# soham2560/MPCHoloNavigation

Hardware: AMD Instinct MI355X
Metric: rollouts/sec per computeVelocityCommands() tick (higher is better)
Workload: dtype f32

## Files before the change

mpcholonavigation_amd/csrc/smpc_api.cpp:

```cpp

#include "smpc_ctx.h"

#include <emmintrin.h>

namespace smpc_impl {

thread_local std::string g_create_error;

int fail(smpc_ctx* c, int code, const std::string& msg)
{
  if (c) c->err = msg; else g_create_error = msg;
  return code;
}

int wait_map_upload(smpc_ctx* c)
{
  if (!c->map_pending) return SMPC_OK;
  HIPCK(c, hipEventSynchronize(c->ev_map));
  c->map_pending = false;
  return SMPC_OK;
}

void bar_copy(void* dev_dst, const void* host_src, size_t n)
{
  const __m128i* src = static_cast<const __m128i*>(host_src);
  __m128i* dst = static_cast<__m128i*>(dev_dst);
  for (size_t i = 0; i < n / 16; ++i) _mm_stream_si128(dst + i, _mm_load_si128(src + i));
  _mm_sfence();
}

void bar_flush(const smpc_ctx* c)
{
  if (c->hdp_flush) *c->hdp_flush = 1u;
}

static volatile uint32_t* find_hdp_flush(int dev)
{
  hipDeviceProp_t prop;
  if (hipGetDeviceProperties(&prop, dev) != hipSuccess) return nullptr;
  void* h = dlopen("libhsa-runtime64.so.1", RTLD_NOW | RTLD_NOLOAD);
  if (!h) h = dlopen("libhsa-runtime64.so.1", RTLD_NOW | RTLD_LOCAL);
  if (!h) return nullptr;
  using agent_t = struct {uint64_t handle;};
  using iterate_fn = int (*)(int (*)(agent_t, void*), void*);
  using info_fn = int (*)(agent_t, int, void*);
  using init_fn = int (*)();
  static init_fn p_init = reinterpret_cast<init_fn>(dlsym(h, "hsa_init"));
  static iterate_fn p_iter = reinterpret_cast<iterate_fn>(dlsym(h, "hsa_iterate_agents"));
  static info_fn p_info = reinterpret_cast<info_fn>(dlsym(h, "hsa_agent_get_info"));
  if (!p_init || !p_iter || !p_info || p_init() != 0) return nullptr;
  struct Want {
    uint32_t domain, bdf;
    volatile uint32_t* reg;
  } want{static_cast<uint32_t>(prop.pciDomainID),
         (static_cast<uint32_t>(prop.pciBusID) << 8) | (static_cast<uint32_t>(prop.pciDeviceID) << 3), nullptr};
  auto cb = [](agent_t a, void* data) -> int {
    Want* w = static_cast<Want*>(data);
    int type = 0;
    if (p_info(a, 17, &type) != 0 || type != 1) return 0;
    uint32_t bdf = 0, domain = 0;
    if (p_info(a, 0xA006, &bdf) != 0) return 0;
    if (p_info(a, 0xA00F, &domain) != 0) domain = w->domain;
    if ((bdf & ~7u) != w->bdf || domain != w->domain) return 0;
    struct {uint32_t* mem; uint32_t* reg;} f{nullptr, nullptr};
    if (p_info(a, 0xA00E, &f) == 0) w->reg = f.mem;
    return 1;
  };
  (void)p_iter(cb, &want);
  return want.reg;
}

void free_ctx(smpc_ctx* c)
{
  if (!c) return;
  (void)hipSetDevice(c->device);
  for (float* p : {c->d_tvx, c->d_nvx, c->d_nvy, c->d_nwz, c->d_costs[0], c->d_costs[1], c->d_traj[0],
         c->d_traj[1], c->d_traj[2], c->d_partials, c->d_tuple, c->d_out, c->d_u_iter, c->d_furthest})
    if (p) (void)hipFree(p);
  if (c->d_stats || c->d_stats_part) {
    (void)hipStreamSynchronize(c->stream);
    if (c->d_stats) (void)hipFree(c->d_stats);
    if (c->d_stats_part) (void)hipFree(c->d_stats_part);
  }
  for (hipEvent_t e : c->ev_stats) if (e) (void)hipEventDestroy(e);
  if (c->l_gm || c->l_rm[0] || c->l_rm[1] || c->l_rm[2]) {
    (void)hipStreamSynchronize(c->stream);
    for (float* p : {c->l_gm, c->l_rm[0], c->l_rm[1], c->l_rm[2]})
      if (p) (void)hipFree(p);
  }
  for (hipEvent_t e : c->ev_lim) if (e) (void)hipEventDestroy(e);
  if (c->fill_stream) {
    (void)hipStreamSynchronize(c->fill_stream);
    (void)hipStreamDestroy(c->fill_stream);
  }
  if (c->ev_fill) (void)hipEventDestroy(c->ev_fill);
  for (float* p : {c->b_tvx, c->b_nvx, c->b_nvy, c->b_nwz})
    if (p) (void)hipFree(p);
  if (c->d_map) (void)hipFree(c->d_map);
  if (c->d_timeline) (void)hipFree(c->d_timeline);
  if (c->map.cells) (void)hipHostFree(c->map.cells);
  if (c->ev_map) (void)hipEventDestroy(c->ev_map);
  if (c->d_tick && !c->defer_upload) (void)hipFree(c->d_tick);
  if (c->d_lut) (void)hipFree(c->d_lut);
  if (c->d_lut_fp) (void)hipFree(c->d_lut_fp);
  if (c->h_lut_fp) (void)hipHostFree(c->h_lut_fp);
  if (c->h_lut) (void)hipHostFree(c->h_lut);
  if (c->h_tick && !c->defer_upload) (void)hipHostFree(c->h_tick);
  if (c->h_out) (void)hipHostFree(c->h_out);
  if (c->comm && rccl()) (void)rccl()->CommDestroy(c->comm);
  if (c->d_all) (void)hipFree(c->d_all);
  for (uint32_t r = 0; r < c->p2p.world; ++r)
    if (r != c->p2p.rank && c->p2p.peer[r]) (void)hipIpcCloseMemHandle(c->p2p.peer[r]);
  if (c->p2p_mailbox) (void)hipFree(c->p2p_mailbox);
  if (c->ev0) (void)hipEventDestroy(c->ev0);
  if (c->ev1) (void)hipEventDestroy(c->ev1);
  for (hipEvent_t e : c->evp) if (e) (void)hipEventDestroy(e);
  if (c->own_stream) (void)hipStreamDestroy(c->own_stream);
  delete c;
}

void begin_limit_iteration(smpc_ctx* c, const float* u_dev)
{
  c->lim_u_dev = u_dev;
  if (++c->lim_iter == 0) ++c->lim_iter;
}

static int limit_noise(smpc_ctx* c, bool group_major)
{
  const uint32_t B = c->cfg.batch_size, T = c->cfg.time_steps;
  SmpcLimitArgs a{};
  if (group_major) {
    const size_t ngm = SMPC_GM_ELEMS(B, T);
    if (!c->l_gm) {
      HIPCK(c, hipMalloc(&c->l_gm, 3 * ngm * sizeof(float)));
      HIPCK(c, hipMemsetAsync(c->l_gm, 0, 3 * ngm * sizeof(float), c->stream));
    }
    a.src[0] = c->d_tvx; a.src[1] = c->holonomic ? c->d_tvy : nullptr; a.src[2] = c->d_twz;
    a.dst[0] = c->l_gm; a.dst[1] = c->holonomic ? c->l_gm + ngm : nullptr; a.dst[2] = c->l_gm + 2 * ngm;
  } else {
    const int rc = ensure_row_major(c);
    if (rc != SMPC_OK) return rc;
    for (int k = 0; k < 3; ++k)
      if (!c->l_rm[k] && (k != 1 || c->holonomic)) HIPCK(c, hipMalloc(&c->l_rm[k], static_cast<size_t>(B) * T * sizeof(float)));
    a.src[0] = c->d_nvx; a.src[1] = c->holonomic ? c->d_nvy : nullptr; a.src[2] = c->d_nwz;
    for (int k = 0; k < 3; ++k) a.dst[k] = c->l_rm[k];
  }
  a.B = B; a.T = T;
  a.u_dev = c->lim_u_dev;
  if (!a.u_dev) {
    const TickLayout tl = tick_layout(T, std::max(c->P, 1u));
    memcpy(a.u_arg, c->h_tick + tl.u, 3 * T * sizeof(float));
  }
  a.v0[0] = c->dev.svx; a.v0[1] = c->dev.svy; a.v0[2] = c->dev.swz;
  const float dt = c->cfg.model_dt;
  a.dhi[0] = dt * c->lim[0]; a.dhi[1] = dt * c->lim[2]; a.dhi[2] = dt * c->lim[3];
  a.dlo[0] = dt * c->lim[1]; a.dlo[1] = -a.dhi[1]; a.dlo[2] = -a.dhi[2];
  const bool prof = (c->cfg.flags & SMPC_FLAG_PROFILE) != 0;
  if (prof) {
    for (hipEvent_t& e : c->ev_lim)
      if (!e) HIPCK(c, hipEventCreate(&e));
    HIPCK(c, hipEventRecord(c->ev_lim[0], c->stream));
  }
  c->launched = true;
  HIPCK(c, smpc_launch_limit_noise(a, group_major, c->stream));
  if (prof) HIPCK(c, hipEventRecord(c->ev_lim[1], c->stream));
  return SMPC_OK;
}

int use_limited_noise(smpc_ctx* c, SmpcDev& d, bool group_major)
{
  if (!c->lim_on) return SMPC_OK;
  uint32_t& have = group_major ? c->lim_gm_iter : c->lim_rm_iter;
  if (have != c->lim_iter || c->lim_iter == 0) {
    if (c->lim_iter == 0) begin_limit_iteration(c, nullptr);
    const int rc = limit_noise(c, group_major);
    if (rc != SMPC_OK) return rc;
    have = c->lim_iter;
  }
  if (group_major) {
    const size_t ngm = SMPC_GM_ELEMS(c->cfg.batch_size, c->cfg.time_steps);
    d.tvx = c->l_gm; d.tvy = c->l_gm + ngm; d.twz = c->l_gm + 2 * ngm;
  } else {
    d.nvx = c->l_rm[0]; d.nwz = c->l_rm[2];
    if (c->holonomic) d.nvy = c->l_rm[1];
  }
  return SMPC_OK;
}

int launch_furthest(smpc_ctx* c, float* d_furthest)
{
  {
    const int rc = ensure_row_major(c);
    if (rc != SMPC_OK) return rc;
  }
  HIPCK(c, hipMemsetAsync(d_furthest, 0, sizeof(float), c->stream));
  SmpcDev d = c->dev;
  {
    const int rc = use_limited_noise(c, d, false);
    if (rc != SMPC_OK) return rc;
  }
  d.flags = c->gate_flags & SD_NEED_FURTHEST;
  d.furthest_out = reinterpret_cast<uint32_t*>(d_furthest);
  SmpcLds L = make_lds(0, c->P, d.T, (pass_block(c->R) / 64), false);
  c->launched = true;
  HIPCK(c, wave_launch(wave_select(c->R, 1, d.T), d, L, c->plan.wave.grid, c->plan.wave.block, c->stream));
  return SMPC_OK;
}

int begin_tick(smpc_ctx* c, const smpc_tick_in* in, const float* u_in)
{
  const int rc = prepare_tick(c, in, u_in);
  if (rc != SMPC_OK) return rc;
  c->passes = 0;
  c->evp_used = 0;
  c->costs_cur = 0;
  return SMPC_OK;
}

int refuse_sharded(smpc_ctx* c)
{
  if (c->two_coll_fp)
    return fail(c, SMPC_ERR_UNSUPPORTED,
                "sharded tick: consider_footprint=true with both ObstaclesCritic and CostCritic in the list");
  if (c->cfg.iteration_count != 1)
    return fail(c, SMPC_ERR_UNSUPPORTED, "sharded tick: iteration_count must be 1");
  return SMPC_OK;
}

uint32_t next_seq(smpc_ctx* c)
{
  if (++c->seq == 0) ++c->seq;
  c->poll_seq = c->seq;
  return c->seq;
}

void fill_score_args(smpc_ctx* c, uint32_t flags, const float* u_dev, const float* d_furthest,
                     uint32_t furthest_hint, bool finish, const float* finish_furthest, SmpcDev& d,
                     SmpcFinal& fin)
{
  d = c->dev;
  d.flags = flags;
  if (u_dev) {
    d.u = u_dev;
    d.u_inline = 0;
  }
  d.d_furthest = d_furthest;
  d.furthest_hint = furthest_hint;
  d.costs = c->d_costs[c->costs_cur];
  d.costs_prev = c->d_costs[c->costs_cur ^ 1];
  fin = SmpcFinal{};
  fin.enabled = finish ? 1 : 0;
  fin.vx_max = c->c_vx_max; fin.vx_min = c->c_vx_min; fin.vy_max = c->c_vy; fin.wz_max = c->c_wz;
  fin.u_dev = c->d_out; fin.u_host = c->h_out_dev; fin.furthest_used = finish_furthest;
  if (finish && c->knobs.poll) {
    fin.done_counter = scratch_word(c, SMPC_SCRATCH_REDUCE_COUNTER);
    fin.seq = next_seq(c);
  }
  if (finish && c->acker_r >= 0.f) {
    c->acker_seq = fin.seq;
    fin.done_counter = nullptr;
    fin.seq = 0;
  }
}

struct PassChoice {
  PassPlan::Kind kind;
  const void* inst;
  const PassGeom* geom;
};
static PassChoice pass_for(const smpc_ctx* c, uint32_t flags)
{
  const PassPlan& pl = c->plan;
  const uint32_t T = c->dev.T;
  if (pl.kind == PassPlan::kSplit)
    if (const SplitInst* k = split_select(flags, T, c->dev.step, pl.split_nseg)) return {PassPlan::kSplit, k, &pl.split};
  if (pl.kind != PassPlan::kWave) {
    const LaneInst* k = lane_select(flags, T, pl.rr, false, c->acker_r, pl.pow, pl.nh);
    if (k || !(pl.rr || (flags & SD_STORE_TRAJ))) return {PassPlan::kLane, k, &pl.lane};
  }
  return {PassPlan::kWave, wave_select(c->R, c->score_mode, T), &pl.wave};
}

int launch_score(smpc_ctx* c, uint32_t flags, const float* u_dev, const float* d_furthest,
                 uint32_t furthest_hint, float* d_tuple, bool finish, const float* finish_furthest)
{
  SmpcDev d;
  SmpcFinal fin;
  fill_score_args(c, flags, u_dev, d_furthest, furthest_hint, finish, finish_furthest, d, fin);
  const PassChoice pass = pass_for(c, flags);
  {
    const int rc = use_limited_noise(c, d, pass.kind != PassPlan::kWave);
    if (rc != SMPC_OK) return rc;
  }
  const bool prof = (c->cfg.flags & SMPC_FLAG_PROFILE) && c->evp_used + 2 <= 8;
  if (prof) HIPCK(c, hipEventRecord(c->evp[c->evp_used], c->stream));
  const uint32_t nblk = pass.geom->grid;
  const bool tail = pass.kind != PassPlan::kSplit && c->knobs.fused_reduce && nblk <= SMPC_TAIL_MAX_GRID &&
    (pass.kind != PassPlan::kLane || pass.geom->block == smpc_lane_block()) && pass.geom->lds.total >= smpc_tail_lds_bytes(d.T);
  const bool polled = fin.enabled && fin.done_counter;
  c->poll_words = !polled ? 0u : tail ? smpc_tail_reduce_blocks(d.T, nblk) : smpc_reduce_blocks(d.T);
  static_assert(smpc_reduce_blocks(64u * SMPC_MAX_R) <= kPollWords, "one completion word per reducing block");
  if (tail) {
    float& mark = c->h_out[SMPC_RESULT_AT(d.T) + SMPC_R_MARK];
    if (mark == SMPC_MARK_TAIL_LATE) mark = SMPC_MARK_NONE;
    d.tail = 1;
    d.tail_counter = scratch_word(c, SMPC_SCRATCH_TAIL_COUNTER);
    d.tuple = d_tuple;
    d.fin = fin;
  }
  c->launched = true;
  c->last_pass_kind = pass.kind;
  if (pass.kind == PassPlan::kSplit) {
    HIPCK(c, split_launch(static_cast<const SplitInst*>(pass.inst), d, pass.geom->lds, nblk, c->stream));
  } else if (pass.kind == PassPlan::kLane) {
    HIPCK(c, lane_launch(static_cast<const LaneInst*>(pass.inst), d, nullptr, 1, pass.geom->lds, nblk, pass.geom->block, c->stream));
  } else {
    const int rc_rm = ensure_row_major(c);
    if (rc_rm != SMPC_OK) return rc_rm;
    HIPCK(c, wave_launch(static_cast<const WaveInst*>(pass.inst), d, pass.geom->lds, nblk, pass.geom->block, c->stream));
  }
  if (prof) {
    HIPCK(c, hipEventRecord(c->evp[c->evp_used + 1], c->stream));
    c->evp_used += 2;
  }
  if (!tail) HIPCK(c, smpc_launch_reduce(c->d_partials, nblk, d.T, d.neg_inv_temp, d_tuple, fin, c->stream));
  if (finish && c->acker_r >= 0.f)
    HIPCK(c, smpc_launch_ackermann(c->d_out, c->h_out_dev, d.T, c->acker_r, c->acker_seq, c->stream));
  c->passes++;
  return SMPC_OK;
}

int launch_combine(smpc_ctx* c, const float* d_tuples, uint32_t n, const float* d_furthest_used)
{
  const uint32_t T = c->cfg.time_steps;
  uint32_t seq = 0;
  if (c->knobs.poll) {
    seq = next_seq(c);
    c->poll_words = 0;
  }
  const bool acker = c->acker_r >= 0.f;
  HIPCK(c, smpc_launch_combine(d_tuples, n, T, c->dev.neg_inv_temp, c->c_vx_max, c->c_vx_min,
                               c->c_vy, c->c_wz, c->d_out, c->d_out + SMPC_RESULT_AT(T), d_furthest_used,
                               c->h_out_dev, acker ? 0u : seq, c->stream));
  if (acker) HIPCK(c, smpc_launch_ackermann(c->d_out, c->h_out_dev, T, c->acker_r, seq, c->stream));
  return SMPC_OK;
}

void store_control_sequence(const smpc_ctx* c, float* u_inout)
{
  const uint32_t T = c->cfg.time_steps;
  if (c->holonomic) {
    memcpy(u_inout, c->h_out, 3 * T * sizeof(float));
    return;
  }
  memcpy(u_inout, c->h_out, T * sizeof(float));
  memcpy(u_inout + 2 * T, c->h_out + 2 * T, T * sizeof(float));
}

static int check_canary(smpc_ctx* c)
{
  c->launched = false;
  if (!c->canary_expect) return SMPC_OK;
  const uint32_t got = reinterpret_cast<const volatile uint32_t*>(c->h_out)[SMPC_RESULT_AT(c->cfg.time_steps) + SMPC_R_CANARY];
  if (got == c->canary_expect) return SMPC_OK;
  char msg[200];
  snprintf(msg, sizeof(msg), "the scoring pass read tick block %u, not %u: the per-tick upload did not reach the "
           "device in time (CPU stores through the BAR: %s); SMPC_NO_BAR_TICK=1 selects the copy", got, c->canary_expect,
           c->bar_tick ? "on" : "off");
  c->bar_tick = false;
  return fail(c, SMPC_ERR_DEVICE, msg);
}

int fetch_out(smpc_ctx* c)
{
  if (c->poll_seq) {
    const volatile uint32_t* flag =
      reinterpret_cast<const volatile uint32_t*>(c->h_out + SMPC_RESULT_AT(c->cfg.time_steps) + SMPC_R_DONE);
    const uint32_t want = c->poll_seq;
    c->poll_seq = 0;
    const uint32_t nwords = c->poll_words;
    static_assert(SMPC_R_BLOCK_DONE == SMPC_R_DONE + 1u, "the per-block words follow the completion word");
    c->poll_words = 0;
    auto arrived = [&]() {
      if (nwords == 0) return *flag == want;
      for (uint32_t r = 0; r < nwords; ++r)
        if (flag[1 + r] != want) return false;
      return true;
    };
    for (uint32_t spin = 0; spin < 4000000u; ++spin) {
      if (arrived()) {
        __atomic_thread_fence(__ATOMIC_ACQUIRE);
        if (tick_result(c).mark() == SMPC_MARK_TAIL_LATE)
          return fail(c, SMPC_ERR_DEVICE, "the scoring launch's reduction did not see every block's partial");
        return check_canary(c);
      }
      __builtin_ia32_pause();
    }
  }
  HIPCK(c, hipStreamSynchronize(c->stream));
  return check_canary(c);
}

float profile_pass_ms(smpc_ctx* c)
{
  float sum = 0.f;
  uint32_t n = 0;
  for (uint32_t i = 0; i + 1 < c->evp_used; i += 2) {
    float ms = 0.f;
    if (hipEventElapsedTime(&ms, c->evp[i], c->evp[i + 1]) == hipSuccess) {
      sum += ms;
      n++;
    }
  }
  return n ? sum / n : 0.f;
}

int fill_tick_out(smpc_ctx* c, smpc_tick_out* out, bool fail_flag, bool furthest_valid, uint32_t furthest,
                  const float* non_colliding, bool device_ms)
{
  if (!out) return SMPC_OK;
  const TickResult r = tick_result(c);
  memset(out, 0, sizeof(*out));
  out->fail_flag = fail_flag ? 1 : 0;
  out->furthest_valid = furthest_valid ? 1 : 0;
  out->furthest_reached_path_point = furthest;
  out->non_colliding = static_cast<uint32_t>(non_colliding ? *non_colliding : r.non_colliding());
  out->min_cost = r.min_cost();
  out->sum_w = r.sum_w();
  out->passes = c->passes;
  if (device_ms && (c->cfg.flags & SMPC_FLAG_PROFILE)) {
    HIPCK(c, hipEventSynchronize(c->ev1));
    float ms = 0.f;
    if (hipEventElapsedTime(&ms, c->ev0, c->ev1) == hipSuccess) out->device_ms = ms;
  }
  out->score_pass_ms = profile_pass_ms(c);
  out->pass_kind = c->last_pass_kind;
  return SMPC_OK;
}

uint32_t fail_only_flags(const smpc_ctx* c)
{
  const uint32_t coll = (c->gate_flags & SD_COST) ? (SD_COST | SD_FP_COST) : (SD_OBSTACLES | SD_FP_OBSTACLES);
  return c->gate_flags & (SD_CONSTRAINT | coll | SD_STORE_TRAJ | SD_TRACK_UNKNOWN);
}

uint32_t scoring_flags(const smpc_ctx* c, bool fail_sticky)
{
  const uint32_t keep = SD_STORE_TRAJ | SD_TRACK_UNKNOWN;
  return fail_sticky ? (c->gate_flags & keep) : c->gate_flags;
}

int update_time_major(smpc_ctx* c)
{
  if (!c->use_tpr) return SMPC_OK;
  const uint32_t B = c->cfg.batch_size, T = c->cfg.time_steps;
  HIPCK(c, smpc_launch_relayout(c->d_nvx, c->d_tvx, B, T, true, c->stream));
  HIPCK(c, smpc_launch_relayout(c->d_nvy, c->d_tvy, B, T, true, c->stream));
  HIPCK(c, smpc_launch_relayout(c->d_nwz, c->d_twz, B, T, true, c->stream));
  return SMPC_OK;
}

int ensure_row_major(smpc_ctx* c)
{
  if (c->rm_valid) return SMPC_OK;
  const uint32_t B = c->cfg.batch_size, T = c->cfg.time_steps;
  HIPCK(c, smpc_launch_relayout(c->d_tvx, c->d_nvx, B, T, false, c->stream));
  if (c->holonomic) HIPCK(c, smpc_launch_relayout(c->d_tvy, c->d_nvy, B, T, false, c->stream));
  HIPCK(c, smpc_launch_relayout(c->d_twz, c->d_nwz, B, T, false, c->stream));
  c->rm_valid = true;
  return SMPC_OK;
}

static int launch_draw(smpc_ctx* c, float* nvx, float* nvy, float* nwz, float* tvx, float* tvy, float* twz,
                       hipStream_t st, bool* rm_valid_out)
{
  const uint64_t n = static_cast<uint64_t>(c->cfg.batch_size) * c->cfg.time_steps;
  const uint64_t base = c->cfg.shard_offset * c->cfg.time_steps;
  const uint32_t B = c->cfg.batch_size, T = c->cfg.time_steps;
  if (c->use_tpr && (T & 3u) == 0 && !getenv("SMPC_NO_FUSED_FILL")) {
    HIPCK(c, smpc_launch_fill_noise_tm(tvx, B, T, base, c->seed, 0, c->epoch, c->cfg.vx_std, st));
    HIPCK(c, smpc_launch_fill_noise_tm(twz, B, T, base, c->seed, 1, c->epoch, c->cfg.wz_std, st));
    if (c->holonomic)
      HIPCK(c, smpc_launch_fill_noise_tm(tvy, B, T, base, c->seed, 2, c->epoch, c->cfg.vy_std, st));
    else
      HIPCK(c, hipMemsetAsync(tvy, 0, SMPC_GM_ELEMS(B, T) * sizeof(float), st));
    *rm_valid_out = false;
    return SMPC_OK;
  }
  HIPCK(c, smpc_launch_fill_noise(nvx, n, base, c->seed, 0, c->epoch, c->cfg.vx_std, st));
  HIPCK(c, smpc_launch_fill_noise(nwz, n, base, c->seed, 1, c->epoch, c->cfg.wz_std, st));
  if (c->holonomic) HIPCK(c, smpc_launch_fill_noise(nvy, n, base, c->seed, 2, c->epoch, c->cfg.vy_std, st));
  if (c->use_tpr) {
    HIPCK(c, smpc_launch_relayout(nvx, tvx, B, T, true, st));
    HIPCK(c, smpc_launch_relayout(nvy, tvy, B, T, true, st));
    HIPCK(c, smpc_launch_relayout(nwz, twz, B, T, true, st));
  }
  *rm_valid_out = true;
  return SMPC_OK;
}

int cancel_redraw(smpc_ctx* c)
{
  if (!c->redraw_pending) return SMPC_OK;
  HIPCK(c, hipEventSynchronize(c->ev_fill));
  c->redraw_pending = false;
  return SMPC_OK;
}

int absorb_redraw(smpc_ctx* c)
{
  if (!c->redraw_pending) return SMPC_OK;
  HIPCK(c, hipStreamWaitEvent(c->stream, c->ev_fill, 0));
  std::swap(c->d_nvx, c->b_nvx);
  std::swap(c->d_nvy, c->b_nvy);
  std::swap(c->d_nwz, c->b_nwz);
  std::swap(c->d_tvx, c->b_tvx);
  std::swap(c->d_tvy, c->b_tvy);
  std::swap(c->d_twz, c->b_twz);
  c->rm_valid = c->redraw_rm_valid;
  c->redraw_pending = false;
  c->noise_gen++;
  return SMPC_OK;
}

int draw_noise(smpc_ctx* c)
{
  int rc = cancel_redraw(c);
  if (rc != SMPC_OK) return rc;
  bool rm = true;
  rc = launch_draw(c, c->d_nvx, c->d_nvy, c->d_nwz, c->d_tvx, c->d_tvy, c->d_twz, c->stream, &rm);
  if (rc != SMPC_OK) return rc;
  HIPCK(c, hipStreamSynchronize(c->stream));
  c->have_noise = true;
  c->rm_valid = rm;
  c->noise_gen++;
  return SMPC_OK;
}

int redraw_async(smpc_ctx* c)
{
  if (c->redraw_pending) return SMPC_OK;
  const size_t n = static_cast<size_t>(c->cfg.batch_size) * c->cfg.time_steps * sizeof(float);
  if (!c->fill_stream) {
    HIPCK(c, hipStreamCreateWithFlags(&c->fill_stream, hipStreamNonBlocking));
    HIPCK(c, hipEventCreateWithFlags(&c->ev_fill, hipEventDisableTiming));
  }
  if (c->use_tpr && !c->b_tvx) {
    const size_t ngm = SMPC_GM_ELEMS(c->cfg.batch_size, c->cfg.time_steps) * sizeof(float);
    HIPCK(c, hipMalloc(&c->b_tvx, 3 * ngm));
    HIPCK(c, hipMemset(c->b_tvx, 0, 3 * ngm));
    c->b_tvy = c->b_tvx + ngm / sizeof(float);
    c->b_twz = c->b_tvy + ngm / sizeof(float);
  }
  if (!c->b_nvx) {
    HIPCK(c, hipMalloc(&c->b_nvx, n));
    HIPCK(c, hipMalloc(&c->b_nvy, n));
    HIPCK(c, hipMalloc(&c->b_nwz, n));
    if (!c->holonomic) HIPCK(c, hipMemset(c->b_nvy, 0, n));
  }
  c->epoch++;
  bool rm = true;
  const int rc = launch_draw(c, c->b_nvx, c->b_nvy, c->b_nwz, c->b_tvx, c->b_tvy, c->b_twz, c->fill_stream, &rm);
  if (rc != SMPC_OK) return rc;
  HIPCK(c, hipEventRecord(c->ev_fill, c->fill_stream));
  c->redraw_rm_valid = rm;
  c->redraw_pending = true;
  return SMPC_OK;
}

static Knobs read_knobs()
{
  Knobs k;
  auto set = [](const char* name) {return getenv(name) != nullptr;};
  auto number = [](const char* name, int unset) {const char* e = getenv(name); return e ? atoi(e) : unset;};
  if (const char* e = getenv("SMPC_PASS"))
    k.pass = !strcmp(e, "wave") ? Knobs::kWave : !strcmp(e, "lane") ? Knobs::kLane : !strcmp(e, "split") ? Knobs::kSplit : Knobs::kAuto;
  k.no_split = set("SMPC_NO_SPLIT");
  k.split_nseg = static_cast<uint32_t>(std::max(0, number("SMPC_SPLIT_NSEG", 0)));
  k.lane_reread = number("SMPC_LANE_REREAD", 0) != 0;
  k.half_blocks = !set("SMPC_NO_HALF_BLOCKS");
  k.max_blocks_per_cu = static_cast<uint32_t>(std::max(0, number("SMPC_MAX_BLOCKS_PER_CU", 0)));
  k.balanced_grid = !set("SMPC_NO_BALANCED_GRID");
  k.fused_reduce = set("SMPC_FUSED_REDUCE");
  k.no_inline_tick = set("SMPC_NO_INLINE_TICK");
  k.pinned_tick = set("SMPC_PINNED_TICK");
  k.poll = !set("SMPC_NO_POLL");
  k.bar_tick = !set("SMPC_NO_BAR_TICK");
  k.hdp_flush = !set("SMPC_NO_HDP_FLUSH");
  k.repeat_pass = set("SMPC_DEBUG_REPEAT_PASS");
  k.stale_tick = static_cast<uint32_t>(number("SMPC_DEBUG_STALE_TICK", 0));
  k.small_window = set("SMPC_SMALL_WINDOW");
  k.window_side_max = number("SMPC_WINDOW_SIDE_MAX", -1);
  k.furthest_prune = number("SMPC_FURTHEST_PRUNE", 1) != 0;
  if (const char* e = getenv("SMPC_FOOTPRINT_PASS")) k.footprint_general = !strcmp(e, "general");
  if (const char* e = getenv("SMPC_NONHOLO_PASS")) k.nonholo_omni = !strcmp(e, "omni");
  return k;
}

using clk = std::chrono::steady_clock;
static void report_tick_timing(clk::time_point t_in, clk::time_point t_prep, clk::time_point t_launch, clk::time_point t_fetch)
{
  static thread_local double acc[5] = {0, 0, 0, 0, 0};
  static thread_local unsigned n = 0;
  static thread_local clk::time_point t_prev_out;
  const auto t_out = clk::now();
  auto us = [](clk::time_point a, clk::time_point b) {return std::chrono::duration<double, std::micro>(b - a).count();};
  if (n > 0) acc[0] += us(t_prev_out, t_in);
  acc[1] += us(t_in, t_prep);
  acc[2] += us(t_prep, t_launch);
  acc[3] += us(t_launch, t_fetch);
  acc[4] += us(t_fetch, t_out);
  t_prev_out = t_out;
  if (++n == 1024) {
    fprintf(stderr, "[smpc tick timing] caller %.2f us, prepare + upload %.2f, launches %.2f, wait %.2f, collect %.2f (per tick, %u ticks)\n",
            acc[0] / (n - 1), acc[1] / n, acc[2] / n, acc[3] / n, acc[4] / n, n);
    n = 0;
    for (double& a : acc) a = 0;
  }
// ... 817 lines not shown
```

mpcholonavigation_amd/csrc/smpc_ctx.h:

```cpp
#ifndef SMPC_CTX_H_
#define SMPC_CTX_H_

#include <hip/hip_runtime.h>
#include <rccl/rccl.h>
#include <dlfcn.h>

#include <algorithm>
#include <chrono>
#include <cmath>
#include <cstdio>
#include <cstdlib>
#include <cstring>
#include <limits>
#include <new>
#include <string>
#include <vector>

#include "../../include/smpc.h"
#include "smpc_dev.h"
#include "smpc_inst.h"
#include "smpc_limit.h"

#pragma GCC visibility push(hidden)

hipError_t smpc_launch_reduce(const float* partials, uint32_t nblk, uint32_t T,
                              float neg_inv_temp, float* tuple, const SmpcFinal& fin,
                              hipStream_t st);
hipError_t smpc_launch_combine(const float* tuples, uint32_t G, uint32_t T, float neg_inv_temp,
                               float vx_max, float vx_min, float vy_max, float wz_max,
                               float* u_out, float* result, const float* furthest_used,
                               float* host_out, uint32_t seq, hipStream_t st);
hipError_t smpc_launch_fill_noise(float* out, uint64_t n, uint64_t base, uint64_t seed,
                                  uint32_t stream, uint32_t epoch, float sigma, hipStream_t st);
hipError_t smpc_launch_fill_noise_tm(float* dst, uint32_t B, uint32_t T, uint64_t base, uint64_t seed,
                                     uint32_t stream, uint32_t epoch, float sigma, hipStream_t st);
hipError_t smpc_launch_ackermann(float* u_dev, float* u_host, uint32_t T, float min_r, uint32_t seq,
                                 hipStream_t st);
hipError_t smpc_launch_p2p_exchange(const float* my_tuple, const SmpcP2P& x, uint32_t T, int mode,
                                    float* d_furthest, float neg_inv_temp, float vx_max, float vx_min,
                                    float vy_max, float wz_max, float* u_out, float* result,
                                    const float* furthest_used, float* host_out, uint32_t seq,
                                    hipStream_t st);

hipError_t smpc_launch_relayout(const float* src, float* dst, uint32_t B, uint32_t T, bool to_gm, hipStream_t st);
uint32_t smpc_lane_block();
uint32_t smpc_lane_block_rr();
hipError_t smpc_launch_lane_reduce(const float* v, const float* w, float* out, hipStream_t st);
hipError_t smpc_launch_row_reduce(const float* v, float* out, uint32_t n, hipStream_t st);
uint32_t smpc_split_block();
uint32_t smpc_split_rollouts_per_block(uint32_t nseg);
hipError_t smpc_launch_reduce_many(const SmpcReduceArgs* d_many, uint32_t n, uint32_t T, hipStream_t st);
hipError_t smpc_launch_sincos(const float* x, uint32_t n, float* sn, float* cs, hipStream_t st);
hipError_t smpc_launch_philox(const uint32_t* ctr, uint32_t k0, uint32_t k1, uint32_t n, uint32_t* out,
                              hipStream_t st);
hipError_t smpc_launch_box_muller(const uint32_t* r0, const uint32_t* r1, uint32_t n, float* z0, float* z1,
                                  hipStream_t st);

hipError_t smpc_launch_limit_noise(const SmpcLimitArgs& a, bool group_major, hipStream_t st);

namespace smpc_impl {

extern thread_local std::string g_create_error;


struct RcclApi {
  ncclResult_t (*GetUniqueId)(ncclUniqueId*) = nullptr;
  ncclResult_t (*CommInitRank)(ncclComm_t*, int, ncclUniqueId, int) = nullptr;
  ncclResult_t (*CommDestroy)(ncclComm_t) = nullptr;
  ncclResult_t (*AllGather)(const void*, void*, size_t, ncclDataType_t, ncclComm_t, hipStream_t) = nullptr;
  ncclResult_t (*AllReduce)(const void*, void*, size_t, ncclDataType_t, ncclRedOp_t, ncclComm_t,
                            hipStream_t) = nullptr;
  const char* (*GetErrorString)(ncclResult_t) = nullptr;
};
const RcclApi* rccl();

inline uint32_t pass_block(int R) {return R == 4 ? 512u : 1024u;}
constexpr uint32_t kLaneMinBatch = 60u * 1024u;
constexpr uint32_t kSplitMinBatch = 12u * 1024u;
constexpr uint32_t kSplitMinBatchShort = 20000u;
constexpr uint32_t kLaneMaxT = 128;
constexpr uint32_t kPollWords = SMPC_BLOCK_DONE_WORDS;
static_assert(SMPC_TUPLE_HEADER == SMPC_R_F_USED, "the shard tuple's header is the first four result slots, in their order");
constexpr uint32_t kMaxGrid = SMPC_MAX_GRID;
constexpr uint32_t kWindowBytes = 96 * 96;
constexpr uint32_t kWindowSideMax = 144;
constexpr uint32_t kLdsPerCu = 160 * 1024;

inline uint32_t align_up(uint32_t v, uint32_t a) {return (v + a - 1) / a * a;}

struct HostCostmap {
  uint8_t* cells = nullptr;
  size_t cap = 0;
  uint32_t W = 0, H = 0;
  double ox = 0, oy = 0, res = 1;
  bool track_unknown = false;
  float inscribed_radius = 0, cost_scaling_factor = 0, inflation_radius = 0;
  bool set = false;
};

inline bool world_to_map(const HostCostmap& c, double wx, double wy, unsigned& mx, unsigned& my)
{
  if (wx < c.ox || wy < c.oy) return false;
  const double qx = (wx - c.ox) / c.res, qy = (wy - c.oy) / c.res;
  if (!(qx < 4294967296.0) || !(qy < 4294967296.0)) return false;
  mx = static_cast<unsigned>(qx);
  my = static_cast<unsigned>(qy);
  return mx < c.W && my < c.H;
}

inline bool within_tol(float tol, double rx, double ry, double gx, double gy)
{
  const double dist_sq = std::pow(gx - rx, 2) + std::pow(gy - ry, 2);
  const float tol_sq = tol * tol;
  return dist_sq < tol_sq;
}

struct Knobs {
  enum Pass {kAuto, kWave, kLane, kSplit} pass = kAuto;
  bool no_split = false;
  uint32_t split_nseg = 0;
  bool lane_reread = false;
  bool half_blocks = true;
  uint32_t max_blocks_per_cu = 0;
  bool balanced_grid = true;
  bool fused_reduce = false;
  bool no_inline_tick = false;
  bool pinned_tick = false;
  bool poll = true;
  bool bar_tick = true;
  bool hdp_flush = true;
  bool repeat_pass = false;
  uint32_t stale_tick = 0;
  bool small_window = false;
  int window_side_max = -1;
  bool furthest_prune = true;
  bool footprint_general = false;
  bool nonholo_omni = false;
};

struct OccCache {
  const void* fn = nullptr;
  uint32_t block = 0, lds = 0;
  uint32_t blocks = 1;
  uint32_t get(const void* f, uint32_t blk, uint32_t lds_bytes)
  {
    if (f != fn || blk != block || lds_bytes != lds) {
      int nb = 0;
      if (inst_occupancy(f, blk, lds_bytes, &nb) != hipSuccess || nb < 1) nb = 1;
      fn = f; block = blk; lds = lds_bytes;
      blocks = static_cast<uint32_t>(nb);
    }
    return blocks;
  }
};

struct PassGeom {
  uint32_t grid = 0, block = 0;
  SmpcLds lds{};
};
struct PassPlan {
  enum Kind : uint32_t {kWave = 0, kLane = 1, kSplit = 2};
  Kind kind = kWave;
  PassGeom wave;
  PassGeom lane;
  PassGeom split;
  bool rr = false;
  bool pow = false;
  bool nh = false;
  uint32_t split_nseg = 4;
  uint32_t window_bytes = 0;
};

struct FurthestPredictor {
  bool hint_valid = false;
  uint32_t hint = 0;
  float hint_F = 0.f;
  float hint_Fp = 0.f;
  bool hint_Fp_valid = false;
  bool hint_is_this_ticks = false;
  float hint_drift = 0.f;
  bool anchor_valid = false;
  double anchor_x = 0, anchor_y = 0;
  double anchor_ex = 0, anchor_ey = 0, cur_ex = 0, cur_ey = 0;
  bool anchor_e_valid = false, cur_e_valid = false;
  std::vector<float> anchor_px, anchor_py;
  uint32_t noise_gen_remembered = 0;
  void forget()
  {
    hint_valid = false;
    hint_Fp_valid = false;
    hint_is_this_ticks = false;
    hint_drift = 0.f;
  }
  void drop_hint() {hint_valid = false;}
};

}

struct smpc_ctx {
  smpc_config cfg{};
  smpc_critic_params critics{};
  float c_vx_max = 0, c_vx_min = 0, c_vy = 0, c_wz = 0;
  int device = 0;
  int num_cu = 256;
  hipStream_t own_stream = nullptr, stream = nullptr;
  hipEvent_t ev0 = nullptr, ev1 = nullptr;
  hipEvent_t evp[8] = {};
  uint32_t evp_used = 0;
  float* d_nvx = nullptr;
  float* d_nvy = nullptr;
  float* d_nwz = nullptr;
  float* d_tvx = nullptr;
  float* d_tvy = nullptr;
  float* d_twz = nullptr;
  float* b_nvx = nullptr;
  float* b_nvy = nullptr;
  float* b_nwz = nullptr;
  float* b_tvx = nullptr;
  float* b_tvy = nullptr;
  float* b_twz = nullptr;
  hipStream_t fill_stream = nullptr;
  hipEvent_t ev_fill = nullptr;
  bool redraw_pending = false, redraw_rm_valid = true;
  uint32_t noise_gen = 0;
  bool use_tpr = false;
  bool rm_valid = true;
  smpc_impl::Knobs knobs;
  smpc_impl::PassPlan plan;
  smpc_impl::OccCache occ_wave, occ_lane, occ_split;
  bool lane_forced = false;
  bool two_coll_fp = false;
  uint32_t last_pass_kind = 0;
  bool defer_upload = false;
  std::vector<double> fp_x, fp_y;
  double fp_circumscribed_radius = 0.0, fp_layer_scale = -1.0;
  SmpcLut* d_lut_fp = nullptr;
  SmpcLut* h_lut_fp = nullptr;
  ncclComm_t comm = nullptr;
  int comm_rank = 0, comm_world = 0;
  float* d_all = nullptr;
  float* p2p_mailbox = nullptr;
  SmpcP2P p2p{};
  uint32_t p2p_xseq = 0;
  uint32_t p2p_timeout_ms = 10000;
  bool p2p_failed = false;
  bool pang_any = false;
  float prune_table[SMPC_PRUNE_FLOATS] = {};
  std::vector<float> prune_px, prune_py;
  uint32_t prune_k0 = 0;
  bool in_group = false;
  float* d_costs[2] = {nullptr, nullptr};
  float* d_traj[3] = {nullptr, nullptr, nullptr};
  int costs_cur = 0;
  bool have_noise = false, rng_mode = false;
  uint64_t seed = 0;
  uint32_t epoch = 0;
  smpc_impl::HostCostmap map;
  uint8_t* d_map = nullptr;
  size_t d_map_bytes = 0;
  hipEvent_t ev_map = nullptr;
  bool map_pending = false;
  uint64_t map_bytes_last = 0, map_bytes_total = 0;
  unsigned long long* d_timeline = nullptr;
  SmpcLut* d_lut = nullptr;
  SmpcLut* h_lut = nullptr;
  uint64_t lut_key = 0, map_version = 1, critics_version = 1;
  bool lut_valid = false;
  uint8_t* d_tick = nullptr;
  uint8_t* h_tick = nullptr;
  size_t tick_cap = 0;
  bool bar_tick = false;
  volatile uint32_t* hdp_flush = nullptr;
  size_t tick_used = 0;
  uint32_t tick_no = 0;
  uint32_t canary_expect = 0;
  bool launched = false;
  float* d_partials = nullptr;
  float* d_tuple = nullptr;
  float* d_out = nullptr;
  float* d_u_iter = nullptr;
  float* h_out = nullptr;
  float* h_out_dev = nullptr;
  float* d_furthest = nullptr;
  int R = 1;
  SmpcDev dev{};
  uint32_t gate_flags = 0;
  int score_mode = 0;
  static int score_mode_for(const smpc_critic_params& cr)
  {
    return (cr.obstacles.cost_power == 1 && cr.path_align.cost_power == 1 &&
           cr.path_follow.cost_power == 1 && cr.goal_angle.cost_power == 1 &&
           cr.prefer_forward.cost_power == 1) ? 0 : 2;
  }
  bool tick_ready = false;
  bool fail_in = false;
  uint32_t P = 0;
  uint32_t passes = 0;
  smpc_impl::FurthestPredictor pred;
  uint64_t spec_misses = 0;
  smpc_tick_in step_in{};
  std::vector<float> step_px, step_py;
  bool step_remembered = false;
  bool holonomic = true;
  float acker_r = -1.f;
  uint32_t acker_seq = 0;
  uint32_t seq = 0, poll_seq = 0;
  uint32_t poll_words = 0;
  float* d_stats = nullptr;
  double* d_stats_part = nullptr;
  uint32_t stats_ld = 0;
  bool lim_on = false;
  float lim[4] = {0.f, 0.f, 0.f, 0.f};
  float* l_rm[3] = {nullptr, nullptr, nullptr};
  float* l_gm = nullptr;
  const float* lim_u_dev = nullptr;
  uint32_t lim_iter = 0;
  uint32_t lim_rm_iter = 0, lim_gm_iter = 0;
  hipEvent_t ev_lim[2] = {};
  hipEvent_t ev_stats[4] = {};
  float stats_pass_ms = 0.f, stats_reduce_ms = 0.f;
  std::string err;
};

namespace smpc_impl {

int fail(smpc_ctx* c, int code, const std::string& msg);

#define HIPCK(ctx, call)                                                               \
  do {                                                                                 \
    hipError_t e__ = (call);                                                           \
    if (e__ != hipSuccess)                                                             \
      return fail(ctx, SMPC_ERR_DEVICE,                                                \
                  std::string(#call) + ": " + hipGetErrorString(e__));                \
  } while (0)

int wait_map_upload(smpc_ctx* c);
void bar_copy(void* dev_dst, const void* host_src, size_t n);
void bar_flush(const smpc_ctx* c);
void free_ctx(smpc_ctx* c);

struct TickLayout {
  size_t u, px, py, pyaw, D, pf_idx, pvalid, pa_active, pang_active, pal_active, lut_cost, canary, prune, total;
};
TickLayout tick_layout(uint32_t T, uint32_t P);
void build_prune_table(const float* px, const float* py, uint32_t P, uint32_t k0, bool on, float* out);

SmpcLds make_lds(uint32_t window_bytes, uint32_t P, uint32_t T, uint32_t nwave, bool with_map,
                 uint32_t nsamp = 0);
SmpcLds lane_lds(uint32_t window_bytes, uint32_t P, uint32_t T, bool rr = false);
SmpcLds split_lds(uint32_t window_bytes, uint32_t P, uint32_t T, uint32_t nseg);

int check_tick(smpc_ctx* c, const smpc_tick_in* in);
void remember_furthest(smpc_ctx* c, const smpc_tick_in* in, float F);
void predict_hint(smpc_ctx* c, const smpc_tick_in* in, const float* u_in);
int prepare_tick(smpc_ctx* c, const smpc_tick_in* in, const float* u_in);

int launch_furthest(smpc_ctx* c, float* d_furthest);
void fill_score_args(smpc_ctx* c, uint32_t flags, const float* u_dev, const float* d_furthest,
                     uint32_t furthest_hint, bool finish, const float* finish_furthest, SmpcDev& d,
                     SmpcFinal& fin);
int launch_score(smpc_ctx* c, uint32_t flags, const float* u_dev, const float* d_furthest,
                 uint32_t furthest_hint, float* d_tuple, bool finish = false,
                 const float* finish_furthest = nullptr);
int launch_combine(smpc_ctx* c, const float* d_tuples, uint32_t n, const float* d_furthest_used);
void store_control_sequence(const smpc_ctx* c, float* u_inout);
int fetch_out(smpc_ctx* c);

int begin_tick(smpc_ctx* c, const smpc_tick_in* in, const float* u_in);
int refuse_sharded(smpc_ctx* c);
uint32_t next_seq(smpc_ctx* c);
inline uint32_t* scratch_word(const smpc_ctx* c, uint32_t k) {return reinterpret_cast<uint32_t*>(c->d_furthest) + k;}
struct TickResult {
  const float* slot;
  float min_cost() const {return slot[SMPC_R_MIN_COST];}
  float sum_w() const {return slot[SMPC_R_SUM_W];}
  float F_local() const {return slot[SMPC_R_F_LOCAL];}
  float non_colliding() const {return slot[SMPC_R_NON_COLLIDING];}
  float F_used() const {return slot[SMPC_R_F_USED];}
  float mark() const {return slot[SMPC_R_MARK];}
};
inline TickResult tick_result(const smpc_ctx* c) {return TickResult{c->h_out + SMPC_RESULT_AT(c->cfg.time_steps)};}
int fill_tick_out(smpc_ctx* c, smpc_tick_out* out, bool fail_flag, bool furthest_valid, uint32_t furthest,
                  const float* non_colliding = nullptr, bool device_ms = false);
float profile_pass_ms(smpc_ctx* c);
uint32_t fail_only_flags(const smpc_ctx* c);
uint32_t scoring_flags(const smpc_ctx* c, bool fail_sticky);
void begin_limit_iteration(smpc_ctx* c, const float* u_dev);
int use_limited_noise(smpc_ctx* c, SmpcDev& d, bool group_major);
int update_time_major(smpc_ctx* c);
int ensure_row_major(smpc_ctx* c);
int draw_noise(smpc_ctx* c);
int redraw_async(smpc_ctx* c);
int cancel_redraw(smpc_ctx* c);
int absorb_redraw(smpc_ctx* c);

}

#pragma GCC visibility pop

#endif
```

mpcholonavigation_amd/csrc/smpc_dev.h:

```cpp
#ifndef SMPC_DEV_H_
#define SMPC_DEV_H_

#include <stdint.h>

#define SD_OBSTACLES 0x001u
#define SD_PATH_ALIGN 0x002u
#define SD_PATH_FOLLOW 0x004u
#define SD_GOAL_ANGLE 0x008u
#define SD_PREFER_FORWARD 0x010u
#define SD_USE_PATH_YAW 0x020u
#define SD_ACCUMULATE 0x040u
#define SD_STORE_TRAJ 0x080u
#define SD_TRACK_UNKNOWN 0x100u
#define SD_NEED_FURTHEST 0x200u
#define SD_LOCAL_FURTHEST 0x400u
#define SD_CONSTRAINT 0x800u
#define SD_COST 0x1000u
#define SD_GOAL 0x2000u
#define SD_TWIRLING 0x4000u
#define SD_PATH_ANGLE 0x8000u
#define SD_DEADBAND 0x10000u
#define SD_FP_OBSTACLES 0x20000u
#define SD_FP_COST 0x40000u
#define SD_PATH_ALIGN_LEGACY 0x80000u
#define SD_PAL_USE_PATH_YAW 0x100000u
#define SD_EXTRA_CRITICS (SD_CONSTRAINT | SD_COST | SD_GOAL | SD_TWIRLING | SD_PATH_ANGLE | SD_DEADBAND | \
                          SD_FP_OBSTACLES | SD_FP_COST | SD_PATH_ALIGN_LEGACY)

#define SMPC_GM_ROLLOUTS(B) ((((B) + 63u) / 64u) * 64u)
#define SMPC_GM_STEPS(T) (((T) + 3u) & ~3u)
#define SMPC_GM_ELEMS(B, T) ((size_t)SMPC_GM_ROLLOUTS(B) * SMPC_GM_STEPS(T))
#define SMPC_GM_INDEX(b, t, T) \
  (((((size_t)(b) >> 6) * (SMPC_GM_STEPS(T) >> 2) + ((t) >> 2)) * 64u + ((b) & 63u)) * 4u + ((t) & 3u))

#define SMPC_MAX_PATH 1024
#define SMPC_MAX_R 4

struct SmpcLut {
  float crit;
  float rep;
};

struct SmpcFinal {
  int enabled;
  float vx_max, vx_min, vy_max, wz_max;
  float* u_dev;
  float* u_host;
  const float* furthest_used;
  uint32_t* done_counter;
  uint32_t seq;
};

struct SmpcDev {
  uint32_t B, T, P;
  uint32_t nsamp;
  uint32_t step;
  uint32_t flags;
  double x0, y0;
  float yaw0, cos0, sin0;
  float svx, svy, swz;
  float dt;
  const float* nvx;
  const float* nvy;
  const float* nwz;
  const float* tvx;
  const float* tvy;
  const float* twz;
  const float* u;
  const float* costs_prev;
  float* costs;
  float* traj_x;
  float* traj_y;
  float* traj_yaw;
  const uint8_t* map;
  uint32_t W, H;
  double ox, oy, res;
  float oxf, oyf, rinvf;
  float cell_eps;
  uint32_t cost_t0;
  int32_t win_x0, win_y0, win_w, win_h;
  float wxf, wyf;
  float cxf, cyf;
  float cell_eps_w;
  float x00f, y00f;
  const SmpcLut* lut;
  const float* px;
  const float* py;
  const float* pyaw;
  const float* D;
  const uint8_t* pvalid;
  const uint8_t* pa_active;
  const uint32_t* pf_idx;
  const float* prune;
  const float* d_furthest;
  uint32_t furthest_hint;
  float obs_critical_w, obs_repulsion_w, obs_collision_cost;
  float obs_rep_over_T;
  uint32_t obs_power;
  float pa_weight;
  uint32_t pa_power;
  float pf_weight;
  uint32_t pf_power;
  float ga_weight, ga_goal_yaw;
  uint32_t ga_power;
  float pfw_weight;
  uint32_t pfw_power;
  float con_weight, con_max_vel, con_min_vel;
  uint32_t con_power;
  float con_acker_r;
  const float* lut_cost;
  float cost_w254, cost_collision_cost;
  float cost_critical;
  uint32_t cost_near_goal;
  uint32_t cost_power;
  double goal_x, goal_y;
  float goal_weight;
  uint32_t goal_power;
  float tw_weight;
  uint32_t tw_power;
  const uint8_t* pang_active;
  float pang_weight;
  uint32_t pang_power, pang_offset;
  int32_t pang_correct;
  const uint8_t* pal_active;
  float pal_weight, pal_eval;
  uint32_t pal_power;
  double db_vx, db_vy, db_wz;
  float db_weight;
  uint32_t db_power;
  uint32_t fp_n;
  float fp_pic;
  const SmpcLut* lut_fp;
  double fp_x[16], fp_y[16];
  float g_vx, g_vy, g_wz;
  float neg_inv_temp;
  float k2;
  float* partials;
  uint32_t* furthest_out;
  uint32_t tail;
  uint32_t* tail_counter;
  float* tuple;
  SmpcFinal fin;
  unsigned long long* timeline;
  uint32_t canary_echo;
  uint32_t tick_inline;
  uint32_t u_inline;
  uint16_t io_px, io_py, io_pyaw, io_D, io_pf_idx, io_pvalid, io_pa_active, io_pang_active, io_pal_active, io_pad;
  uint8_t tick_bytes[1536] __attribute__((aligned(16)));
  float u_arg[3 * 64] __attribute__((aligned(16)));
};
#define SMPC_INLINE_TICK_CAP 1536u
#define SMPC_MAX_GRID 2048u
#define SMPC_CANARY_SLOT(T) (SMPC_MAX_GRID * (4u + 3u * (T)))
#define SMPC_TAIL_MAX_GRID 512u
#define SMPC_TAIL_STAMPS_AT (8192u + 2048u * 8u)
#define SMPC_SCAN_COUNT_AT (SMPC_TAIL_STAMPS_AT + 8u * 16u)
#define SMPC_PRUNE_ENTRIES 16u
#define SMPC_PRUNE_FLOATS (4u + 8u * SMPC_PRUNE_ENTRIES)
static inline uint32_t smpc_tail_lds_bytes(uint32_t T) {return (512u + 64u + ((4u + 3u * T + 63u) / 64u) * 2048u + 4u) * 4u;}

#define SMPC_R_MIN_COST 0u
#define SMPC_R_SUM_W 1u
#define SMPC_R_F_LOCAL 2u
#define SMPC_R_NON_COLLIDING 3u
#define SMPC_R_F_USED 4u
#define SMPC_R_CANARY 5u
#define SMPC_R_MARK 6u
#define SMPC_R_DONE 7u
#define SMPC_R_BLOCK_DONE 8u
#define SMPC_BLOCK_DONE_WORDS 32u
#define SMPC_RESULT_AT(T) (3u * (T))
#define SMPC_RESULT_FLOATS(T) (SMPC_RESULT_AT(T) + SMPC_R_BLOCK_DONE)
#define SMPC_RESULT_HOST_FLOATS(T) (SMPC_RESULT_FLOATS(T) + SMPC_BLOCK_DONE_WORDS)
static_assert(SMPC_R_MIN_COST == 0u && SMPC_R_SUM_W == 1u && SMPC_R_F_LOCAL == 2u && SMPC_R_NON_COLLIDING == 3u &&
              SMPC_R_F_USED == 4u, "result slots 0-4: the tuple header, then the furthest point used");
static_assert(SMPC_R_CANARY == 5u && SMPC_R_MARK == 6u && SMPC_R_DONE == 7u && SMPC_R_BLOCK_DONE == 8u,
              "result slots 5-8: canary echo, mark, completion word, per-block completion words");
static inline constexpr uint32_t smpc_tuple_floats(uint32_t T) {return SMPC_R_F_USED + 3u * T;}
#define SMPC_MARK_NONE 0.0f
#define SMPC_MARK_PEER_LATE 1.0f
#define SMPC_MARK_TAIL_LATE 2.0f
static inline constexpr uint32_t smpc_reduce_blocks(uint32_t T) {return (smpc_tuple_floats(T) + 31u) / 32u;}
static inline constexpr uint32_t smpc_tail_reduce_blocks(uint32_t T, uint32_t grid)
{
  const uint32_t groups = (smpc_tuple_floats(T) + 63u) / 64u;
  return groups < grid ? groups : grid;
}

#define SMPC_SCRATCH_FURTHEST 0u
#define SMPC_SCRATCH_REDUCE_COUNTER 2u
#define SMPC_SCRATCH_P2P_STATE 3u
#define SMPC_SCRATCH_TAIL_COUNTER 4u
#define SMPC_SCRATCH_WORDS 8u
static_assert(SMPC_SCRATCH_TAIL_COUNTER + 2u <= SMPC_SCRATCH_WORDS, "the scratch allocation holds every word");

#if defined(__HIPCC__)
struct SmpcTickPtrs {
  const float* u;
  const float* px;
  const float* py;
  const float* pyaw;
  const float* D;
  const uint32_t* pf_idx;
  const uint8_t* pvalid;
  const uint8_t* pa_active;
  const uint8_t* pang_active;
  const uint8_t* pal_active;
};
__device__ __forceinline__ SmpcTickPtrs smpc_tick_ptrs(const SmpcDev& p, bool kernarg_is_dev)
{
  SmpcTickPtrs t{p.u, p.px, p.py, p.pyaw, p.D, p.pf_idx, p.pvalid, p.pa_active, p.pang_active, p.pal_active};
#if defined(__HIP_DEVICE_COMPILE__)
  if (kernarg_is_dev && p.tick_inline) {
    const uint8_t* k = reinterpret_cast<const uint8_t*>(__builtin_amdgcn_kernarg_segment_ptr()) +
                       __builtin_offsetof(SmpcDev, tick_bytes);
    if (p.u_inline) t.u = reinterpret_cast<const float*>(reinterpret_cast<const uint8_t*>(__builtin_amdgcn_kernarg_segment_ptr()) +
                                                         __builtin_offsetof(SmpcDev, u_arg));
    t.px = reinterpret_cast<const float*>(k + p.io_px);
    t.py = reinterpret_cast<const float*>(k + p.io_py);
    t.pyaw = reinterpret_cast<const float*>(k + p.io_pyaw);
    t.D = reinterpret_cast<const float*>(k + p.io_D);
    t.pf_idx = reinterpret_cast<const uint32_t*>(k + p.io_pf_idx);
    t.pvalid = k + p.io_pvalid;
    t.pa_active = k + p.io_pa_active;
    t.pang_active = k + p.io_pang_active;
    t.pal_active = k + p.io_pal_active;
  }
#else
  (void)kernarg_is_dev;
#endif
  return t;
}
#endif

#if defined(__HIPCC__)
__host__ __device__
#endif
static inline uint32_t smpc_furthest_index(float F) {return (uint32_t)(F + 0.5f);}


#define SMPC_P2P_MAX_RANKS 16
struct SmpcP2P {
  float* peer[SMPC_P2P_MAX_RANKS];
  uint32_t world, rank;
  uint32_t slot_floats;
  uint32_t xseq;
  uint32_t* state;
  unsigned long long timeout_ticks;
};

struct SmpcReduceArgs {
  const float* partials;
  float* tuple;
  uint32_t nblk;
  SmpcFinal fin;
  float* host_out;
  uint32_t seq;
  float neg_inv_temp;
};

struct SmpcLds {
  uint32_t off_lut, off_px, off_py, off_pyaw, off_D, off_valid, off_scr;
  uint32_t off_pts4;
  uint32_t off_prune;
  uint32_t scr_stride;
  uint32_t scr_pts;
  uint32_t scr_ring;
  uint32_t scr_c;
  uint32_t seg_shift;
  uint32_t group;
  uint32_t total;
};

struct SmpcWaveGeom {
  SmpcLds lds;
  uint32_t grid;
};

struct SmpcStatsDst {
  float* stats;
  uint32_t ld;
};

#endif
```

mpcholonavigation_amd/csrc/smpc_group.cpp:

```cpp
#include "smpc_ctx.h"
#include "smpc_group.h"

using namespace smpc_impl;

extern "C" {

int smpc_group_create(smpc_ctx* const* ctxs, uint32_t n, smpc_group** out)
{
  if (!ctxs || !n || !out) return fail(nullptr, SMPC_ERR_INVALID, "null argument");
  *out = nullptr;
  for (uint32_t i = 0; i < n; ++i) {
    if (!ctxs[i]) return fail(nullptr, SMPC_ERR_INVALID, "null ctx");
    if (ctxs[i]->device != ctxs[0]->device || ctxs[i]->cfg.time_steps != ctxs[0]->cfg.time_steps)
      return fail(nullptr, SMPC_ERR_INVALID, "a group's contexts share the device and time_steps");
    if (ctxs[i]->defer_upload) return fail(nullptr, SMPC_ERR_STATE, "ctx already in a group");
  }
  smpc_group* g = new (std::nothrow) smpc_group();
  if (!g) return fail(nullptr, SMPC_ERR_NOMEM, "out of memory");
  smpc_ctx* c0 = ctxs[0];
  if (hipSetDevice(c0->device) != hipSuccess) {
    delete g;
    return fail(nullptr, SMPC_ERR_DEVICE, "hipSetDevice");
  }
  g->slot = align_up(static_cast<uint32_t>(c0->tick_cap), 256);
  g->off_dev = g->slot * n;
  g->off_red = g->off_dev + align_up(static_cast<uint32_t>(sizeof(SmpcDev)) * n, 256);
  g->off_geo = g->off_red + align_up(static_cast<uint32_t>(sizeof(SmpcReduceArgs)) * n, 256);
  g->total = g->off_geo + align_up(static_cast<uint32_t>(sizeof(SmpcWaveGeom)) * n, 256);
  g->off_fdev = g->total;
  g->off_fgeo = g->off_fdev + align_up(static_cast<uint32_t>(sizeof(SmpcDev)) * n, 256);
  g->off_sdst = g->off_fgeo + align_up(static_cast<uint32_t>(sizeof(SmpcWaveGeom)) * n, 256);
  g->off_sred = g->off_sdst + align_up(static_cast<uint32_t>(sizeof(SmpcStatsDst)) * n, 256);
  g->total_stats = g->off_sred + align_up(static_cast<uint32_t>(sizeof(SmpcStatsReduceArgs)) * n, 256);
  if (hipHostMalloc(&g->h_all, g->total_stats, hipHostMallocDefault) != hipSuccess ||
    hipMalloc(&g->d_all, g->total_stats) != hipSuccess)
  {
    if (g->h_all) (void)hipHostFree(g->h_all);
    delete g;
    return fail(nullptr, SMPC_ERR_NOMEM, "group buffers");
  }
  g->stream = c0->own_stream;
  for (uint32_t i = 0; i < n; ++i) {
    smpc_ctx* c = ctxs[i];
    (void)hipStreamSynchronize(c->stream);
    g->ctxs.push_back(c);
    g->saved_stream.push_back(c->stream);
    g->saved_h_tick.push_back(c->h_tick);
    g->saved_d_tick.push_back(c->d_tick);
    c->stream = g->stream;
    c->h_tick = g->h_all + g->slot * i;
    c->d_tick = g->d_all + g->slot * i;
    c->defer_upload = true;
    c->in_group = true;
    c->lut_valid = false;
  }
  *out = g;
  return SMPC_OK;
}

void smpc_group_destroy(smpc_group* g)
{
  if (!g) return;
  (void)hipStreamSynchronize(g->stream);
  for (size_t i = 0; i < g->ctxs.size(); ++i) {
    smpc_ctx* c = g->ctxs[i];
    c->stream = g->saved_stream[i];
    c->h_tick = g->saved_h_tick[i];
    c->d_tick = g->saved_d_tick[i];
    c->defer_upload = false;
    c->in_group = false;
  }
  if (g->h_all) (void)hipHostFree(g->h_all);
  if (g->d_all) (void)hipFree(g->d_all);
  if (g->d_stats) (void)hipFree(g->d_stats);
  if (g->d_stats_part) (void)hipFree(g->d_stats_part);
  if (g->h_stats_out) (void)hipHostFree(g->h_stats_out);
  delete g;
}

int smpc_group_stats(const smpc_group* g, uint64_t* batched_launches, uint64_t* single_ticks)
{
  if (!g) return SMPC_ERR_INVALID;
  if (batched_launches) *batched_launches = g->batched_launches;
  if (single_ticks) *single_ticks = g->single_ticks;
  return SMPC_OK;
}

int smpc_group_optimize_some(smpc_group* g, const smpc_tick_in* ins, float* const* u_inout,
                             smpc_tick_out* outs, const uint8_t* take)
{
  if (!g || !ins || !u_inout) return fail(nullptr, SMPC_ERR_INVALID, "null argument");
  const uint32_t n = static_cast<uint32_t>(g->ctxs.size());
  auto taken = [&](uint32_t i) {return !take || take[i] != 0;};
  uint32_t first = 0;
  while (first < n && !taken(first)) ++first;
  if (first == n) return SMPC_OK;
  smpc_ctx* c0 = g->ctxs[first];
  HIPCK(c0, hipSetDevice(c0->device));
  if (g->launched) {
    HIPCK(c0, hipStreamSynchronize(g->stream));
    g->launched = false;
  }
  auto single = [&](uint32_t i) -> int {
    smpc_ctx* c = g->ctxs[i];
    c->defer_upload = false;
    const int rc = smpc_optimize(c, &ins[i], u_inout[i], outs ? &outs[i] : nullptr);
    c->defer_upload = true;
    g->single_ticks++;
    return rc;
  };
  static const bool timing = getenv("SMPC_GROUP_TIMING") != nullptr;
  auto now = [] {return std::chrono::steady_clock::now();};
  auto us_between = [](auto a, auto b) {return std::chrono::duration<double, std::micro>(b - a).count();};
  const auto t_start = now();
  const uint32_t T = c0->cfg.time_steps;
  std::vector<const void*> part(n, nullptr);
  std::vector<uint32_t> flags(n);
  bool lane_ok = true;
  uint32_t lane_first = n, Pmax = 0, window_bytes = 0, gridx = 0;
  const LaneInst* inst = nullptr;
  static const char kLaneTag = 0;
  for (uint32_t i = 0; i < n; ++i) {
    if (!taken(i)) continue;
    smpc_ctx* c = g->ctxs[i];
    if (!u_inout[i]) return fail(c, SMPC_ERR_INVALID, "null control sequence");
    int rc = begin_tick(c, &ins[i], u_inout[i]);
    if (rc != SMPC_OK) return rc;
    flags[i] = scoring_flags(c, c->fail_in);
    const bool need_f = (flags[i] & SD_NEED_FURTHEST) != 0;
    if (need_f) flags[i] |= SD_LOCAL_FURTHEST;
    const bool ok = c->cfg.iteration_count == 1 && !c->fail_in &&
      !(c->cfg.flags & (SMPC_FLAG_NO_SPECULATION | SMPC_FLAG_PROFILE)) && (!need_f || c->pred.hint_valid) &&
      c->knobs.poll && c->acker_r < 0.f && !c->two_coll_fp;
    if (!ok) continue;
    const LaneInst* k = c->plan.kind == PassPlan::kLane && !c->plan.rr && !c->plan.pow
      ? lane_select(flags[i], T, false, true, c->acker_r, false) : nullptr;
    if (k) {
      part[i] = &kLaneTag;
      if (lane_first == n) {
        lane_first = i;
        window_bytes = c->plan.window_bytes;
      }
      else if (c->plan.window_bytes != window_bytes || (inst && k->obst != inst->obst) ||
               c->plan.lane.block != g->ctxs[lane_first]->plan.lane.block)
        lane_ok = false;
      if (!inst || k->dep) inst = k;
      Pmax = std::max(Pmax, c->P);
      gridx = std::max(gridx, c->plan.lane.grid);
      continue;
    }
    if (c->plan.kind == PassPlan::kWave && c->R == 1 && !c->knobs.fused_reduce)
      part[i] = wave_select(c->R, c->score_mode, T, true);
  }
  SmpcLds L{};
  if (lane_first != n) {
    L = lane_lds(window_bytes, Pmax, T);
    if (L.total > kLdsPerCu) lane_ok = false;
  }
  struct Launch { const WaveInst* wave; uint32_t first, count, grid, lds; };
  std::vector<uint32_t> order;
  std::vector<Launch> launches;
  if (lane_first != n && lane_ok) {
    launches.push_back({nullptr, 0, 0, gridx, L.total});
    for (uint32_t i = 0; i < n; ++i)
      if (part[i] == &kLaneTag) order.push_back(i);
    launches.back().count = static_cast<uint32_t>(order.size());
  }
  for (uint32_t i = 0; i < n; ++i) {
    if (!part[i] || part[i] == &kLaneTag) continue;
    bool seen = false;
    for (const Launch& l : launches) seen = seen || l.wave == part[i];
    if (seen) continue;
    Launch l{static_cast<const WaveInst*>(part[i]), static_cast<uint32_t>(order.size()), 0, 0, 0};
    for (uint32_t j = i; j < n; ++j) {
      if (part[j] != part[i]) continue;
      order.push_back(j);
      l.count++;
      l.grid = std::max(l.grid, g->ctxs[j]->plan.wave.grid);
      l.lds = std::max(l.lds, g->ctxs[j]->plan.wave.lds.total);
    }
    if (l.count >= 2) launches.push_back(l);
    else order.pop_back();
  }
  {
    std::vector<bool> rides(n, false);
    for (uint32_t i : order) rides[i] = true;
    for (uint32_t i = 0; i < n; ++i) {
      if (rides[i] || !taken(i)) continue;
      const int rc = single(i);
      if (rc != SMPC_OK) return rc;
    }
  }
  if (order.empty()) return SMPC_OK;
  const uint32_t m = static_cast<uint32_t>(order.size());
  const auto t_prep = now();
  SmpcDev* hd = reinterpret_cast<SmpcDev*>(g->h_all + g->off_dev);
  SmpcReduceArgs* hr = reinterpret_cast<SmpcReduceArgs*>(g->h_all + g->off_red);
  SmpcWaveGeom* hg = reinterpret_cast<SmpcWaveGeom*>(g->h_all + g->off_geo);
  for (const Launch& l : launches) {
    for (uint32_t j = l.first; j < l.first + l.count; ++j) {
      const uint32_t i = order[j];
      smpc_ctx* c = g->ctxs[i];
      if (l.wave) {
        const int rc = ensure_row_major(c);
        if (rc != SMPC_OK) return rc;
      }
      SmpcFinal fin;
      fill_score_args(c, flags[i], nullptr, nullptr, c->pred.hint, true, nullptr, hd[j], fin);
      {
        const int rc = use_limited_noise(c, hd[j], !l.wave);
        if (rc != SMPC_OK) return rc;
      }
      hr[j].partials = c->d_partials;
      hr[j].tuple = c->d_tuple;
      hr[j].nblk = l.wave ? c->plan.wave.grid : gridx;
      hr[j].host_out = fin.u_host;
      hr[j].seq = fin.seq;
      hr[j].neg_inv_temp = c->dev.neg_inv_temp;
      fin.u_host = nullptr;
      fin.done_counter = nullptr;
      hr[j].fin = fin;
      hg[j].lds = c->plan.wave.lds;
      hg[j].grid = c->plan.wave.grid;
      c->passes++;
      c->last_pass_kind = l.wave ? PassPlan::kWave : PassPlan::kLane;
    }
  }
  if (c0->bar_tick) {
    for (uint32_t i : order) bar_copy(g->d_all + g->slot * i, g->h_all + g->slot * i, g->ctxs[i]->tick_used);
    bar_copy(g->d_all + g->off_dev, g->h_all + g->off_dev, g->total - g->off_dev);
    bar_flush(c0);
  }
  else HIPCK(c0, hipMemcpyAsync(g->d_all, g->h_all, g->total, hipMemcpyHostToDevice, g->stream));
  for (const Launch& l : launches) {
    const SmpcDev* d_dev = reinterpret_cast<const SmpcDev*>(g->d_all + g->off_dev) + l.first;
    if (l.wave) {
      HIPCK(c0, wave_launch_many(l.wave, d_dev, reinterpret_cast<const SmpcWaveGeom*>(g->d_all + g->off_geo) + l.first,
                                 l.count, l.grid, l.lds, pass_block(1), g->stream));
    } else {
      HIPCK(c0, lane_launch(inst, c0->dev, d_dev, l.count, L, l.grid, g->ctxs[lane_first]->plan.lane.block, g->stream));
    }
    g->launched = true;
    if (l.count >= 2) g->batched_launches++;
  }
  HIPCK(c0, smpc_launch_reduce_many(reinterpret_cast<const SmpcReduceArgs*>(g->d_all + g->off_red), m,
                                    T, g->stream));
  g->batched_ticks++;
  const auto t_launch = now();
  for (uint32_t i : order) {
    smpc_ctx* c = g->ctxs[i];
    int rc = fetch_out(c);
    if (rc != SMPC_OK) return rc;
    const bool need_f = (flags[i] & SD_NEED_FURTHEST) != 0;
    const TickResult res = tick_result(c);
    const float F_true = res.F_local();
    const uint32_t S_true = smpc_furthest_index(F_true);
    const bool miss = need_f && S_true != c->pred.hint;
    const bool all_collide = (flags[i] & (SD_OBSTACLES | SD_COST)) && res.non_colliding() == 0.0f;
    if (miss || all_collide) {
      if (miss) {
        c->spec_misses++;
        remember_furthest(c, &ins[i], F_true);
        c->pred.hint_F = F_true;
        c->pred.hint_is_this_ticks = true;
      }
      rc = single(i);
      if (rc != SMPC_OK) return rc;
      if (outs) outs[i].passes++;
      continue;
    }
    if (need_f) remember_furthest(c, &ins[i], F_true);
    store_control_sequence(c, u_inout[i]);
    rc = fill_tick_out(c, outs ? &outs[i] : nullptr, false, need_f, need_f ? S_true : 0u);
    if (rc != SMPC_OK) return rc;
  }
  g->launched = false;
  if (timing && (g->batched_ticks % 64) == 0)
    fprintf(stderr, "[smpc_group] prepare %.1f us, fill+launch %.1f us, wait+collect %.1f us; batched %llu single %llu\n",
            us_between(t_start, t_prep), us_between(t_prep, t_launch), us_between(t_launch, now()),
            (unsigned long long)g->batched_ticks, (unsigned long long)g->single_ticks);
  return SMPC_OK;
}

int smpc_group_optimize(smpc_group* g, const smpc_tick_in* ins, float* const* u_inout,
                        smpc_tick_out* outs)
{
  return smpc_group_optimize_some(g, ins, u_inout, outs, nullptr);
}

}
```

mpcholonavigation_amd/csrc/smpc_inst.h:

```cpp
#ifndef SMPC_INST_H_
#define SMPC_INST_H_

#include <hip/hip_runtime.h>
#include <stdint.h>

#include "smpc_dev.h"

#pragma GCC visibility push(hidden)

struct WaveInst { int r, mode; bool full, many; const void* fn; };
struct LaneInst { bool full, obst, many; int nch; bool rr, ga, quads; int tc; bool dep; const void* fn; bool pow, nh; };
struct SplitInst { int nseg; bool full; const void* fn; };

const WaveInst* wave_select(int R, int mode, uint32_t T, bool many = false);
const LaneInst* lane_select(uint32_t flags, uint32_t T, bool rr, bool many, float acker_r, bool pow, bool nh = false);
const SplitInst* split_select(uint32_t flags, uint32_t T, uint32_t step, uint32_t nseg);

const LaneInst* lane_occupancy_row(uint32_t T, bool rr);
const SplitInst* split_occupancy_row(uint32_t nseg);

hipError_t wave_launch(const WaveInst* k, const SmpcDev& p, const SmpcLds& L, uint32_t grid, uint32_t block, hipStream_t st);
hipError_t wave_launch_many(const WaveInst* k, const SmpcDev* d_many, const SmpcWaveGeom* d_geom, uint32_t n, uint32_t grid_max,
                            uint32_t lds_max, uint32_t block, hipStream_t st);
hipError_t lane_launch(const LaneInst* k, const SmpcDev& p, const SmpcDev* d_many, uint32_t n, const SmpcLds& L,
                       uint32_t grid, uint32_t block, hipStream_t st);
hipError_t split_launch(const SplitInst* k, const SmpcDev& p, const SmpcLds& L, uint32_t grid, hipStream_t st);

struct StatsInst { int r; bool full; const void* fn; };
const StatsInst* stats_select(int R, uint32_t T);
hipError_t stats_launch(const StatsInst* k, const SmpcDev& p, const SmpcLds& L, float* stats, uint32_t ld, uint32_t grid,
                        uint32_t block, hipStream_t st);
hipError_t stats_set_lds_limit(int bytes);
struct SmpcStatsOut {
  uint32_t best_rollout;
  float best_cost, effective_samples;
  float non_colliding;
  float sum[13], min[13], max[13], weighted[13], at_best[13];
};
uint32_t stats_reduce_slices(uint32_t B, uint32_t* slice_out);
hipError_t stats_launch_reduce(const float* stats, uint32_t ld, const float* costs, uint32_t B, float k2, double* part,
                               const float* pass_partials, uint32_t nblk, uint32_t T, SmpcStatsOut* out, hipStream_t st);

struct StatsManyInst { int r; bool full; const void* fn; const void* fn_furthest; };
const StatsManyInst* stats_many_select(int R, uint32_t T);
hipError_t stats_many_set_lds_limit(int bytes);
struct SmpcStatsReduceArgs {
  const float* stats;
  const float* costs;
  double* part;
  const float* pass_partials;
  SmpcStatsOut* out;
  uint32_t ld, B, slice, S;
  uint32_t nblk, TL;
  float k2;
};
hipError_t stats_launch_furthest_many(const StatsManyInst* k, const SmpcDev* d_many, const SmpcWaveGeom* d_geom, uint32_t n,
                                      uint32_t grid_max, uint32_t lds_max, uint32_t block, hipStream_t st);
hipError_t stats_launch_many(const StatsManyInst* k, const SmpcDev* d_many, const SmpcWaveGeom* d_geom, const SmpcStatsDst* d_dst,
                             uint32_t n, uint32_t grid_max, uint32_t lds_max, uint32_t block, hipStream_t st);
hipError_t stats_launch_reduce_many(const SmpcStatsReduceArgs* d_many, uint32_t n, uint32_t slices_max, hipStream_t st);

hipError_t wave_set_lds_limit(int bytes);
hipError_t lane_set_lds_limit(int bytes);
hipError_t split_set_lds_limit(int bytes);

extern char smpc_last_pass_kernel[96];

template <typename Inst, size_t N>
inline hipError_t inst_set_lds_limit(const Inst (&table)[N], int bytes)
{
  hipError_t e = hipSuccess;
  for (size_t k = 0; k < N && e == hipSuccess; ++k)
    e = hipFuncSetAttribute(table[k].fn, hipFuncAttributeMaxDynamicSharedMemorySize, bytes);
  return e;
}

inline hipError_t inst_occupancy(const void* fn, uint32_t block, uint32_t lds_bytes, int* blocks_per_cu)
{
  if (!fn) return hipErrorInvalidValue;
  return hipOccupancyMaxActiveBlocksPerMultiprocessor(blocks_per_cu, fn, static_cast<int>(block), lds_bytes);
}

inline hipError_t inst_launch(const void* fn, dim3 grid, uint32_t block, void** args, uint32_t lds_bytes, hipStream_t st)
{
  (void)hipLaunchKernel(fn, grid, dim3(block), args, lds_bytes, st);
  return hipGetLastError();
}

#pragma GCC visibility pop

#endif
```

mpcholonavigation_amd/csrc/smpc_lane.hip:

```cpp

#include <hip/hip_runtime.h>
#include <stdint.h>
#include <stdio.h>

#include <type_traits>

#include "smpc_dev.h"
#include "smpc_device_math.h"
#include "smpc_tail.h"
#include "smpc_lane_common.h"
#include "smpc_inst.h"

#ifndef WAVE
#define WAVE 64
#endif
#define LANE_BLOCK 512
#define LANE_BLOCK_RR 512

template <bool TO_GM>
__global__ void __launch_bounds__(256) smpc_relayout(const float* __restrict__ src, float* __restrict__ dst,
                                                    uint32_t B, uint32_t T)
{
  __shared__ float tile[32][33];
  const uint32_t b0 = blockIdx.x * 32, t0 = blockIdx.y * 32;
  const uint32_t lx = threadIdx.x & 31, ly = threadIdx.x >> 5;
  if (TO_GM) {
    for (uint32_t k = ly; k < 32; k += 8) {
      const uint32_t b = b0 + k, t = t0 + lx;
      tile[k][lx] = (b < B && t < T) ? src[(size_t)b * T + t] : 0.f;
    }
    __syncthreads();
    for (uint32_t k = ly; k < 32; k += 8) {
      const uint32_t e = k * 32 + lx, tl = 4 * (e >> 7) + (e & 3), bb = (e >> 2) & 31;
      const uint32_t t = t0 + tl, b = b0 + bb;
      if (b < B && t < T) dst[SMPC_GM_INDEX(b, t, T)] = tile[bb][tl];
    }
  } else {
    for (uint32_t k = ly; k < 32; k += 8) {
      const uint32_t e = k * 32 + lx, tl = 4 * (e >> 7) + (e & 3), bb = (e >> 2) & 31;
      const uint32_t t = t0 + tl, b = b0 + bb;
      tile[bb][tl] = (b < B && t < T) ? src[SMPC_GM_INDEX(b, t, T)] : 0.f;
    }
    __syncthreads();
    for (uint32_t k = ly; k < 32; k += 8) {
      const uint32_t b = b0 + k, t = t0 + lx;
      if (b < B && t < T) dst[(size_t)b * T + t] = tile[k][lx];
    }
  }
}

hipError_t smpc_launch_relayout(const float* src, float* dst, uint32_t B, uint32_t T, bool to_gm, hipStream_t st)
{
  const dim3 grid((B + 31) / 32, (T + 31) / 32);
  if (to_gm) hipLaunchKernelGGL(smpc_relayout<true>, grid, dim3(256), 0, st, src, dst, B, T);
  else hipLaunchKernelGGL(smpc_relayout<false>, grid, dim3(256), 0, st, src, dst, B, T);
  return hipGetLastError();
}

__global__ void __launch_bounds__(64) smpc_lane_reduce_kernel(const float* __restrict__ v,
                                                              const float* __restrict__ w,
                                                              float* __restrict__ out)
{
  const int lane = threadIdx.x;
  float V[64];
#pragma unroll
  for (int t = 0; t < 64; ++t) V[t] = v[lane * 64 + t];
  const LaneW lw = lane_weights(w[lane], lane);
  out[lane] = lane_reduce64(V, lw, lane);
}

hipError_t smpc_launch_lane_reduce(const float* v, const float* w, float* out, hipStream_t st)
{
  hipLaunchKernelGGL(smpc_lane_reduce_kernel, dim3(1), dim3(64), 0, st, v, w, out);
  return hipGetLastError();
}

#define LANE_PASS_KERNEL smpc_pass_lane
#define LANE_PASS_POW false
#define LANE_PASS_NH false
#include "smpc_lane_pass.inc"
#undef LANE_PASS_KERNEL
#undef LANE_PASS_POW
#undef LANE_PASS_NH
#define LANE_PASS_KERNEL smpc_pass_lane_pow
#define LANE_PASS_POW true
#define LANE_PASS_NH false
#include "smpc_lane_pass.inc"
#undef LANE_PASS_KERNEL
#undef LANE_PASS_POW
#undef LANE_PASS_NH
#define LANE_PASS_KERNEL smpc_pass_lane_nh
#define LANE_PASS_POW false
#define LANE_PASS_NH true
#include "smpc_lane_pass.inc"
#undef LANE_PASS_KERNEL
#undef LANE_PASS_POW
#undef LANE_PASS_NH

#define LANE_INST(...) {__VA_ARGS__, reinterpret_cast<const void*>(&smpc_pass_lane<__VA_ARGS__>), false, false}
#define LANE_INST_POW(...) {__VA_ARGS__, reinterpret_cast<const void*>(&smpc_pass_lane_pow<__VA_ARGS__>), true, false}
#define LANE_INST_NH(...) {__VA_ARGS__, reinterpret_cast<const void*>(&smpc_pass_lane_nh<__VA_ARGS__>), false, true}
static const LaneInst kLaneInst[] = {
  LANE_INST(false, false, false, 1, false, false, false, 0, false),
  LANE_INST(true, false, false, 1, false, false, true, 0, false),
  LANE_INST(false, true, false, 1, false, false, false, 0, false),
  LANE_INST(true, true, false, 1, false, false, true, 0, false),
  LANE_INST(false, true, false, 1, false, false, true, 0, false),
  LANE_INST(false, true, false, 1, false, false, true, 56, false),
  LANE_INST(false, false, true, 1, false, false, false, 0, false),
  LANE_INST(true, false, true, 1, false, false, true, 0, false),
  LANE_INST(false, true, true, 1, false, false, false, 0, false),
  LANE_INST(true, true, true, 1, false, false, true, 0, false),
  LANE_INST(true, true, false, 1, true, false, true, 0, false),
  LANE_INST(true, true, false, 2, true, false, true, 0, false),
  LANE_INST(false, true, false, 1, false, true, false, 0, false),
  LANE_INST(true, true, false, 1, false, true, true, 0, false),
  LANE_INST(true, true, false, 1, false, false, true, 0, true),
  LANE_INST(false, true, false, 1, false, false, true, 56, true),
  LANE_INST(true, true, true, 1, false, false, true, 0, true),
  LANE_INST(false, true, true, 1, false, false, true, 56, true),
  LANE_INST_POW(true, true, false, 1, false, false, true, 0, false),
  LANE_INST_POW(false, true, false, 1, false, false, true, 0, false),
  LANE_INST_POW(false, true, false, 1, false, false, true, 56, false),
  LANE_INST_POW(false, true, false, 1, false, false, false, 0, false),
  LANE_INST_POW(true, true, false, 1, false, true, true, 0, false),
  LANE_INST_POW(false, true, false, 1, false, true, false, 0, false),
  LANE_INST_POW(true, false, false, 1, false, false, true, 0, false),
  LANE_INST_POW(false, false, false, 1, false, false, false, 0, false),
  LANE_INST_NH(true, true, false, 1, false, false, true, 0, false),
  LANE_INST_NH(false, true, false, 1, false, false, true, 56, false),
  LANE_INST_NH(false, true, false, 1, false, false, true, 0, false),
};
#undef LANE_INST
#undef LANE_INST_POW
#undef LANE_INST_NH

static const LaneInst* lane_find(bool full, bool obst, bool many, int nch, bool rr, bool ga, bool quads, int tc, bool dep,
                                 bool pow = false, bool nh = false)
{
  for (const LaneInst& k : kLaneInst)
    if (k.full == full && k.obst == obst && k.many == many && k.nch == nch && k.rr == rr && k.ga == ga &&
        k.quads == quads && k.tc == tc && k.dep == dep && k.pow == pow && k.nh == nh)
      return &k;
  return nullptr;
}

const LaneInst* lane_select(uint32_t flags, uint32_t T, bool rr, bool many, float acker_r, bool pow, bool nh)
{
  if (nh) {
    const LaneInst* k = lane_select(flags, T, rr, many, acker_r, pow, false);
    if (!k || !k->obst || k->many || k->rr || k->ga || k->dep || k->pow || !k->quads) return k;
    return lane_find(k->full, true, false, 1, false, false, true, k->tc, false, false, true);
  }
  const uint32_t dep_set = SD_CONSTRAINT | SD_COST | SD_TWIRLING, lean_extra = dep_set | SD_GOAL | SD_PATH_ANGLE;
  if (flags & (SD_STORE_TRAJ | SD_USE_PATH_YAW | (SD_EXTRA_CRITICS & ~lean_extra))) return nullptr;
  const bool obst = (flags & (SD_OBSTACLES | SD_COST)) != 0;
  const bool full = T == 64u;
  if (pow) {
    if (rr || many || T > 64u || (flags & lean_extra)) return nullptr;
    if (flags & SD_GOAL_ANGLE) return obst ? lane_find(full, true, false, 1, false, true, full, 0, false, true) : nullptr;
    if (obst && T == 56u) return lane_find(false, true, false, 1, false, false, true, 56, false, true);
    return lane_find(full, obst, false, 1, false, false, full || (obst && (T & 3u) == 0u), 0, false, true);
  }
  if (rr) {
    if (!(flags & SD_OBSTACLES) || (flags & (lean_extra | SD_GOAL_ANGLE)) || (T != 64u && T != 128u)) return nullptr;
    return lane_find(true, true, many, T > 64u ? 2 : 1, true, false, true, 0, false);
  }
  if (T > 64u) return nullptr;
  if (flags & dep_set) {
    if (!obst || (flags & (SD_GOAL_ANGLE | SD_GOAL)) || ((flags & SD_COST) && (flags & SD_OBSTACLES)) ||
        acker_r >= 0.f || (!full && T != 56u))
      return nullptr;
    return lane_find(full, true, many, 1, false, false, true, full ? 0 : 56, true);
  }
  if (flags & (SD_GOAL | SD_PATH_ANGLE)) return nullptr;
  if (flags & SD_GOAL_ANGLE)
    return obst ? lane_find(full, true, many, 1, false, true, full, 0, false) : nullptr;
  if (many) return lane_find(full, obst, true, 1, false, false, full, 0, false);
  if (obst && T == 56u) return lane_find(false, true, false, 1, false, false, true, 56, false);
  return lane_find(full, obst, false, 1, false, false, full || (obst && (T & 3u) == 0u), 0, false);
}

const LaneInst* lane_occupancy_row(uint32_t T, bool rr)
{
  if (rr) return lane_find(true, true, false, T > 64u ? 2 : 1, true, false, true, 0, false);
  return lane_find(T == 64u, true, false, 1, false, false, T == 64u, 0, false);
}

hipError_t lane_launch(const LaneInst* k, const SmpcDev& p, const SmpcDev* d_many, uint32_t n, const SmpcLds& L,
                       uint32_t grid, uint32_t block, hipStream_t st)
{
  if (!k || k->many != (d_many != nullptr)) return hipErrorInvalidValue;
  if (k->rr ? block != LANE_BLOCK_RR : (block != LANE_BLOCK && block != LANE_BLOCK / 2)) return hipErrorInvalidValue;
  auto b = [](bool v) {return v ? "true" : "false";};
  snprintf(smpc_last_pass_kernel, sizeof(smpc_last_pass_kernel), "smpc_pass_lane%s<%s, %s, %s, %d, %s, %s, %s, %d, %s>",
           k->pow ? "_pow" : (k->nh ? "_nh" : ""), b(k->full), b(k->obst), b(k->many), k->nch, b(k->rr), b(k->ga), b(k->quads), k->tc, b(k->dep));
  static const SmpcDev none{};
  void* args[] = {const_cast<SmpcDev*>(d_many ? &none : &p), const_cast<SmpcLds*>(&L), &d_many};
  return inst_launch(k->fn, d_many ? dim3(grid, n) : dim3(grid), block, args, L.total, st);
}

uint32_t smpc_lane_block() {return LANE_BLOCK;}
uint32_t smpc_lane_block_rr() {return LANE_BLOCK_RR;}

hipError_t lane_set_lds_limit(int bytes) {return inst_set_lds_limit(kLaneInst, bytes);}
```

mpcholonavigation_amd/csrc/smpc_lane_common.h:

```cpp
#ifndef SMPC_LANE_COMMON_H_
#define SMPC_LANE_COMMON_H_

#include <hip/hip_runtime.h>
#include <stdint.h>

#include "smpc_dev.h"
#include "smpc_device_math.h"

#ifndef WAVE
#define WAVE 64
#endif

typedef unsigned u32x2 __attribute__((ext_vector_type(2)));
typedef const float __attribute__((address_space(4))) * cfloat_p;
typedef float f32x32 __attribute__((ext_vector_type(32)));
typedef float f32x4 __attribute__((ext_vector_type(4)));
typedef float f32x2 __attribute__((ext_vector_type(2)));
#define LANE_PARK_STRIDE 68

struct LaneW {
  float wa, wb;
};

#define SMPC_DPP_NODE(NAME, CTRL, BANKS)                                                    \
  __device__ __forceinline__ float NAME(float a, float b)                                   \
  {                                                                                         \
    float t;                                                                                \
    asm("s_nop 1\n\t"                                                              \
                 "v_add_f32_dpp %0, %1, %1 " CTRL " row_mask:0xf bank_mask:0xf\n\t"         \
                 "v_add_f32_dpp %0, %2, %2 " CTRL " row_mask:0xf bank_mask:" BANKS          \
                 : "=&v"(t)                                                                 \
                 : "v"(a), "v"(b));                                                         \
    return t;                                                                               \
  }
SMPC_DPP_NODE(node_bit3, "row_ror:8", "0xc")
SMPC_DPP_NODE(node_bit2, "row_half_mirror", "0xa")

template <int CTRL>
__device__ __forceinline__ float dpp_mov(float v)
{
  return __uint_as_float(
    (uint32_t)__builtin_amdgcn_update_dpp(0, (int)__float_as_uint(v), CTRL, 0xF, 0xF, false));
}

template <int K, int Rr>
__device__ __forceinline__ float lane_reduce_node(const float (&V)[64], const LaneW& w, int lane)
{
  if constexpr (K == 0) {
    return V[Rr];
  } else {
    const float a = lane_reduce_node<K - 1, Rr>(V, w, lane);
    const float b = lane_reduce_node<K - 1, Rr + (64 >> K)>(V, w, lane);
    if constexpr (K == 1) {
      const u32x2 s = __builtin_amdgcn_permlane32_swap(__float_as_uint(a), __float_as_uint(b),
                                                       false, false);
      return fmaf(w.wa, __uint_as_float(s.x), w.wb * __uint_as_float(s.y));
    } else if constexpr (K == 2) {
      const u32x2 s = __builtin_amdgcn_permlane16_swap(__float_as_uint(a), __float_as_uint(b),
                                                       false, false);
      return __uint_as_float(s.x) + __uint_as_float(s.y);
    } else if constexpr (K == 3) {
      return node_bit3(a, b);
    } else if constexpr (K == 4) {
      return node_bit2(a, b);
    } else if constexpr (K == 5) {
      const float ta = a + dpp_mov<0x4E>(a);
      const float tb = b + dpp_mov<0x4E>(b);
      return (lane & 2) ? tb : ta;
    } else {
      const float ta = a + dpp_mov<0xB1>(a);
      const float tb = b + dpp_mov<0xB1>(b);
      return (lane & 1) ? tb : ta;
    }
  }
}

__device__ __forceinline__ LaneW lane_weights(float w, int lane)
{
  const float wo = __shfl_xor(w, 32, WAVE);
  LaneW r;
  r.wa = lane < 32 ? w : wo;
  r.wb = lane < 32 ? wo : w;
  return r;
}

__device__ __forceinline__ float lane_reduce64(const float (&V)[64], const LaneW& w, int lane)
{
  return lane_reduce_node<6, 0>(V, w, lane);
}

__device__ __forceinline__ int cvt_floor_i32(float q)
{
  int r;
  asm("v_cvt_flr_i32_f32 %0, %1" : "=v"(r) : "v"(q));
  return r;
}

__device__ __forceinline__ float add_min_zero(float acc, float x)
{
  float m;
  asm("v_min_f32 %1, 0, %2\n\tv_add_f32 %0, %0, %1" : "+v"(acc), "=&v"(m) : "v"(x));
  return acc;
}

__device__ __forceinline__ uint32_t cell_byte_exact(const SmpcDev& p, uint8_t* s_map, float x,
                                                    float y, uint32_t slot)
{
  const uint32_t nwin = (uint32_t)(p.win_w * p.win_h);
  uint32_t mx = 0, my = 0;
  bool on = cell_index_exact((double)x, p.ox, p.res, p.W, mx);
  on = cell_index_exact((double)y, p.oy, p.res, p.H, my) && on;
  if (!on) return nwin;
  const uint32_t wx = mx - (uint32_t)p.win_x0, wy = my - (uint32_t)p.win_y0;
  if (wx < (uint32_t)p.win_w && wy < (uint32_t)p.win_h) return wy * p.win_w + wx;
  s_map[nwin + 1 + slot] = p.map[(size_t)my * p.W + mx];
  return nwin + 1 + slot;
}

#endif
```

mpcholonavigation_amd/csrc/smpc_lane_furthest.inc:

```
    if (want_local_furthest) {
      int reps = 1;
      if constexpr (LANE_FURTHEST_PRUNE) {
        if (furthest_pending) {
          reps = 2;
        } else if (wave != 0 && grp == gw && grp + nW < ngroups &&
                   __builtin_amdgcn_readfirstlane((int)__float_as_uint(fmaxf(F_local, s_prune[2]))) == 0) {
          park[lane * LANE_PARK_STRIDE + 64] = x;
          park[lane * LANE_PARK_STRIDE + 65] = y;
          furthest_pending = true;
          reps = 0;
        }
      }
      for (int rep = 0; rep < reps; ++rep) {
      bool flive = live;
      if constexpr (LANE_FURTHEST_PRUNE) {
        if (rep == 1) {
          x = park[lane * LANE_PARK_STRIDE + 64];
          y = park[lane * LANE_PARK_STRIDE + 65];
          flive = true;
          furthest_pending = false;
        }
      }
      bool scan = true;
      if constexpr (LANE_FURTHEST_PRUNE) {
        const uint32_t* s_prune_u = reinterpret_cast<const uint32_t*>(s_prune);
        const float theta = __uint_as_float((uint32_t)__builtin_amdgcn_readfirstlane(
            (int)__float_as_uint(fmaxf(F_local, s_prune[2]))));
        const float Kf = rintf(theta);
        const uint32_t ent = (uint32_t)(int)Kf - s_prune_u[0];
        bool may_raise = flive;
        if (ent < s_prune_u[1]) {
          const f32x4 ea = reinterpret_cast<const f32x4*>(s_prune + 4)[2 * ent];
          const f32x4 eb = reinterpret_cast<const f32x4*>(s_prune + 4)[2 * ent + 1];
          const float ex = x - ea[0], ey = y - ea[1];
          const float ps = ea[2] * ex + ea[3] * ey, pt = ea[2] * ey - ea[3] * ex;
          const bool prunable = (fmaxf(fabsf(ps), fabsf(pt)) <= 1.0f) && (ps + eb[0] * fabsf(pt) <= eb[1]) &&
                                (Kf + fmaxf(ps * eb[2] + eb[3], -0.45f) <= theta);
          may_raise = flive && !prunable;
        }
        scan = __any(may_raise);
      }
      if (scan) {
      auto block_d2 = [&](const float* bx, const float* by, float (&dd)[4]) {
        const f32x4 qx = *reinterpret_cast<const f32x4*>(bx);
        const f32x4 qy = *reinterpret_cast<const f32x4*>(by);
#pragma unroll
        for (int e = 0; e < 4; ++e) {
          const float ex = qx[e] - x, ey = qy[e] - y;
          dd[e] = ex * ex + ey * ey;
        }
      };
      float best = 3.4028234663852886e38f;
      uint32_t bj = 0;
      const uint32_t P4 = (p.P + 3u) & ~3u;
      constexpr bool kWindow = !GA && !DEP && !MANY;
      const uint32_t j_lo = (kWindow && (S >> 2) > 3u) ? ((S >> 2) - 3u) << 2 : 0u;
      for (uint32_t j = j_lo; j < P4; j += 4) {
        float dd[4];
        block_d2(s_px + j, s_py + j, dd);
        const float mn = fminf(fminf(dd[0], dd[1]), fminf(dd[2], dd[3]));
        if (mn < best) {
          best = mn;
          bj = j;
        }
      }
      auto point_F = [&]() -> float {
        float dd[4];
        block_d2(s_px + bj, s_py + bj, dd);
        const uint32_t bi = bj + (dd[0] == best ? 0u : dd[1] == best ? 1u : dd[2] == best ? 2u : dd[3] == best ? 3u : 0u);
        float F = (float)bi;
        if (bi + 1 < p.P) {
          const float nx = s_px[bi + 1], ny = s_py[bi + 1];
          const float sgx = nx - s_px[bi], sgy = ny - s_py[bi];
          const float d_next = (nx - x) * (nx - x) + (ny - y) * (ny - y);
          const float seg2 = sgx * sgx + sgy * sgy;
          const float tt = seg2 > 0.f ? 0.5f + 0.5f * (best - d_next) * fast_rcp(seg2) : 0.f;
          F = fmaxf(F + fminf(fmaxf(tt, -0.45f), 0.45f), 0.f);
        }
        return F;
      };
      float F = point_F();
      float m = flive ? F : 0.f;
      for (int o = 32; o > 0; o >>= 1) m = fmaxf(m, __shfl_xor(m, o, WAVE));
      if (kWindow && j_lo) {
        const unsigned long long holders = __ballot(flive && F == m);
        bool below = false;
        if (holders) {
          const int wl = __builtin_ctzll(holders);
          const float wx = __shfl(x, wl, WAVE), wy = __shfl(y, wl, WAVE), wbest = __shfl(best, wl, WAVE);
          for (uint32_t k = (uint32_t)lane; k < j_lo; k += WAVE) {
            const float ex = s_px[k] - wx, ey = s_py[k] - wy;
            below = below || (ex * ex + ey * ey <= wbest);
          }
        }
        if (__builtin_expect(__any(below), 0)) {
          for (uint32_t jj = j_lo; jj > 0; jj -= 4) {
            const uint32_t j = jj - 4;
            float dd[4];
            block_d2(s_px + j, s_py + j, dd);
            const float mn = fminf(fminf(dd[0], dd[1]), fminf(dd[2], dd[3]));
            if (mn <= best) {
              best = mn;
              bj = j;
            }
          }
          F = point_F();
          m = flive ? F : 0.f;
          for (int o = 32; o > 0; o >>= 1) m = fmaxf(m, __shfl_xor(m, o, WAVE));
        }
      }
      F_local = fmaxf(F_local, m);
      if constexpr (LANE_FURTHEST_PRUNE) {
        if (lane == 0)
          (void)__hip_atomic_fetch_max(reinterpret_cast<uint32_t*>(s_prune) + 2, __float_as_uint(m), __ATOMIC_RELAXED,
                                       __HIP_MEMORY_SCOPE_WORKGROUP);
        if (__builtin_expect(p.timeline != nullptr, 0) && lane == 0)
          p.timeline[SMPC_SCAN_COUNT_AT + blockIdx.x * 8 + wave] += 1ull;
      }
      }
      }
    }
```

mpcholonavigation_amd/csrc/smpc_lane_pass.inc:

```
template <bool FULL, bool OBST, bool MANY, int NCH, bool RR, bool GA = false, bool QUADS = FULL, int TC = 0, bool DEP = false>
__global__ void __launch_bounds__(RR ? LANE_BLOCK_RR : LANE_BLOCK, 1)
LANE_PASS_KERNEL(const SmpcDev p0, const SmpcLds L, const SmpcDev* __restrict__ many)
{
  constexpr bool POW = LANE_PASS_POW;
  constexpr bool NH = LANE_PASS_NH;
  static_assert(!NH || (OBST && !MANY && !RR && !GA && !DEP && !POW && NCH == 1 && QUADS),
                "no vy stream: the plain ObstaclesCritic rows of whole quads only");
  static_assert(RR || NCH == 1, "parked controls: one chunk of 64 steps");
  static_assert(!POW || (!MANY && !RR && !DEP), "cost powers: the single-context parking form of the five critics");
  static_assert(!FULL || QUADS, "T == 64 is a multiple of four");
  static_assert(TC == 0 || (!FULL && QUADS && !RR && TC < 64 && (TC & 3) == 0), "compile-time horizon: whole quads below 64");
  static_assert(!DEP || (OBST && !RR && !GA), "deployed-list instances: parking form");
  const SmpcDev& p = MANY ? many[blockIdx.y] : p0;
  const SmpcTickPtrs tk{p.u, p.px, p.py, p.pyaw, p.D, p.pf_idx, p.pvalid, p.pa_active, p.pang_active, p.pal_active};
  extern __shared__ __attribute__((aligned(16))) unsigned char smem[];
  uint8_t* s_map = smem;
  const SmpcLut* s_lut = reinterpret_cast<const SmpcLut*>(smem + L.off_lut);
  float* s_px = reinterpret_cast<float*>(smem + L.off_px);
  float* s_py = reinterpret_cast<float*>(smem + L.off_py);
  float* s_D = reinterpret_cast<float*>(smem + L.off_D) + 1;
  f32x4* s_pts4 = reinterpret_cast<f32x4*>(smem + L.off_pts4);
  float* s_su2 = reinterpret_cast<float*>(smem + L.off_scr) - 4;
  constexpr bool kPrune = !GA && !DEP && !MANY && !RR && !POW;
  float* s_prune = reinterpret_cast<float*>(smem + L.off_prune);

  constexpr int BLK = RR ? LANE_BLOCK_RR : LANE_BLOCK;
  const int blk = blockDim.x;
  const int tid = threadIdx.x;
  const int lane = tid & (WAVE - 1);
  const int wave = __builtin_amdgcn_readfirstlane(tid >> 6);
  const int nwave = blockDim.x >> 6;
  auto stamp = [&](int k) {
    if (__builtin_expect(p.timeline != nullptr, 0) && tid == 0)
      p.timeline[blockIdx.x * 8 + k] = __builtin_amdgcn_s_memtime();
  };
  stamp(0);
  float* park = reinterpret_cast<float*>(smem + L.off_scr) + (size_t)wave * L.scr_stride;
  float* s_w = park + 64 * LANE_PARK_STRIDE;

  {
    const int ww = OBST ? p.win_w : 0, wh = OBST ? p.win_h : 0;
    const bool vec = OBST && ((ww & 3) == 0) && ((p.W & 3u) == 0) && ((p.win_x0 & 3) == 0);
    const int w4 = OBST ? (ww >> 2) : 1, n4 = vec ? w4 * wh : 0;
    auto word = [&](int i) -> uint32_t {
      const int ry = i / w4, rx = i - ry * w4;
      return reinterpret_cast<const uint32_t*>(p.map + (size_t)(p.win_y0 + ry) * p.W + p.win_x0)[rx];
    };
    constexpr int kAhead = 96 * 96 / 4 / BLK + 1;
    uint32_t tmp[kAhead];
#pragma unroll
    for (int k = 0; k < kAhead; ++k) {
      const int i = tid + k * blk;
      tmp[k] = i < n4 ? word(i) : 0u;
    }
    const SmpcLut lut_e = (OBST && tid < 256) ? p.lut[tid] : SmpcLut{0.f, 0.f};
    const bool pt_on = (uint32_t)tid < p.P, seg_on = (uint32_t)tid + 1 < p.P;
    const float g_px = pt_on ? tk.px[tid] : 0.f, g_py = pt_on ? tk.py[tid] : 0.f;
    const float g_D = seg_on ? tk.D[tid] : 0.f;
    const bool g_valid = seg_on && tk.pvalid[tid] != 0;
    const float g_prune = (kPrune && tid < (int)SMPC_PRUNE_FLOATS) ? p.prune[tid] : 0.f;

    if (OBST) {
#pragma unroll
      for (int k = 0; k < kAhead; ++k) {
        const int i = tid + k * blk;
        if (i < n4) reinterpret_cast<uint32_t*>(s_map)[i] = tmp[k];
      }
      for (int i = tid + kAhead * blk; i < n4; i += blk)
        reinterpret_cast<uint32_t*>(s_map)[i] = word(i);
      if (!vec) {
        for (int i = tid; i < ww * wh; i += blockDim.x) {
          const int ry = i / ww, rx = i - ry * ww;
          s_map[i] = p.map[(size_t)(p.win_y0 + ry) * p.W + p.win_x0 + rx];
        }
      }
      if (tid < 256) const_cast<SmpcLut*>(s_lut)[tid] = lut_e;
      if (tid == 0) const_cast<SmpcLut*>(s_lut)[256] = SmpcLut{0.f, 0.f};
      if (tid == 0) s_map[ww * wh] = 255;
    }
    for (uint32_t i = p.P + tid; i < ((p.P + 3u) & ~3u); i += blockDim.x) s_px[i] = s_py[i] = 1.0e18f;
    if (kPrune && tid < (int)SMPC_PRUNE_FLOATS) s_prune[tid] = g_prune;
    if (pt_on) {
      s_px[tid] = g_px;
      s_py[tid] = g_py;
      if (seg_on) s_D[tid] = g_D;
      s_pts4[tid] = f32x4{g_px, g_py, g_valid ? 1.0f : 0.f, 0.f};
    }
    if (tid < WAVE) {
      float a = 0.f, b = 0.f, c = 0.f;
      const uint32_t Tn = FULL ? 64u * NCH : (TC ? (uint32_t)TC : p.T);
      for (uint32_t t = (uint32_t)tid; t < Tn; t += WAVE) {
        const float ux = tk.u[t], uy = NH ? 0.f : tk.u[Tn + t], uz = tk.u[2 * Tn + t];
        a = fmaf(ux, ux, a);
        b = fmaf(uy, uy, b);
        c = fmaf(uz, uz, c);
      }
      for (int o = 32; o > 0; o >>= 1) {
        a += __shfl_xor(a, o, WAVE);
        b += __shfl_xor(b, o, WAVE);
        c += __shfl_xor(c, o, WAVE);
      }
      if (tid == 0) {
        s_su2[0] = a;
        s_su2[1] = b;
        s_su2[2] = c;
      }
    }
    for (uint32_t i = tid + blk; i < p.P; i += blk) {
      const float qx = tk.px[i], qy = tk.py[i];
      const bool seg = i + 1 < p.P;
      s_px[i] = qx;
      s_py[i] = qy;
      if (seg) s_D[i] = tk.D[i];
      s_pts4[i] = f32x4{qx, qy, (seg && tk.pvalid[i]) ? 1.0f : 0.f, 0.f};
    }
  }
  __syncthreads();
  stamp(1);

  const cfloat_p cu = (cfloat_p)(uintptr_t)p.u;
  const uint32_t T = FULL ? 64u * NCH : (TC ? (uint32_t)TC : p.T), B = p.B;
  const uint32_t T4 = SMPC_GM_STEPS(T);
  const uint32_t noise_bytes = (uint32_t)SMPC_GM_ELEMS(B, T) * 4u;
  const __amdgpu_buffer_rsrc_t rn = __builtin_amdgcn_make_buffer_rsrc(const_cast<float*>(p.tvx), 0, 3u * noise_bytes, 0x00020000);
  const float dt = p.dt, yaw0 = p.yaw0;
  const double x0 = p.x0, y0 = p.y0;
  uint32_t S = 0;
  if (p.flags & SD_NEED_FURTHEST) {
    S = p.d_furthest ? smpc_furthest_index(*p.d_furthest) : p.furthest_hint;
    if (S >= p.P) S = p.P ? p.P - 1 : 0;
  }
  if (lane == 0) {
    s_D[-1] = -3.0e38f;
    s_D[S] = 3.0e38f;
  }
  const bool pa_on = (p.flags & SD_PATH_ALIGN) && p.P > 0 && tk.pa_active[S] && S > 0;
  float pf_x = 0.f, pf_y = 0.f;
  if ((p.flags & SD_PATH_FOLLOW) && p.P > 0) {
    const uint32_t idx = tk.pf_idx[S];
    pf_x = tk.px[idx];
    pf_y = tk.py[idx];
  }
  const uint32_t bs_iters = S > 1 ? 32u - (uint32_t)__builtin_clz(S - 1) : 0u;
  float pa_inv_spacing = 0.f;
  if (pa_on && S > 1 && tk.D[S - 1] > 0.f) pa_inv_spacing = (float)(S - 1) / tk.D[S - 1];
  const bool want_local_furthest = (p.flags & SD_NEED_FURTHEST) && (p.flags & SD_LOCAL_FURTHEST);
  const bool con_on = DEP && (p.flags & SD_CONSTRAINT) != 0, tw_on = DEP && (p.flags & SD_TWIRLING) != 0;
  const float k_con = p.dt * p.con_weight, k_tw = p.tw_weight / (float)(FULL ? 64 * NCH : (TC ? TC : (int)p.T));
  const bool cost_mode = DEP && (p.flags & SD_COST) != 0;
  constexpr bool ga_on = GA;
  const uint32_t nquad = (T + 3u) >> 2;

  float m_run = 3.0e38f, s_run = 0.f;
  float Ux[NCH], Uy[NCH], Uz[NCH];
#pragma unroll
  for (int h = 0; h < NCH; ++h) Ux[h] = Uy[h] = Uz[h] = 0.f;
  float F_local = 0.f;
  bool furthest_pending = false;
  uint32_t n_noncoll = 0;

  const uint32_t ngroups = (B + WAVE - 1) / WAVE;
  const uint32_t gw = blockIdx.x * nwave + wave;
  const uint32_t nW = gridDim.x * nwave;

  using T_ = std::true_type;
  using F_ = std::false_type;
  auto group_body = [&](auto safe_c, const uint32_t grp) -> bool {
    constexpr bool SAFE = decltype(safe_c)::value;
    const uint32_t b = grp * WAVE + lane;
    const bool live = b < B;
    const uint32_t bl = live ? b : B - 1;
    f32x32 PX0, PX1, PY0, PY1;
    if constexpr (NH) {
      if (!FULL) PX0 = PX1 = (f32x32)(0.f);
    } else if (!FULL && !RR) PX0 = PX1 = PY0 = PY1 = (f32x32)(0.f);

    float cpx = p.svx, cpy = NH ? 0.f : p.svy, cpz = p.swz;
    float acc_yaw = 0.f, ax = 0.f, ay = 0.f;
    float cs_prev = p.cos0, sn_prev = p.sin0;
    float x = 0.f, y = 0.f;
    float crit = 0.f, rep = 0.f;
    float yaw_max = 0.f;
    float alive = 1.0f;
    uint32_t cell_q = 256u;
    f32x2 e_q = {0.f, 0.f};
    auto lookup_wait = [&]() {};
    auto lookup_accumulate = [&]() {
      alive = e_q.x < 0.f ? 0.f : alive;
      crit = fmaf(alive, e_q.x, crit);
      rep = fmaf(alive, e_q.y, rep);
    };
    auto lookup_issue_entry = [&]() {
      const SmpcLut e = s_lut[cell_q];
      e_q = f32x2{e.crit, e.rep};
    };
    auto lookup_issue_byte = [&](uint32_t idx) {cell_q = s_map[idx];};
    float pfw = 0.f, gx = 0.f, gy = 0.f, gz = 0.f;
    float ga_sum = 0.f;
    float ext = 0.f;
    float traj_dist = 0.f, pa_sum = 0.f, pa_num = 0.f, sx_prev = p.x00f, sy_prev = p.y00f;
    uint32_t path_pt = 0;

    constexpr bool kCellVgpr = OBST && QUADS && (FULL || TC != 0) && !GA && !DEP && !MANY && !RR && !POW;
    const float k_rinv = p.rinvf, k_cx = kCellVgpr ? in_vgpr(p.cxf) : p.cxf, k_cy = kCellVgpr ? in_vgpr(p.cyf) : p.cyf;
    const float k_edge = 0.5f - p.cell_eps_w;
    constexpr bool kAddAtTop = FULL && !RR && (GA || (MANY && DEP));
    constexpr int kFetchAt = GA ? 3 : 1;
    auto do_step = [&](const uint32_t t, const bool sample_slot, const float ux, const float uy, const float uz,
                       const float n0, const float n1, const float n2, float& cvx, float& cvy,
                       float& cwz) __attribute__((always_inline)) {
      if constexpr (!kAddAtTop) {
        cvx = ux + n0;
        if constexpr (!NH) cvy = uy + n1;
        cwz = uz + n2;
      }
      const float vx = cpx, vy = cpy, wz = cpz;
      cpx = cvx;
      if constexpr (!NH) cpy = cvy;
      cpz = cwz;
      acc_yaw = acc_yaw + wz * dt;
      const float yaw = acc_yaw + yaw0;
      const float dxr = NH ? vx * cs_prev : vx * cs_prev - vy * sn_prev;
      const float dyr = NH ? vx * sn_prev : vx * sn_prev + vy * cs_prev;
      ax = ax + dxr * dt;
      ay = ay + dyr * dt;
      if constexpr (DEP) {
        if (con_on) {
          const float sp = fast_sqrt(vx * vx + vy * vy);
          const float vt = vx > 0.f ? sp : -sp;
          const float e = fmaxf(vt - p.con_max_vel, 0.f) + fmaxf(p.con_min_vel - vt, 0.f);
          ext = fmaf(e, k_con, ext);
        }
        if (tw_on) ext = fmaf(fabsf(wz), k_tw, ext);
      }
      if (ga_on) {
        const float a = p.ga_goal_yaw - yaw;
        const float kf = fmaf(a, 0.15915494309189535f, 12582912.0f);
        const float k = kf - 12582912.0f;
        float r = fmaf(-k, 6.2831854820251465f, a);
        r = fmaf(-k, -1.7484555e-07f, r);
        ga_sum += fabsf(r);
      }

      uint32_t idx = 0;
      if (OBST) {
        const float qx = fmaf(ax, k_rinv, k_cx), qy = fmaf(ay, k_rinv, k_cy);
        const float rx = __builtin_amdgcn_fractf(qx), ry = __builtin_amdgcn_fractf(qy);
        const int lx = cvt_floor_i32(qx), ly = cvt_floor_i32(qy);
        const float edge = fmaxf(fabsf(rx - 0.5f), fabsf(ry - 0.5f));
        const bool fast = (edge <= k_edge) &
                          ((uint32_t)lx < (uint32_t)p.win_w) & ((uint32_t)ly < (uint32_t)p.win_h);
        idx = __umul24((uint32_t)ly, (uint32_t)p.win_w) + (uint32_t)lx;
        if (__builtin_expect(__builtin_amdgcn_ballot_w64(!fast) != 0, 0)) {
          if (!fast)
            idx = cell_byte_exact(p, s_map, (float)(x0 + (double)ax), (float)(y0 + (double)ay),
                                  (uint32_t)(wave * WAVE + lane));
        }
      }

      if (SAFE) {
        smpc_sincos(yaw, sn_prev, cs_prev);
      } else {
        yaw_max = fmaxf(yaw_max, fabsf(yaw));
        smpc_sincos_fast(yaw, sn_prev, cs_prev);
      }
      pfw = add_min_zero(pfw, vx);
      gx = fmaf(ux, cvx, gx);
      gz = fmaf(uz, cwz, gz);
      if constexpr (!NH) gy = fmaf(uy, cvy, gy);

      if (sample_slot && pa_on && t != 0) {
        x = (float)(x0 + (double)ax);
        y = (float)(y0 + (double)ay);
        const float ddx = x - sx_prev, ddy = y - sy_prev;
        traj_dist += fast_sqrt(ddx * ddx + ddy * ddy);
        sx_prev = x;
        sy_prev = y;
        const float dist = traj_dist;
        uint32_t gi = (uint32_t)(dist * pa_inv_spacing);
        gi = gi < S ? gi : S - 1;
        const float da = s_D[(int)gi - 1];
        const float db = s_D[gi];
        const float dc = s_D[gi + 1];
        const bool c0 = da < dist, c1 = db < dist, c2 = dc < dist;
        uint32_t lo = gi + (c1 ? 1u : 0u);
        float dl = c1 ? db : da, dh = c1 ? dc : db;
        if (__builtin_expect(__builtin_amdgcn_ballot_w64(!c0 || c2) != 0, 0)) {
          uint32_t base = 0, nn = S;
          for (uint32_t it = 0; it < bs_iters; ++it) {
            const uint32_t half = nn >> 1;
            base = (s_D[base + half - 1 + (half == 0)] < dist && half) ? base + half : base;
            nn -= half;
          }
          const float d_base = s_D[base];
          lo = base + (d_base < dist ? 1u : 0u);
          dl = lo > 0 ? s_D[lo - 1] : 0.f;
          dh = lo < S ? s_D[lo] : 0.f;
        }
        uint32_t pt;
        if (lo == path_pt) pt = 0;
        else if (lo >= S) pt = S - 1;
        else pt = (dist - dl < dh - dist) ? lo - 1 : lo;
        path_pt = pt;
        const f32x4 q = s_pts4[pt];
        const float ex = q[0] - x, ey = q[1] - y;
        const float d = fast_sqrt(ex * ex + ey * ey);
        pa_num += q[2];
        pa_sum = fmaf(q[2], d, pa_sum);
      }
      if (OBST) {
        lookup_wait();
        lookup_accumulate();
        lookup_issue_entry();
        lookup_issue_byte(idx);
      }
    };

    const uint32_t loff = (bl >> 6) * (T4 * 256u) + (bl & 63u) * 16u;
    constexpr uint32_t quad_bytes = 1024u;
    auto ldq = [&](uint32_t tensor, uint32_t q) -> f32x4 {
      const uint32_t qc = (FULL || TC || q < nquad) ? q : nquad - 1;
      return __builtin_bit_cast(f32x4, __builtin_amdgcn_raw_buffer_load_b128(rn, loff, tensor * noise_bytes + qc * quad_bytes, 0));
    };
    auto ldu = [&](uint32_t ctrl, uint32_t t) -> float {return cu[ctrl * T + ((FULL || t < T) ? t : T - 1)];};
    f32x4 nq0, nq1, nq2;
    float uq[12];
    nq0 = ldq(0, 0);
    if constexpr (!NH) nq1 = ldq(1, 0);
    nq2 = ldq(2, 0);
#pragma unroll
    for (int i = 0; i < 4; ++i) {
#pragma unroll
      for (int k = 0; k < 3; ++k) {
        if constexpr (NH) {
          if (k == 1) continue;
        }
        uq[3 * i + k] = ldu(k, i);
      }
    }
    uint64_t clk = __builtin_amdgcn_s_memtime();
    auto run_quad = [&](auto hi_c, auto swap_c, const uint32_t q, float (&cq)[12]) __attribute__((always_inline)) {
      constexpr bool SWAP = decltype(swap_c)::value;
      if constexpr (SWAP) {
        __builtin_amdgcn_s_setprio(0);
        if (((uint32_t)(clk >> 15) + (uint32_t)(wave >> 2)) & 1u) __builtin_amdgcn_s_setprio(1);
        clk = __builtin_amdgcn_s_memtime();
      }
      float uc[12];
#pragma unroll
      for (int j = 0; j < 12; ++j) {
        if constexpr (NH) {
          if (j % 3 == 1) continue;
        }
        uc[j] = uq[j];
      }
      constexpr bool kAlwaysAhead = !FULL && TC == 0;
      if (kAlwaysAhead || q + 1 < nquad) {
#pragma unroll
        for (int i = 0; i < 4; ++i)
#pragma unroll
          for (int k = 0; k < 3; ++k) {
            if constexpr (NH) {
              if (k == 1) continue;
            }
            uq[3 * i + k] = ldu(k, 4 * (q + 1) + i);
          }
      }
      const f32x4 nc0 = nq0, nc1 = NH ? (f32x4)(0.f) : nq1, nc2 = nq2;
      if constexpr (kAddAtTop) {
#pragma unroll
        for (int i = 0; i < 4; ++i) {
          cq[3 * i] = uc[3 * i] + nc0[i];
          cq[3 * i + 1] = uc[3 * i + 1] + nc1[i];
          cq[3 * i + 2] = uc[3 * i + 2] + nc2[i];
        }
      }
      auto fetch = [&]() __attribute__((always_inline)) {
        if (kAlwaysAhead || q + 1 < nquad) {
          nq0 = ldq(0, q + 1);
          if constexpr (!NH) nq1 = ldq(1, q + 1);
          nq2 = ldq(2, q + 1);
        }
      };
      if constexpr (!kAddAtTop) fetch();
#pragma unroll
      for (int i = 0; i < 4; ++i) {
        const uint32_t t = 4 * q + i;
        if constexpr (kAddAtTop) {
          if (i == kFetchAt) {
            __builtin_amdgcn_sched_barrier(0);
            fetch();
            __builtin_amdgcn_sched_barrier(0);
          }
        }
        const float n0 = nc0[i], n1 = nc1[i], n2 = nc2[i];
        if constexpr (!kAddAtTop) cq[3 * i] = cq[3 * i + 1] = cq[3 * i + 2] = 0.f;
        if (QUADS || t < T)
          do_step(t, i == 0, uc[3 * i], NH ? 0.f : uc[3 * i + 1], uc[3 * i + 2], n0, n1, n2, cq[3 * i], cq[3 * i + 1],
                  cq[3 * i + 2]);
      }
    };
    constexpr bool kPairLoops = FULL || TC != 0;
#define LANE_PARK_QUAD(HI, Q) \
      if constexpr (!RR) { \
        _Pragma("unroll") for (int i = 0; i < 4; ++i) { \
          if constexpr (HI) { \
            PX1[8 * i + ((Q) - 8)] = cq[3 * i]; \
            if constexpr (!NH) PY1[8 * i + ((Q) - 8)] = cq[3 * i + 1]; \
          } else { \
            PX0[8 * i + (Q)] = cq[3 * i]; \
            if constexpr (!NH) PY0[8 * i + (Q)] = cq[3 * i + 1]; \
          } \
          park[(4 * (Q) + i) * LANE_PARK_STRIDE + lane] = cq[3 * i + 2]; \
        } \
      }
    if constexpr (kPairLoops) {
#define LANE_QUAD(HI, SWAP, Q) \
    { \
      float cq[12]; \
      run_quad(std::bool_constant<HI>{}, std::bool_constant<SWAP>{}, (Q), cq); \
      LANE_PARK_QUAD(HI, Q) \
    }
#define LANE_QUADS(HI, Q0, QE)    \
    { \
      uint32_t q = (Q0); \
      const uint32_t qe = (QE); \
      for (; q + 1 < qe; q += 2) { \
        LANE_QUAD(HI, true, q) \
        LANE_QUAD(HI, false, q + 1) \
      } \
      if (q < qe) LANE_QUAD(HI, true, q) \
    }
    if constexpr (RR) {
      LANE_QUADS(false, 0u, nquad)
    } else {
      LANE_QUADS(false, 0u, nquad < 8u ? nquad : 8u)
      LANE_QUADS(true, 8u, nquad)
    }
#undef LANE_QUADS
#undef LANE_QUAD
    } else if constexpr (RR) {
#pragma unroll 2
      for (uint32_t q = 0; q < nquad; ++q) {
        float cq[12];
        run_quad(F_{}, T_{}, q, cq);
      }
    } else {
      const uint32_t qh = nquad < 8u ? nquad : 8u;
      if constexpr (QUADS && !FULL && TC == 0) {
        auto quad_lo = [&](const uint32_t q) {
          float cq[12];
          run_quad(F_{}, T_{}, q, cq);
          LANE_PARK_QUAD(false, q)
        };
        auto quad_hi = [&](const uint32_t q) {
          float cq[12];
          run_quad(T_{}, T_{}, q, cq);
          LANE_PARK_QUAD(true, q)
        };
        uint32_t q = 0;
        for (; q + 1 < qh; q += 2) {
          quad_lo(q);
          quad_lo(q + 1);
        }
        if (q < qh) quad_lo(q);
        q = 8;
        for (; q + 1 < nquad; q += 2) {
          quad_hi(q);
          quad_hi(q + 1);
        }
        if (q < nquad) quad_hi(q);
      } else {
#pragma unroll 2
        for (uint32_t q = 0; q < qh; ++q) {
          float cq[12];
          run_quad(F_{}, T_{}, q, cq);
          LANE_PARK_QUAD(false, q)
        }
#pragma unroll 2
        for (uint32_t q = 8; q < nquad; ++q) {
          float cq[12];
          run_quad(T_{}, T_{}, q, cq);
          LANE_PARK_QUAD(true, q)
        }
      }
    }
#undef LANE_PARK_QUAD
    if (OBST) {
      lookup_wait();
      lookup_accumulate();
      lookup_issue_entry();
      lookup_wait();
      lookup_accumulate();
    }
    if (!SAFE && __builtin_expect(__any(!(yaw_max < 65536.0f) || !(fabsf(acc_yaw) < 65536.0f)), 0)) return true;

    x = (float)(x0 + (double)ax);
    y = (float)(y0 + (double)ay);

    if constexpr (!kPrune) {
#define LANE_FURTHEST_PRUNE false
#include "smpc_lane_furthest.inc"
#undef LANE_FURTHEST_PRUNE
    }
    float cost = (p.flags & SD_ACCUMULATE) ? p.costs_prev[bl] : 0.f;
    if constexpr (POW) {
      if (OBST) {
        const bool collided = alive == 0.f;
        const float raw = collided ? p.obs_collision_cost : crit;
        const float v = (p.obs_critical_w * raw) + (p.obs_repulsion_w * rep / (float)T);
        cost = add_cost_pow(cost, (double)v, p.obs_power);
        n_noncoll += (uint32_t)__popcll(__ballot(live && !collided));
      }
      if (pa_on) {
        const float c_pa = pa_num > 0.f ? pa_sum / pa_num : 0.f;
        cost = add_cost_pow(cost, (double)(c_pa * p.pa_weight), p.pa_power);
      }
      if (p.flags & SD_PATH_FOLLOW) {
        const double ddx = (double)(x - pf_x), ddy = (double)(y - pf_y);
        cost = add_cost_pow(cost, (double)in_vgpr(p.pf_weight) * sqrt_unscaled(ddx * ddx + ddy * ddy), p.pf_power);
      }
      if (ga_on) {
        const double Td = (FULL || TC) ? (double)T : (double)in_vgpr((float)T);
        cost = add_cost_pow(cost, (double)ga_sum / Td * (double)in_vgpr(p.ga_weight), p.ga_power);
      }
      if (p.flags & SD_PREFER_FORWARD) cost = add_cost_pow(cost, (double)((pfw * -dt) * p.pfw_weight), p.pfw_power);
      cost += p.g_vx * (gx - s_su2[0]);
      cost += p.g_wz * (gz - s_su2[2]);
      cost += p.g_vy * (gy - s_su2[1]);
    } else {
      float lin = 0.f, uni = 0.f;
      if (OBST) {
        const bool collided = alive == 0.f;
        if (cost_mode) {
          const float k = p.cost_w254 / (float)T;
          lin = collided ? 0.f : k * rep;
          uni = collided ? k * p.cost_collision_cost : 0.f;
        } else {
          lin = (collided ? 0.f : p.obs_critical_w * crit) + p.obs_rep_over_T * rep;
          uni = collided ? p.obs_critical_w * p.obs_collision_cost : 0.f;
        }
        n_noncoll += (uint32_t)__popcll(__ballot(live && !collided));
      }
      if constexpr (DEP) lin += ext;
      if (p.flags & SD_PATH_FOLLOW) {
        const float fdx = x - pf_x, fdy = y - pf_y;
        uni += p.pf_weight * fast_sqrt(fdx * fdx + fdy * fdy);
      }
      if (p.flags & SD_PREFER_FORWARD) lin += (pfw * -dt) * p.pfw_weight;
      if (ga_on) uni += (ga_sum / (float)T) * p.ga_weight;
      lin += p.g_vx * (gx - s_su2[0]);
      lin += p.g_wz * (gz - s_su2[2]);
      if constexpr (!NH) lin += p.g_vy * (gy - s_su2[1]);
      cost += uni + lin;
      if (pa_on) {
        const float c_pa = pa_num > 0.f ? pa_sum * fast_rcp(pa_num) : 0.f;
        cost += c_pa * p.pa_weight;
      }
    }
    if (live) p.costs[b] = cost;

    float cmin = live ? cost : 3.0e38f;
    for (int o = 32; o > 0; o >>= 1) cmin = fminf(cmin, __shfl_xor(cmin, o, WAVE));
    const float m_new = fminf(m_run, cmin);
    const float f = __builtin_amdgcn_exp2f(p.k2 * (m_run - m_new));
    const float w = live ? __builtin_amdgcn_exp2f(p.k2 * (cost - m_new)) : 0.f;
    float wsum = w;
    for (int o = 32; o > 0; o >>= 1) wsum += __shfl_xor(wsum, o, WAVE);
    s_run = fmaf(s_run, f, wsum);
    m_run = m_new;

    const LaneW lw = lane_weights(w, lane);
    if constexpr (RR) {
#pragma unroll
      for (int h = 0; h < NCH; ++h) {
#pragma unroll
        for (int ctrl = 0; ctrl < 3; ++ctrl) {
          float V[64];
#pragma unroll
          for (int j = 0; j < 16; ++j) {
            const f32x4 v = ldq(ctrl, 16u * h + j);
#pragma unroll
            for (int e = 0; e < 4; ++e) V[4 * j + e] = v[e];
          }
          __builtin_amdgcn_sched_barrier(0);
#pragma unroll
          for (int t = 0; t < 64; ++t) {
            const uint32_t tt = 64u * h + t;
            const float c = ldu(ctrl, tt) + V[t];
            V[t] = (FULL || tt < T) ? c : 0.f;
          }
          const float r = lane_reduce64(V, lw, lane);
          if (ctrl == 0) Ux[h] = fmaf(Ux[h], f, r);
          else if (ctrl == 1) Uy[h] = fmaf(Uy[h], f, r);
          else Uz[h] = fmaf(Uz[h], f, r);
        }
      }
    } else {
      {
        float V[64];
#pragma unroll
        for (int t = 0; t < 32; ++t) {
          V[t] = PX0[8 * (t & 3) + (t >> 2)];
          V[32 + t] = PX1[8 * (t & 3) + (t >> 2)];
        }
        Ux[0] = fmaf(Ux[0], f, lane_reduce64(V, lw, lane));
        if constexpr (!NH) {
#pragma unroll
          for (int t = 0; t < 32; ++t) {
            V[t] = PY0[8 * (t & 3) + (t >> 2)];
            V[32 + t] = PY1[8 * (t & 3) + (t >> 2)];
          }
          Uy[0] = fmaf(Uy[0], f, lane_reduce64(V, lw, lane));
        }
      }
      {
        s_w[lane] = w;
        __builtin_amdgcn_fence(__ATOMIC_RELEASE, "wavefront");
        __builtin_amdgcn_wave_barrier();
        __builtin_amdgcn_fence(__ATOMIC_ACQUIRE, "wavefront");
        const f32x4* row = reinterpret_cast<const f32x4*>(park + lane * LANE_PARK_STRIDE);
        float acc0 = 0.f, acc1 = 0.f;
#pragma unroll
        for (int bq = 0; bq < 16; bq += 2) {
          const f32x4 w0 = reinterpret_cast<const f32x4*>(s_w)[bq], c0 = row[bq];
          const f32x4 w1 = reinterpret_cast<const f32x4*>(s_w)[bq + 1], c1 = row[bq + 1];
#pragma unroll
          for (int e = 0; e < 4; ++e) {
            acc0 = fmaf(w0[e], c0[e], acc0);
            acc1 = fmaf(w1[e], c1[e], acc1);
          }
        }
        Uz[0] = fmaf(Uz[0], f, acc0 + acc1);
        __builtin_amdgcn_wave_barrier();
      }
    }
    if constexpr (kPrune) {
#define LANE_FURTHEST_PRUNE true
#include "smpc_lane_furthest.inc"
#undef LANE_FURTHEST_PRUNE
    }
    return false;
  };

  stamp(2);
  int stamp_k = 3;
  for (uint32_t grp = gw; grp < ngroups; grp += nW) {
    if (__builtin_expect(group_body(F_{}, grp), 0)) group_body(T_{}, grp);
    if (stamp_k < 5) stamp(stamp_k++);
  }

  if (__builtin_expect(p.timeline != nullptr, 0) && lane == 0)
    p.timeline[8192 + blockIdx.x * 8 + wave] = __builtin_amdgcn_s_memtime();
  __syncthreads();
  stamp(5);
  const uint32_t TL = 4 + 3 * T;
  float* myp = reinterpret_cast<float*>(smem + L.off_scr) + (size_t)wave * L.scr_stride;
  if (lane == 0) {
    myp[0] = m_run;
    myp[1] = s_run;
    myp[2] = F_local;
    myp[3] = (float)n_noncoll;
  }
#pragma unroll
  for (int h = 0; h < NCH; ++h) {
    const uint32_t tt = 64u * h + (uint32_t)lane;
    if (tt < T) {
      myp[4 + tt] = Ux[h];
      myp[4 + T + tt] = Uy[h];
      myp[4 + 2 * T + tt] = Uz[h];
    }
  }
  __syncthreads();
  const float* allp = reinterpret_cast<const float*>(smem + L.off_scr);
  float bm = 3.0e38f;
  for (int w = 0; w < nwave; ++w) bm = fminf(bm, allp[(size_t)w * L.scr_stride]);
  float* outp = p.partials + (size_t)blockIdx.x * TL;
  for (uint32_t i = tid; i < TL; i += blockDim.x) {
    float acc = 0.f;
    if (i == 0) {
      acc = bm;
    } else if (i == 2) {
      for (int w = 0; w < nwave; ++w) acc = fmaxf(acc, allp[(size_t)w * L.scr_stride + 2]);
    } else if (i == 3) {
      for (int w = 0; w < nwave; ++w) acc += allp[(size_t)w * L.scr_stride + 3];
    } else {
      for (int w = 0; w < nwave; ++w) {
        const float mw = allp[(size_t)w * L.scr_stride];
        const float sc = __builtin_amdgcn_exp2f(p.k2 * (mw - bm));
        acc += sc * allp[(size_t)w * L.scr_stride + i];
      }
    }
    smpc_store_partial(outp + i, acc);
  }
  stamp(6);
  if (!(p.flags & SD_ACCUMULATE) && blockIdx.x == 0 && tid == 0) outp[SMPC_CANARY_SLOT(T)] = cu[-4];
  if constexpr (!MANY && !RR) {
    if (p.tail) smpc_grid_tail<(RR ? LANE_BLOCK_RR : LANE_BLOCK) / 64>(p, smem);
  }
}
```

mpcholonavigation_amd/csrc/smpc_prepare.cpp:

```cpp
#include "smpc_ctx.h"

namespace smpc_impl {

TickLayout tick_layout(uint32_t T, uint32_t P)
{
  TickLayout l{};
  size_t o = 0;
  l.canary = o; o += 16;
  l.u = o; o += align_up(3 * T * 4, 16);
  l.px = o; o += align_up(P * 4, 16);
  l.py = o; o += align_up(P * 4, 16);
  l.pyaw = o; o += align_up(P * 4, 16);
  l.D = o; o += align_up(P * 4, 16);
  l.pf_idx = o; o += align_up(P * 4, 16);
  l.pvalid = o; o += align_up(P, 16);
  l.pa_active = o; o += align_up(P, 16);
  l.pang_active = o; o += align_up(P, 16);
  l.pal_active = o; o += align_up(P, 16);
  l.lut_cost = o; o += 256 * 4;
  l.prune = o; o += SMPC_PRUNE_FLOATS * 4;
  l.total = o;
  return l;
}

SmpcLds make_lds(uint32_t window_bytes, uint32_t P, uint32_t T, uint32_t nwave, bool with_map,
                 uint32_t nsamp)
{
  SmpcLds L{};
  uint32_t o = with_map ? align_up(window_bytes, 16) : 0;
  L.off_lut = o; o += with_map ? (256 + 2) * sizeof(SmpcLut) : 0;
  const uint32_t pf = align_up(std::max(P, 1u) * 4, 16);
  L.off_px = o; o += pf;
  L.off_py = o; o += pf;
  L.off_pyaw = o; o += pf;
  L.off_D = o; o += align_up((std::max(P, 1u) + 2) * 4, 16);
  L.off_valid = o; o += align_up(std::max(P, 1u), 16);
  L.off_scr = o;
  const uint32_t R = T <= 64 ? 1 : (T <= 128 ? 2 : 4);
  L.seg_shift = nsamp + 1 <= 16 ? 4 : (nsamp + 1 <= 32 ? 5 : 6);
  L.group = std::max(1u, std::min(64u >> L.seg_shift, 4u / R));
  L.scr_pts = 0;
  L.scr_ring = 3 * 64;
  L.scr_c = L.scr_ring + 2 * 64;
  L.scr_stride = align_up(std::max(L.scr_c + L.group * 3 * T, 4 + 3 * T), 4);
  o += nwave * L.scr_stride * 4;
  L.total = o;
  return L;
}

SmpcLds lane_lds(uint32_t window_bytes, uint32_t P, uint32_t T, bool rr)
{
  const uint32_t lblock = rr ? smpc_lane_block_rr() : smpc_lane_block();
  SmpcLds Lt = make_lds(window_bytes ? window_bytes + 1 + lblock : 0, P, T, lblock / 64,
                        window_bytes != 0, 0);
  Lt.off_prune = Lt.off_scr;
  Lt.off_pts4 = Lt.off_prune + SMPC_PRUNE_FLOATS * 4;
  Lt.off_scr = Lt.off_pts4 + align_up(std::max(P, 1u) * 16, 16) + 16;
  Lt.scr_stride = rr ? align_up(4u + 3u * T, 4) : align_up(std::max(64u * 68u + 64u, 4u + 3u * T), 4);
  Lt.total = Lt.off_scr + (lblock / 64) * Lt.scr_stride * 4;
  return Lt;
}

SmpcLds split_lds(uint32_t window_bytes, uint32_t P, uint32_t T, uint32_t nseg)
{
  const uint32_t lblock = smpc_split_block();
  SmpcLds Lt = make_lds(window_bytes ? window_bytes + 1 + lblock : 0, P, T, lblock / 64, window_bytes != 0, 0);
  Lt.off_pts4 = Lt.off_scr;
  Lt.off_scr += align_up(std::max(P, 1u) * 16, 16) + 16 + 3 * 64 * 4;
  Lt.scr_stride = align_up(std::max((nseg == 2 ? 2u : 1u) * (64u / nseg) * 64u, 4u + 3u * T), 4);
  Lt.total = Lt.off_scr + (lblock / 64) * Lt.scr_stride * 4;
  return Lt;
}

static float distance_to_obstacle(const HostCostmap& m, float cost, bool using_footprint = false)
{
  const float scale_factor = m.cost_scaling_factor;
  const float min_radius = m.inscribed_radius;
  float d = static_cast<float>(
    (static_cast<double>(scale_factor * min_radius) - std::log(static_cast<double>(cost)) +
    std::log(static_cast<double>(253.0f))) / static_cast<double>(scale_factor));
  if (!using_footprint) d -= min_radius;
  return d;
}

static void build_lut(const HostCostmap& m, const smpc_obstacles_params& p, bool near_goal, SmpcLut* lut,
                      bool consider_fp = false, bool using_fp = false, const float* cost_terms = nullptr)
{
  for (int v = 0; v < 256; ++v) {
    lut[v].crit = 0.f;
    lut[v].rep = 0.f;
    if (cost_terms) {
      if (v == SMPC_COST_LETHAL || (v == SMPC_COST_INSCRIBED && !consider_fp) ||
        (v == SMPC_COST_NO_INFORMATION && !m.track_unknown))
      {
        lut[v].crit = -1.0f;
      } else {
        lut[v].rep = cost_terms[v];
      }
      continue;
    }
    if (v == SMPC_COST_LETHAL || (v == SMPC_COST_INSCRIBED && !consider_fp) ||
      (v == SMPC_COST_NO_INFORMATION && !m.track_unknown))
    {
      lut[v].crit = -1.0f;
      continue;
    }
    if (v < 1) continue;
    if (m.inflation_radius == 0.0f || m.cost_scaling_factor == 0.0f) continue;
    const float d = distance_to_obstacle(m, static_cast<float>(v), using_fp);
    if (d < p.collision_margin_distance) {
      lut[v].crit = p.collision_margin_distance - d;
    } else if (!near_goal) {
      lut[v].rep = m.inflation_radius - d;
    }
  }
}

void build_prune_table(const float* px, const float* py, uint32_t P, uint32_t k0, bool on, float* out)
{
  const double u = 5.9604644775390625e-08;
  const uint32_t n = P > k0 ? std::min(P - k0, SMPC_PRUNE_ENTRIES) : 0u;
  memset(out, 0, SMPC_PRUNE_FLOATS * sizeof(float));
  memcpy(out, &k0, 4);
  memcpy(out + 1, &n, 4);
  for (uint32_t i = 0; i < n; ++i) {
    const uint32_t K = k0 + i;
    float* e = out + 4 + 8 * i;
    const double kx = px[K], ky = py[K];
    e[0] = px[K];
    e[1] = py[K];
    e[5] = -4.0f;
    if (!on) continue;
    const bool last = K + 1 >= P;
    double gx = 1.0, gy = 0.0;
    if (!last) {
      gx = static_cast<double>(px[K + 1]) - kx;
      gy = static_cast<double>(py[K + 1]) - ky;
    } else if (K > 0) {
      gx = kx - px[K - 1];
      gy = ky - py[K - 1];
    }
    const double seg = std::sqrt(gx * gx + gy * gy);
    if (!(seg > 0.0) || !std::isfinite(seg)) {
      if (!last) continue;
      gx = 1.0; gy = 0.0;
    } else {
      gx /= seg; gy /= seg;
    }
    const double R = 64.0 * (seg > 0.0 && std::isfinite(seg) ? seg : 1.0);
    double kappa = 0.0, rho = 1.0e30, m = 0.0;
    bool ok = true;
    for (uint32_t j = K + 1; j < P; ++j) {
      const double vx = static_cast<double>(px[j]) - kx, vy = static_cast<double>(py[j]) - ky;
      const double v2 = vx * vx + vy * vy;
      if (v2 >= 9.0 * R * R) continue;
      const double al = gx * vx + gy * vy, be = gx * vy - gy * vx;
      if (!(al > 0.0)) {
        ok = false;
        break;
      }
      const double ial = 1.0 / al, dj = 4.0 * R * R + 2.0 * v2;
      kappa = std::max(kappa, std::fabs(be) * ial);
      rho = std::min(rho, 0.5 * v2 * ial);
      m = std::max(m, 2.5 * u * (dj + 2.0 * R * R) * ial);
    }
    if (!ok || !std::isfinite(kappa) || kappa > 64.0) continue;
    const double rho_s = (rho - 4.0 * m) / R - 64.0 * u * (1.0 + kappa);
    double inv = 0.0, mb = 0.0;
    if (!last) {
      const double dsum = 2.0 * R * R + (1.4142136 * R + seg) * (1.4142136 * R + seg);
      inv = R / seg;
      mb = 2.0 * (0.5 * 5.0 * u * dsum / (seg * seg) + 10.0 * u * 92.0 + u + 16.0 * u * inv + 2.0 * u * 92.0);
    }
    e[2] = static_cast<float>(gx / R);
    e[3] = static_cast<float>(gy / R);
    e[4] = kappa > 0.0 ? std::nextafter(static_cast<float>(kappa * (1.0 + 4.0 * u)), 3.0e38f) : 0.f;
    e[6] = static_cast<float>(inv);
    e[7] = mb > 0.0 ? std::nextafter(static_cast<float>(mb), 3.0e38f) : 0.f;
    e[5] = std::nextafter(static_cast<float>(std::min(rho_s, 1.0e30)), -3.0e38f);
  }
}

void remember_furthest(smpc_ctx* c, const smpc_tick_in* in, float F)
{
  static const bool trace = getenv("SMPC_TRACE_FURTHEST") != nullptr;
  if (trace)
    fprintf(stderr, "[smpc furthest] true %.3f predicted %.3f (geometry %.3f, valid %d, drift %.3f)\n", F,
            c->pred.hint_Fp + c->pred.hint_drift, c->pred.hint_Fp, (int)c->pred.hint_Fp_valid, c->pred.hint_drift);
  const bool fresh_noise = c->noise_gen != c->pred.noise_gen_remembered;
  c->pred.noise_gen_remembered = c->noise_gen;
  float F_next = F;
  if (c->pred.hint_Fp_valid) {
    const float d = F - c->pred.hint_Fp;
    if (fresh_noise && std::fabs(d) < 2.f) {
      F_next = c->pred.hint_Fp + c->pred.hint_drift + 0.4f * (F - (c->pred.hint_Fp + c->pred.hint_drift));
      c->pred.hint_drift *= 0.5f;
    } else {
      c->pred.hint_drift = std::fabs(d) < 2.f ? d : 0.f;
    }
  } else {
    c->pred.hint_drift = 0.f;
  }
  c->pred.hint_Fp_valid = false;
  c->pred.hint_F = F_next;
  c->pred.hint = smpc_furthest_index(F_next);
  c->pred.hint_valid = true;
  c->pred.anchor_x = in->pose_x;
  c->pred.anchor_y = in->pose_y;
  c->pred.anchor_ex = c->pred.cur_ex;
  c->pred.anchor_ey = c->pred.cur_ey;
  c->pred.anchor_e_valid = c->pred.cur_e_valid;
  c->pred.cur_e_valid = false;
  c->pred.anchor_px.assign(in->path_x, in->path_x + in->path_len);
  c->pred.anchor_py.assign(in->path_y, in->path_y + in->path_len);
  c->pred.anchor_valid = true;
}

static void nominal_endpoint(const smpc_ctx* c, const smpc_tick_in* in, const float* u, double& ex, double& ey)
{
  const uint32_t T = c->cfg.time_steps;
  const double dt = c->cfg.model_dt;
  double co = std::cos(static_cast<double>(in->pose_yaw)), si = std::sin(static_cast<double>(in->pose_yaw));
  double x = 0.0, y = 0.0;
  double vx = in->speed_vx, vy = c->holonomic ? in->speed_vy : 0.0, wz = in->speed_wz;
  for (uint32_t t = 0; t < T; ++t) {
    x += (vx * co - vy * si) * dt;
    y += (vx * si + vy * co) * dt;
    const double a = wz * dt, a2 = a * a;
    const double ca = 1.0 - 0.5 * a2 + a2 * a2 * (1.0 / 24.0), sa = a * (1.0 - a2 * (1.0 / 6.0));
    const double cn = co * ca - si * sa;
    si = si * ca + co * sa;
    co = cn;
    vx = u[t];
    vy = c->holonomic ? u[T + t] : 0.0;
    wz = u[2 * T + t];
  }
  ex = in->pose_x + x;
  ey = in->pose_y + y;
}

void predict_hint(smpc_ctx* c, const smpc_tick_in* in, const float* u_in)
{
  c->pred.cur_e_valid = false;
  if (u_in) {
    nominal_endpoint(c, in, u_in, c->pred.cur_ex, c->pred.cur_ey);
    c->pred.cur_e_valid = true;
  }
  if (!c->pred.hint_valid || !c->pred.anchor_valid) return;
  const uint32_t P0 = static_cast<uint32_t>(c->pred.anchor_px.size()), P = in->path_len;
  c->pred.hint = smpc_furthest_index(c->pred.hint_F);
  if (c->pred.hint_is_this_ticks) {
    c->pred.hint_is_this_ticks = false;
    c->pred.hint_Fp = c->pred.hint_F - c->pred.hint_drift;
    c->pred.hint_Fp_valid = true;
    return;
  }
  c->pred.hint_Fp_valid = false;
  if (P0 < 2 || P < 1) return;
  const float* ox = c->pred.anchor_px.data();
  const float* oy = c->pred.anchor_py.data();
  auto d2 = [](float ax, float ay, float bx, float by) {return (ax - bx) * (ax - bx) + (ay - by) * (ay - by);};
  uint32_t k = 0;
  float best = std::numeric_limits<float>::max();
  for (uint32_t j = 0; j < P0; ++j) {
    const float d = d2(ox[j], oy[j], in->path_x[0], in->path_y[0]);
    if (d < best) {
      best = d;
      k = j;
    }
  }
  const uint32_t kn = k + 1 < P0 ? k + 1 : k - 1;
  const float seg_k = d2(ox[k], oy[k], ox[kn], oy[kn]);
  if (!(best <= 0.0625f * seg_k)) return;
  uint32_t S0 = c->pred.hint;
  if (S0 >= P0) S0 = P0 - 1;
  const uint32_t Sn = S0 + 1 < P0 ? S0 + 1 : S0 - 1;
  const float sx = (S0 + 1 < P0 ? 1.f : -1.f) * (ox[Sn] - ox[S0]), sy = (S0 + 1 < P0 ? 1.f : -1.f) * (oy[Sn] - oy[S0]);
  const float seg2 = sx * sx + sy * sy;
  if (!(seg2 > 0.f)) return;
  const bool by_endpoint = c->pred.cur_e_valid && c->pred.anchor_e_valid;
  const double dx = by_endpoint ? c->pred.cur_ex - c->pred.anchor_ex : in->pose_x - c->pred.anchor_x;
  const double dy = by_endpoint ? c->pred.cur_ey - c->pred.anchor_ey : in->pose_y - c->pred.anchor_y;
  const float disp = static_cast<float>(dx * sx + dy * sy) / seg2;
  if (!(std::fabs(disp) < (by_endpoint ? 8.f : 4.f))) return;
  const float Fp0 = c->pred.hint_F + disp - static_cast<float>(k);
  const float Fp = Fp0 + c->pred.hint_drift;
  c->pred.hint_Fp = Fp0;
  c->pred.hint_Fp_valid = true;
  long h = std::lround(Fp);
  if (h < 0) h = 0;
  if (h > static_cast<long>(P) - 1) h = static_cast<long>(P) - 1;
  c->pred.hint = static_cast<uint32_t>(h);
}

int check_tick(smpc_ctx* c, const smpc_tick_in* in)
{
  if (!c || !in) return SMPC_ERR_INVALID;
  if (!c->have_noise) return fail(c, SMPC_ERR_STATE, "no noise: call smpc_set_noise or smpc_seed");
  if (in->path_len > 0 && (!in->path_x || !in->path_y || !in->path_yaw))
    return fail(c, SMPC_ERR_INVALID, "path arrays missing");
  if (in->path_len > SMPC_MAX_PATH)
    return fail(c, SMPC_ERR_UNSUPPORTED, "path longer than SMPC_MAX_PATH (1024) points");
  if (!c->map.set && (c->critics.obstacles.enabled || c->critics.cost.enabled || !in->path_pts_valid))
    return fail(c, SMPC_ERR_STATE, "no costmap: call smpc_set_costmap");
  if (((c->critics.obstacles.enabled && c->critics.obstacles.consider_footprint) ||
    (c->critics.cost.enabled && c->critics.cost.consider_footprint)) && c->fp_x.empty())
    return fail(c, SMPC_ERR_STATE, "consider_footprint=true needs a footprint: call smpc_set_footprint");
  return SMPC_OK;
}

static int tick_gates(smpc_ctx* c, const smpc_tick_in* in, uint32_t& gates_out, uint32_t& nsamp_out)
{
  const uint32_t T = c->cfg.time_steps, P = in->path_len;
  const auto& cr = c->critics;
  const double rx = in->pose_x, ry = in->pose_y, gx = in->goal_x, gy = in->goal_y;
  uint32_t gates = 0;
  if (cr.obstacles.enabled) gates |= SD_OBSTACLES;
  if (cr.path_align.enabled && !within_tol(cr.path_align.threshold_to_consider, rx, ry, gx, gy))
    gates |= SD_PATH_ALIGN;
  if (cr.path_follow.enabled && P >= 2 &&
    !within_tol(cr.path_follow.threshold_to_consider, rx, ry, gx, gy))
    gates |= SD_PATH_FOLLOW;
// ... 248 lines not shown
  const bool force_split = c->knobs.pass == Knobs::kSplit;
  bool split_now = false;
  if (!pl.rr && mode_now == 0 && T >= 36 && !c->in_group && !c->knobs.no_split && !c->knobs.fused_reduce &&
      (!c->lane_forced || force_split)) {
    const uint32_t waves = static_cast<uint32_t>(c->num_cu) * (smpc_split_block() / 64u);
    uint32_t nseg = 0;
    if ((B + 15u) / 16u <= waves) nseg = 4;
    if (T != 64 && B < kSplitMinBatchShort && !force_split) nseg = 0;
    if (c->knobs.split_nseg == 2 || c->knobs.split_nseg == 4) nseg = (nseg || force_split) ? c->knobs.split_nseg : 0;
    if (nseg == 2 && T != 64) nseg = 4;
    if (!nseg && force_split) nseg = 4;
    if (nseg && split_select(gates, T, step, nseg)) {
      const SmpcLds Ls = split_lds(window_bytes, P, T, nseg);
      if (Ls.total <= kLdsPerCu) {
        const uint32_t occ_blocks = c->occ_split.get(split_occupancy_row(nseg)->fn, smpc_split_block(), Ls.total);
        const uint32_t per_block = smpc_split_rollouts_per_block(nseg);
        const uint32_t blocks = (B + per_block - 1) / per_block;
        const uint32_t resident = static_cast<uint32_t>(c->num_cu) * occ_blocks;
        split_now = true;
        pl.split_nseg = nseg;
        pl.split.lds = Ls;
        pl.split.block = smpc_split_block();
        pl.split.grid = std::max(1u, std::min(std::min(blocks, resident), kMaxGrid));
      }
    }
  }
  return split_now;
}

static bool lane_nonholonomic_rows(const smpc_ctx* c, uint32_t gates, int mode_now, uint32_t step, const PassPlan& pl,
                                   bool lane_now, bool split_now)
{
  const uint32_t T = c->cfg.time_steps, B = c->cfg.batch_size;
  return !c->holonomic && !c->knobs.nonholo_omni && lane_now && !split_now && mode_now == 0 && !pl.pow && !pl.rr &&
    !c->in_group && step == 4 && T <= 64 && (T & 3u) == 0 && B >= kLaneMinBatch &&
    [&] {
      const LaneInst* k = lane_select(gates, T, false, false, c->acker_r, false, true);
      return k && k->nh;
    }();
}

static int plan_launch(smpc_ctx* c, const smpc_tick_in* in, uint32_t gates, uint32_t nsamp, int& mode_out)
{
  const uint32_t B = c->cfg.batch_size, P = in->path_len;
  const uint32_t step = c->critics.path_align.trajectory_point_step;
  const uint32_t window_bytes = plan_window(c, in, gates, c->dev);
  const int mode_now = wave_mode(gates, c->critics, c->knobs);
  PassPlan pl;
  const int rc = plan_wave(c, window_bytes, P, nsamp, mode_now, pl);
  if (rc != SMPC_OK) return rc;

  pl.rr = lane_reread_form(c, gates);
  bool lane_now = lane_eligible(c, gates, mode_now, step);
  pl.pow = lane_power_rows(c, gates, mode_now, step, pl.rr);
  if (pl.pow) lane_now = true;
  if (lane_now) lane_now = plan_lane(c, in, window_bytes, pl);
  const bool split_now = lane_now && plan_split(c, gates, mode_now, step, window_bytes, P, pl);

  if (lane_now && !split_now && B < kLaneMinBatch && !c->lane_forced) lane_now = false;

  pl.pow = pl.pow && lane_now;
  pl.nh = lane_nonholonomic_rows(c, gates, mode_now, step, pl, lane_now, split_now);
  pl.kind = split_now ? PassPlan::kSplit : (lane_now ? PassPlan::kLane : PassPlan::kWave);
  c->plan = pl;
  mode_out = mode_now;
  return SMPC_OK;
}


struct TickBlock {
  uint8_t* h;
  float *px, *py, *pyaw, *D;
  uint32_t* pf_idx;
  uint8_t *pvalid, *pa_active, *pang_active, *pal_active;
  float *lut_cost, *prune;
};
static TickBlock tick_block(uint8_t* h, const TickLayout& tl)
{
  TickBlock b{};
  b.h = h;
  b.px = reinterpret_cast<float*>(h + tl.px);
  b.py = reinterpret_cast<float*>(h + tl.py);
  b.pyaw = reinterpret_cast<float*>(h + tl.pyaw);
  b.D = reinterpret_cast<float*>(h + tl.D);
  b.pf_idx = reinterpret_cast<uint32_t*>(h + tl.pf_idx);
  b.pvalid = h + tl.pvalid;
  b.pa_active = h + tl.pa_active;
  b.pang_active = h + tl.pang_active;
  b.pal_active = h + tl.pal_active;
  b.lut_cost = reinterpret_cast<float*>(h + tl.lut_cost);
  b.prune = reinterpret_cast<float*>(h + tl.prune);
  return b;
}

static void copy_plan(const TickBlock& b, const TickLayout& tl, const smpc_tick_in* in, const float* u_in, uint32_t T,
                      bool holonomic)
{
  const uint32_t P = in->path_len;
  uint8_t* h = b.h;
  memcpy(h + tl.u, u_in, 3 * T * sizeof(float));
  if (!holonomic) memset(h + tl.u + T * sizeof(float), 0, T * sizeof(float));
  if (P) {
    memcpy(b.px, in->path_x, P * 4);
    memcpy(b.py, in->path_y, P * 4);
    memcpy(b.pyaw, in->path_yaw, P * 4);
  }
}

struct FirstPoint {
  float yaw0, cos0, sin0, svx, svy, swz, x00, y00;
  uint32_t cost_t0;
};
static FirstPoint first_point(const smpc_tick_in* in, bool holonomic, float dt, const HostCostmap& map)
{
  const float yaw0 = in->pose_yaw;
  const float cos0 = cosf(yaw0), sin0 = sinf(yaw0);
  const float svx = static_cast<float>(in->speed_vx);
  const float svy = holonomic ? static_cast<float>(in->speed_vy) : 0.f;
  const float swz = static_cast<float>(in->speed_wz);
  const float dx0 = svx * cos0 - svy * sin0;
  const float dy0 = svx * sin0 + svy * cos0;
  const float x00 = static_cast<float>(in->pose_x + static_cast<double>(dx0 * dt));
  const float y00 = static_cast<float>(in->pose_y + static_cast<double>(dy0 * dt));
  uint32_t cost_t0 = SMPC_COST_NO_INFORMATION;
  if (map.set) {
    unsigned mx, my;
    if (world_to_map(map, x00, y00, mx, my))
      cost_t0 = map.cells[static_cast<size_t>(my) * map.W + mx];
  }
  return FirstPoint{yaw0, cos0, sin0, svx, svy, swz, x00, y00, cost_t0};
}


static void occupancy_gate(const float* px, const float* py, const uint8_t* pvalid, uint32_t P, float x00, float y00,
                           const smpc_path_align_params& q, uint8_t* active)
{
  size_t init = 0;
  float best = std::numeric_limits<float>::max();
  for (uint32_t j = 0; j < P; ++j) {
    const float ddx = px[j] - x00, ddy = py[j] - y00;
    const float d = ddx * ddx + ddy * ddy;
    if (d < best) {
      best = d;
      init = j;
    }
  }
  std::vector<uint32_t> inval(P + 1, 0);
  for (uint32_t i = 0; i < P; ++i) inval[i + 1] = inval[i] + ((i + 1 < P && !pvalid[i]) ? 1u : 0u);
  for (uint32_t S = 0; S < P; ++S) {
    bool on = S >= q.offset_from_furthest;
    if (on && S > init) {
      const unsigned int invalid_ctr = inval[S] - inval[init];
      const float range = static_cast<float>(static_cast<size_t>(S) - init);
      if (static_cast<float>(invalid_ctr) / range > q.max_path_occupancy_ratio && invalid_ctr > 2) on = false;
    }
    active[S] = on ? 1 : 0;
  }
}

static void path_follow_targets(const uint8_t* pvalid, uint32_t P, uint32_t offset_from_furthest, uint32_t* pf_idx)
{
  const size_t path_size = P - 1;
  for (uint32_t S = 0; S < P; ++S) {
    size_t idx = std::min(static_cast<size_t>(S) + offset_from_furthest, path_size);
    bool valid = false;
    while (!valid && idx < path_size - 1) {
      valid = pvalid[idx];
      if (!valid) idx++;
    }
    pf_idx[S] = static_cast<uint32_t>(idx);
  }
}

struct PathAngleGates {
  bool any_live;
  bool correct;
};
static PathAngleGates path_angle_gates(const float* px, const float* py, uint32_t P, const smpc_tick_in* in,
                                       const smpc_path_angle_params& q, uint8_t* pang_active)
{
  const double rx = in->pose_x, ry = in->pose_y;
  bool pang_correct = false, pang_any = false;
  bool reversing_allowed = true;
  if (std::fabs(q.vx_min) < 1e-6) reversing_allowed = false;
  else if (q.vx_min < 0.0f) reversing_allowed = true;
  bool forward_preference = q.forward_preference != 0;
  if (!reversing_allowed) forward_preference = true;
  pang_correct = reversing_allowed && !forward_preference;
  for (uint32_t S = 0; S < P; ++S) {
    const size_t idx = std::min(static_cast<size_t>(S) + q.offset_from_furthest,
                                static_cast<size_t>(P) - 1);
    const float pose_x = static_cast<float>(rx), pose_y = static_cast<float>(ry);
    const double point_x = px[idx], point_y = py[idx];
    const float yaw = atan2f(static_cast<float>(point_y - static_cast<double>(pose_y)),
                             static_cast<float>(point_x - static_cast<double>(pose_x)));
    auto norm = [](double a) {
      const double theta = std::fmod(a + M_PI, 2.0 * M_PI);
      return theta <= 0.0 ? theta + M_PI : theta - M_PI;
    };
    const double pyaw0 = static_cast<double>(in->pose_yaw);
    float ang = static_cast<float>(std::fabs(norm(pyaw0 - static_cast<double>(yaw))));
    if (!forward_preference) {
      const double b = std::fabs(norm(norm(pyaw0 + M_PI) - static_cast<double>(yaw)));
      ang = static_cast<float>(std::min(std::fabs(norm(pyaw0 - static_cast<double>(yaw))), b));
    }
    pang_active[S] = ang < q.max_angle_to_furthest ? 0 : 1;
    if (pang_active[S]) pang_any = true;
  }
  return PathAngleGates{pang_any, pang_correct};
}

static void cost_lut(const smpc_cost_params& q, bool near_goal_c, float* lut_cost)
{
  for (int v = 0; v < 256; ++v) {
    float t = 0.0f;
    if (v >= 1) {
      if (static_cast<float>(v) >= static_cast<float>(SMPC_COST_INSCRIBED)) t = q.critical_cost;
      else if (!near_goal_c) t = static_cast<float>(v);
    }
    lut_cost[v] = t;
  }
}

static float circumscribed_cost(const HostCostmap& map, double fp_circumscribed_radius, double fp_layer_scale)
{
  double result = -1.0;
  if (fp_layer_scale >= 0.0) {
    const double distance = fp_circumscribed_radius / map.res;
    unsigned char cost = 0;
    if (distance == 0) {
      cost = SMPC_COST_LETHAL;
    } else if (distance * map.res <= static_cast<double>(map.inscribed_radius)) {
      cost = SMPC_COST_INSCRIBED;
    } else {
      const double factor = std::exp(-1.0 * fp_layer_scale *
                                     (distance * map.res - static_cast<double>(map.inscribed_radius)));
      cost = static_cast<unsigned char>((SMPC_COST_INSCRIBED - 1) * factor);
    }
    result = cost;
  }
  return static_cast<float>(result);
}

static int upload_collision_luts(smpc_ctx* c, const smpc_tick_in* in, uint32_t gates, bool near_goal_cost,
                                 const float* lut_cost)
{
  const auto& cr = c->critics;
  const double rx = in->pose_x, ry = in->pose_y, gx = in->goal_x, gy = in->goal_y;
  if (gates & (SD_OBSTACLES | SD_COST)) {
    const bool near_goal = within_tol(cr.obstacles.near_goal_distance, rx, ry, gx, gy);
    const bool cost_only = (gates & SD_COST) && !(gates & SD_OBSTACLES) && !(gates & (SD_FP_OBSTACLES | SD_FP_COST));
    const uint64_t key = (c->map_version << 20) ^ (c->critics_version << 4) ^ (near_goal ? 1u : 0u) ^
      ((gates & (SD_FP_OBSTACLES | SD_FP_COST)) ? 2u : 0u) ^ (cost_only ? 4u : 0u) ^ (near_goal_cost ? 8u : 0u);
    if (!c->lut_valid || key != c->lut_key) {
      build_lut(c->map, cr.obstacles, near_goal, c->h_lut, false, false, cost_only ? lut_cost : nullptr);
      HIPCK(c, hipMemcpyAsync(c->d_lut, c->h_lut, 256 * sizeof(SmpcLut), hipMemcpyHostToDevice,
                              c->stream));
      if (gates & (SD_FP_OBSTACLES | SD_FP_COST)) {
        build_lut(c->map, cr.obstacles, near_goal, c->h_lut_fp, true, false);
        build_lut(c->map, cr.obstacles, near_goal, c->h_lut_fp + 256, true, true);
        HIPCK(c, hipMemcpyAsync(c->d_lut_fp, c->h_lut_fp, 512 * sizeof(SmpcLut), hipMemcpyHostToDevice,
                                c->stream));
      }
      c->lut_key = key;
      c->lut_valid = true;
    }
  }
  return SMPC_OK;
}

static size_t prune_table_for_tick(smpc_ctx* c, const TickBlock& b, const TickLayout& tl, uint32_t P)
{
  const float* px = b.px;
  const float* py = b.py;
  size_t tick_bytes = tl.total;
  constexpr uint32_t kPruneMaxPath = 256;
  float* table = b.prune;
  uint32_t k0 = (c->pred.hint_valid && c->pred.hint > SMPC_PRUNE_ENTRIES / 2) ? c->pred.hint - SMPC_PRUNE_ENTRIES / 2 : 0u;
  k0 = std::min(k0, P > SMPC_PRUNE_ENTRIES ? P - SMPC_PRUNE_ENTRIES : 0u);
  const bool read = c->plan.kind == PassPlan::kLane && !c->plan.rr && !c->plan.pow && !c->in_group && c->pred.hint_valid &&
    !(c->cfg.flags & SMPC_FLAG_NO_SPECULATION);
  if (!read || P > kPruneMaxPath) {
    memset(table, 0, 16);
    tick_bytes = tl.prune + 16;
  } else if (!c->knobs.furthest_prune) {
    build_prune_table(px, py, P, k0, false, table);
  } else if (c->prune_k0 == k0 && c->prune_px.size() == P && !memcmp(c->prune_px.data(), px, P * 4) &&
             !memcmp(c->prune_py.data(), py, P * 4)) {
    memcpy(table, c->prune_table, sizeof(c->prune_table));
  } else {
    build_prune_table(px, py, P, k0, true, table);
    memcpy(c->prune_table, table, sizeof(c->prune_table));
    c->prune_px.assign(px, px + P);
    c->prune_py.assign(py, py + P);
    c->prune_k0 = k0;
  }
  return tick_bytes;
}

struct HandOver {
  const uint8_t* base;
  bool inline_tick;
};
static int hand_over_tick_block(smpc_ctx* c, uint32_t gates, const TickLayout& tl, size_t tick_bytes, HandOver& ho)
{
  const uint32_t T = c->cfg.time_steps;
  uint8_t* h = c->h_tick;
  const bool inline_tick = !c->defer_upload && !c->use_tpr && T <= 64 && tl.lut_cost - tl.px <= SMPC_INLINE_TICK_CAP &&
    !c->knobs.no_inline_tick;
  const bool pinned_tick = c->knobs.pinned_tick && !c->defer_upload && !inline_tick;
  const uint8_t* const tb = pinned_tick ? h : c->d_tick;
  if (++c->tick_no == 0) ++c->tick_no;
  *reinterpret_cast<uint32_t*>(h + tl.canary) = c->tick_no;
  c->tick_used = tick_bytes;
  const bool bar = c->bar_tick && !c->defer_upload && !pinned_tick && !inline_tick;
  c->canary_expect = (!pinned_tick && !inline_tick && !c->knobs.fused_reduce) ? c->tick_no : 0u;
  if (bar) {
    if (c->launched) {
      HIPCK(c, hipStreamSynchronize(c->stream));
      c->launched = false;
    }
    if (c->knobs.stale_tick && c->tick_no == c->knobs.stale_tick) {
    } else {
      bar_copy(c->d_tick, h, tick_bytes);
      bar_flush(c);
    }
  } else if (!c->defer_upload && !pinned_tick) {
    if (!inline_tick)
      HIPCK(c, hipMemcpyAsync(c->d_tick, h, tick_bytes, hipMemcpyHostToDevice, c->stream));
    else if (gates & SD_COST)
      HIPCK(c, hipMemcpyAsync(c->d_tick + tl.lut_cost, h + tl.lut_cost, 256 * sizeof(float), hipMemcpyHostToDevice,
                              c->stream));
  }
  ho.base = tb;
  ho.inline_tick = inline_tick;
  return SMPC_OK;
}


static void fill_dev_state(smpc_ctx* c, const smpc_tick_in* in, uint32_t nsamp, uint32_t step, const FirstPoint& fp,
                           const TickLayout& tl, const uint8_t* tb)
{
  const uint32_t T = c->cfg.time_steps, B = c->cfg.batch_size, P = in->path_len;
  SmpcDev& d = c->dev;
  memset(&d, 0, sizeof(d));
  d.B = B; d.T = T; d.P = P; d.nsamp = nsamp; d.step = step;
  d.x0 = in->pose_x; d.y0 = in->pose_y;
  d.yaw0 = fp.yaw0; d.cos0 = fp.cos0; d.sin0 = fp.sin0;
  d.svx = fp.svx; d.svy = fp.svy; d.swz = fp.swz; d.dt = c->cfg.model_dt;
  d.nvx = c->d_nvx; d.nvy = c->d_nvy; d.nwz = c->d_nwz;
  d.tvx = c->d_tvx; d.tvy = c->d_tvy; d.twz = c->d_twz;
  d.u = reinterpret_cast<const float*>(tb + tl.u);
  d.traj_x = c->d_traj[0]; d.traj_y = c->d_traj[1]; d.traj_yaw = c->d_traj[2];
  d.map = c->d_map; d.W = c->map.W; d.H = c->map.H;
  d.ox = c->map.ox; d.oy = c->map.oy; d.res = c->map.res;
  d.cost_t0 = fp.cost_t0;
  d.x00f = fp.x00; d.y00f = fp.y00;
  {
    const double rinv = 1.0 / c->map.res;
    d.oxf = static_cast<float>(c->map.ox);
    d.oyf = static_cast<float>(c->map.oy);
    d.rinvf = static_cast<float>(rinv);
    const double e_o = std::max(std::fabs(c->map.ox - static_cast<double>(d.oxf)),
                                std::fabs(c->map.oy - static_cast<double>(d.oyf)));
    const double qmax = static_cast<double>(std::max(c->map.W, c->map.H)) + 2.0;
    const double eps = 2.0 * (e_o * rinv + 3.1 * 5.9604644775390625e-08 * qmax) + 1e-7;
    d.cell_eps = static_cast<float>(std::min(eps, 0.5));
  }
  d.lut = c->d_lut;
  d.px = reinterpret_cast<const float*>(tb + tl.px);
  d.py = reinterpret_cast<const float*>(tb + tl.py);
  d.pyaw = reinterpret_cast<const float*>(tb + tl.pyaw);
  d.D = reinterpret_cast<const float*>(tb + tl.D);
  d.pvalid = tb + tl.pvalid;
  d.pa_active = tb + tl.pa_active;
  d.pf_idx = reinterpret_cast<const uint32_t*>(tb + tl.pf_idx);
  d.prune = reinterpret_cast<const float*>(tb + tl.prune);
  d.lut_cost = reinterpret_cast<const float*>(tb + tl.lut_cost);
  d.pang_active = tb + tl.pang_active;
  d.pal_active = tb + tl.pal_active;
  d.timeline = c->d_timeline;
  d.canary_echo = c->canary_expect ? 1u : 0u;
  d.partials = c->d_partials;
  d.furthest_out = reinterpret_cast<uint32_t*>(c->d_furthest);
}

static void fill_dev_critics(smpc_ctx* c, const smpc_tick_in* in, const float* pyaw, bool near_goal_cost,
                             bool pang_correct)
{
  const uint32_t T = c->cfg.time_steps, P = in->path_len;
  const auto& cr = c->critics;
  SmpcDev& d = c->dev;
  d.obs_critical_w = cr.obstacles.critical_weight;
  d.obs_repulsion_w = cr.obstacles.repulsion_weight;
  d.obs_collision_cost = cr.obstacles.collision_cost;
  d.obs_rep_over_T = cr.obstacles.repulsion_weight / static_cast<float>(T);
  d.obs_power = cr.obstacles.cost_power;
  d.pa_weight = cr.path_align.cost_weight; d.pa_power = cr.path_align.cost_power;
  d.pf_weight = cr.path_follow.cost_weight; d.pf_power = cr.path_follow.cost_power;
  d.ga_weight = cr.goal_angle.cost_weight; d.ga_power = cr.goal_angle.cost_power;
  d.ga_goal_yaw = P ? pyaw[P - 1] : 0.f;
  d.pfw_weight = cr.prefer_forward.cost_weight; d.pfw_power = cr.prefer_forward.cost_power;
  d.con_weight = cr.constraint.cost_weight; d.con_power = cr.constraint.cost_power;
  {
    const float min_sgn = cr.constraint.vx_min > 0.0f ? 1.0f : -1.0f;
    d.con_max_vel = sqrtf(cr.constraint.vx_max * cr.constraint.vx_max + cr.constraint.vy_max * cr.constraint.vy_max);
    d.con_min_vel = min_sgn * sqrtf(cr.constraint.vx_min * cr.constraint.vx_min + cr.constraint.vy_max * cr.constraint.vy_max);
    d.con_acker_r = c->acker_r;
  }
  d.cost_w254 = cr.cost.cost_weight / 254.0f;
  d.cost_collision_cost = cr.cost.collision_cost; d.cost_power = cr.cost.cost_power;
  d.cost_critical = cr.cost.critical_cost;
  d.cost_near_goal = near_goal_cost ? 1u : 0u;
  d.goal_x = in->goal_x; d.goal_y = in->goal_y;
  d.goal_weight = cr.goal.cost_weight; d.goal_power = cr.goal.cost_power;
  d.tw_weight = cr.twirling.cost_weight; d.tw_power = cr.twirling.cost_power;
  d.pal_weight = cr.path_align_legacy.cost_weight;
  d.pal_power = cr.path_align_legacy.cost_power;
  {
    const uint32_t lstep = cr.path_align_legacy.trajectory_point_step;
    d.pal_eval = lstep ? static_cast<float>(T / lstep) : 0.f;
  }
  d.pang_weight = cr.path_angle.cost_weight; d.pang_power = cr.path_angle.cost_power;
  d.pang_offset = cr.path_angle.offset_from_furthest; d.pang_correct = pang_correct ? 1 : 0;
  d.db_vx = std::fabs(static_cast<double>(cr.velocity_deadband.deadband_velocities[0]));
  d.db_vy = c->holonomic ? std::fabs(static_cast<double>(cr.velocity_deadband.deadband_velocities[1])) : 0.0;
  d.db_wz = std::fabs(static_cast<double>(cr.velocity_deadband.deadband_velocities[2]));
  d.db_weight = cr.velocity_deadband.cost_weight; d.db_power = cr.velocity_deadband.cost_power;
  d.g_vx = c->cfg.gamma / powf(c->cfg.vx_std, 2);
  d.g_vy = c->holonomic ? c->cfg.gamma / powf(c->cfg.vy_std, 2) : 0.f;
  d.g_wz = c->cfg.gamma / powf(c->cfg.wz_std, 2);
  d.neg_inv_temp = -1 / c->cfg.temperature;
  d.k2 = d.neg_inv_temp * 1.4426950408889634f;
}

static void fill_dev_footprint_inline(smpc_ctx* c, uint32_t gates, const TickLayout& tl, bool inline_tick)
{
  const uint32_t T = c->cfg.time_steps;
  const uint8_t* h = c->h_tick;
  SmpcDev& d = c->dev;
  d.lut_fp = c->d_lut_fp;
  d.fp_n = static_cast<uint32_t>(c->fp_x.size());
  for (uint32_t i = 0; i < d.fp_n; ++i) {
    d.fp_x[i] = c->fp_x[i];
    d.fp_y[i] = c->fp_y[i];
  }
  d.fp_pic = 0.0f;
  if (gates & (SD_FP_OBSTACLES | SD_FP_COST))
    d.fp_pic = circumscribed_cost(c->map, c->fp_circumscribed_radius, c->fp_layer_scale);
  if (inline_tick) memcpy(d.u_arg, h + tl.u, 3 * T * sizeof(float));
  if (inline_tick) {
    d.tick_inline = 1;
    d.u_inline = 1;
    const size_t o = tl.px;
    d.io_px = static_cast<uint16_t>(tl.px - o); d.io_py = static_cast<uint16_t>(tl.py - o);
    d.io_pyaw = static_cast<uint16_t>(tl.pyaw - o); d.io_D = static_cast<uint16_t>(tl.D - o);
    d.io_pf_idx = static_cast<uint16_t>(tl.pf_idx - o); d.io_pvalid = static_cast<uint16_t>(tl.pvalid - o);
    d.io_pa_active = static_cast<uint16_t>(tl.pa_active - o); d.io_pang_active = static_cast<uint16_t>(tl.pang_active - o);
    d.io_pal_active = static_cast<uint16_t>(tl.pal_active - o);
    memcpy(d.tick_bytes, h + o, tl.lut_cost - o);
  }
}

int prepare_tick(smpc_ctx* c, const smpc_tick_in* in, const float* u_in)
{
  int rc = check_tick(c, in);
  if (rc != SMPC_OK) return rc;
  if (!u_in) return fail(c, SMPC_ERR_INVALID, "control sequence missing");
  rc = absorb_redraw(c);
  if (rc != SMPC_OK) return rc;
  const uint32_t T = c->cfg.time_steps, P = in->path_len;
  const auto& cr = c->critics;
  HIPCK(c, hipSetDevice(c->device));

  const TickLayout tl = tick_layout(T, std::max(P, 1u));
  if (tl.total > c->tick_cap) return fail(c, SMPC_ERR_INVALID, "tick block overflow");
  const TickBlock b = tick_block(c->h_tick, tl);
  copy_plan(b, tl, in, u_in, T, c->holonomic);

  uint32_t gates = 0, nsamp = 0;
  rc = tick_gates(c, in, gates, nsamp);
  if (rc != SMPC_OK) return rc;
  const double rx = in->pose_x, ry = in->pose_y, gx = in->goal_x, gy = in->goal_y;
  const uint32_t step = (gates & SD_PATH_ALIGN) || !(gates & SD_PATH_ALIGN_LEGACY) ? cr.path_align.trajectory_point_step
                                                                                    : cr.path_align_legacy.trajectory_point_step;
  path_tables(c->map, in, gates, b.px, b.py, b.pvalid, b.D);
  const FirstPoint fp = first_point(in, c->holonomic, c->cfg.model_dt, c->map);

  const uint32_t P1 = std::max(P, 1u);
  if (gates & SD_PATH_ALIGN) occupancy_gate(b.px, b.py, b.pvalid, P, fp.x00, fp.y00, cr.path_align, b.pa_active);
  else memset(b.pa_active, 0, P1);
  if (gates & SD_PATH_ALIGN_LEGACY) occupancy_gate(b.px, b.py, b.pvalid, P, fp.x00, fp.y00, cr.path_align_legacy, b.pal_active);
  else memset(b.pal_active, 0, P1);
  if (gates & SD_PATH_FOLLOW) path_follow_targets(b.pvalid, P, cr.path_follow.offset_from_furthest, b.pf_idx);
  else memset(b.pf_idx, 0, P1 * 4);
  PathAngleGates pang{false, false};
  if (gates & SD_PATH_ANGLE) pang = path_angle_gates(b.px, b.py, P, in, cr.path_angle, b.pang_active);
  else memset(b.pang_active, 0, P1);
  c->pang_any = pang.any_live;
  const bool near_goal_cost = (gates & SD_COST) && within_tol(cr.cost.near_goal_distance, rx, ry, gx, gy);
  if (gates & SD_COST) cost_lut(cr.cost, near_goal_cost, b.lut_cost);
  else memset(b.lut_cost, 0, 256 * 4);

  rc = upload_collision_luts(c, in, gates, near_goal_cost, b.lut_cost);
  if (rc != SMPC_OK) return rc;
  rc = wait_map_upload(c);
  if (rc != SMPC_OK) return rc;
  predict_hint(c, in, u_in);
  const size_t tick_bytes = prune_table_for_tick(c, b, tl, P);
  if (c->cfg.flags & SMPC_FLAG_PROFILE) HIPCK(c, hipEventRecord(c->ev0, c->stream));
  HandOver ho{};
  rc = hand_over_tick_block(c, gates, tl, tick_bytes, ho);
  if (rc != SMPC_OK) return rc;

  fill_dev_state(c, in, nsamp, step, fp, tl, ho.base);
  fill_dev_critics(c, in, b.pyaw, near_goal_cost, pang.correct);
  fill_dev_footprint_inline(c, gates, tl, ho.inline_tick);
  int mode_now = 0;
  rc = plan_launch(c, in, gates, nsamp, mode_now);
  if (rc != SMPC_OK) return rc;

  c->gate_flags = gates;
  c->two_coll_fp = (gates & SD_OBSTACLES) && (gates & SD_COST) && (gates & (SD_FP_OBSTACLES | SD_FP_COST));
  c->score_mode = mode_now;
  c->fail_in = in->fail_flag_in != 0;
  c->P = P;
  c->tick_ready = true;
  begin_limit_iteration(c, nullptr);
  return SMPC_OK;
}

}
```

Before: 6.152 billion.

## Move cold lane-kernel parameters into a device-side tick-block struct

Epilogue-only scalars (critic weights, powers, cost buffers, partials, timeline pointer) for the single-instance lane kernel now come from a SmpcLaneCold struct written into the uploaded tick block and read through a constant-address pointer, instead of from the large by-value SmpcDev kernel argument. Cost-buffer selection and timeline presence become flag bits, so the kernel no longer needs those pointers in the argument struct. The goal is to cut preloaded SGPR/kernarg pressure and scalar loads in the hot path, at the cost of extra scalar memory loads in the epilogue and a reordered host fill so the struct is written before upload.

```diff
diff --git a/mpcholonavigation_amd/csrc/smpc_api.cpp b/mpcholonavigation_amd/csrc/smpc_api.cpp
--- a/mpcholonavigation_amd/csrc/smpc_api.cpp
+++ b/mpcholonavigation_amd/csrc/smpc_api.cpp
@@ -248,6 +248,8 @@
   d.furthest_hint = furthest_hint;
   d.costs = c->d_costs[c->costs_cur];
   d.costs_prev = c->d_costs[c->costs_cur ^ 1];
+  if (c->costs_cur) d.flags |= SD_COSTS_SWAPPED;
+  if (d.timeline) d.flags |= SD_TIMELINE;
   fin = SmpcFinal{};
   fin.enabled = finish ? 1 : 0;
   fin.vx_max = c->c_vx_max; fin.vx_min = c->c_vx_min; fin.vy_max = c->c_vy; fin.wz_max = c->c_wz;
@@ -313,7 +315,7 @@
   if (pass.kind == PassPlan::kSplit) {
     HIPCK(c, split_launch(static_cast<const SplitInst*>(pass.inst), d, pass.geom->lds, nblk, c->stream));
   } else if (pass.kind == PassPlan::kLane) {
-    HIPCK(c, lane_launch(static_cast<const LaneInst*>(pass.inst), d, nullptr, 1, pass.geom->lds, nblk, pass.geom->block, c->stream));
+    HIPCK(c, lane_launch(static_cast<const LaneInst*>(pass.inst), d, c->cold_dev, nullptr, 1, pass.geom->lds, nblk, pass.geom->block, c->stream));
   } else {
     const int rc_rm = ensure_row_major(c);
     if (rc_rm != SMPC_OK) return rc_rm;
diff --git a/mpcholonavigation_amd/csrc/smpc_ctx.h b/mpcholonavigation_amd/csrc/smpc_ctx.h
--- a/mpcholonavigation_amd/csrc/smpc_ctx.h
+++ b/mpcholonavigation_amd/csrc/smpc_ctx.h
@@ -272,6 +272,7 @@
   bool bar_tick = false;
   volatile uint32_t* hdp_flush = nullptr;
   size_t tick_used = 0;
+  const SmpcLaneCold* cold_dev = nullptr;
   uint32_t tick_no = 0;
   uint32_t canary_expect = 0;
   bool launched = false;
@@ -340,7 +341,7 @@
 void free_ctx(smpc_ctx* c);
 
 struct TickLayout {
-  size_t u, px, py, pyaw, D, pf_idx, pvalid, pa_active, pang_active, pal_active, lut_cost, canary, prune, total;
+  size_t u, px, py, pyaw, D, pf_idx, pvalid, pa_active, pang_active, pal_active, lut_cost, canary, cold, prune, total;
 };
 TickLayout tick_layout(uint32_t T, uint32_t P);
 void build_prune_table(const float* px, const float* py, uint32_t P, uint32_t k0, bool on, float* out);
diff --git a/mpcholonavigation_amd/csrc/smpc_dev.h b/mpcholonavigation_amd/csrc/smpc_dev.h
--- a/mpcholonavigation_amd/csrc/smpc_dev.h
+++ b/mpcholonavigation_amd/csrc/smpc_dev.h
@@ -24,6 +24,8 @@
 #define SD_FP_COST 0x40000u
 #define SD_PATH_ALIGN_LEGACY 0x80000u
 #define SD_PAL_USE_PATH_YAW 0x100000u
+#define SD_COSTS_SWAPPED 0x200000u
+#define SD_TIMELINE 0x400000u
 #define SD_EXTRA_CRITICS (SD_CONSTRAINT | SD_COST | SD_GOAL | SD_TWIRLING | SD_PATH_ANGLE | SD_DEADBAND | \
                           SD_FP_OBSTACLES | SD_FP_COST | SD_PATH_ALIGN_LEGACY)
 
@@ -50,6 +52,21 @@
   uint32_t* done_counter;
   uint32_t seq;
 };
+
+struct SmpcLaneCold {
+  float* costs_ab[2];
+  float* partials;
+  unsigned long long* timeline;
+  uint32_t P;
+  float k2;
+  float g_vx, g_vy, g_wz;
+  float obs_critical_w, obs_repulsion_w, obs_collision_cost, obs_rep_over_T;
+  float cost_w254, cost_collision_cost;
+  float pa_weight, pf_weight, ga_weight, pfw_weight;
+  uint32_t obs_power, pa_power, pf_power, ga_power, pfw_power;
+  uint32_t pad[4];
+};
+static_assert(sizeof(SmpcLaneCold) % 16 == 0, "a whole number of 16-byte rows of the tick block");
 
 struct SmpcDev {
   uint32_t B, T, P;
@@ -150,6 +167,21 @@
   float u_arg[3 * 64] __attribute__((aligned(16)));
 };
 #define SMPC_INLINE_TICK_CAP 1536u
+static inline SmpcLaneCold smpc_lane_cold(const SmpcDev& d, float* costs_a, float* costs_b)
+{
+  SmpcLaneCold k{};
+  k.costs_ab[0] = costs_a; k.costs_ab[1] = costs_b;
+  k.partials = d.partials; k.timeline = d.timeline;
+  k.P = d.P; k.k2 = d.k2;
+  k.g_vx = d.g_vx; k.g_vy = d.g_vy; k.g_wz = d.g_wz;
+  k.obs_critical_w = d.obs_critical_w; k.obs_repulsion_w = d.obs_repulsion_w;
+  k.obs_collision_cost = d.obs_collision_cost; k.obs_rep_over_T = d.obs_rep_over_T;
+  k.cost_w254 = d.cost_w254; k.cost_collision_cost = d.cost_collision_cost;
+  k.pa_weight = d.pa_weight; k.pf_weight = d.pf_weight; k.ga_weight = d.ga_weight; k.pfw_weight = d.pfw_weight;
+  k.obs_power = d.obs_power; k.pa_power = d.pa_power; k.pf_power = d.pf_power; k.ga_power = d.ga_power;
+  k.pfw_power = d.pfw_power;
+  return k;
+}
 #define SMPC_MAX_GRID 2048u
 #define SMPC_CANARY_SLOT(T) (SMPC_MAX_GRID * (4u + 3u * (T)))
 #define SMPC_TAIL_MAX_GRID 512u
diff --git a/mpcholonavigation_amd/csrc/smpc_group.cpp b/mpcholonavigation_amd/csrc/smpc_group.cpp
--- a/mpcholonavigation_amd/csrc/smpc_group.cpp
+++ b/mpcholonavigation_amd/csrc/smpc_group.cpp
@@ -238,7 +238,7 @@
       HIPCK(c0, wave_launch_many(l.wave, d_dev, reinterpret_cast<const SmpcWaveGeom*>(g->d_all + g->off_geo) + l.first,
                                  l.count, l.grid, l.lds, pass_block(1), g->stream));
     } else {
-      HIPCK(c0, lane_launch(inst, c0->dev, d_dev, l.count, L, l.grid, g->ctxs[lane_first]->plan.lane.block, g->stream));
+      HIPCK(c0, lane_launch(inst, c0->dev, nullptr, d_dev, l.count, L, l.grid, g->ctxs[lane_first]->plan.lane.block, g->stream));
     }
     g->launched = true;
     if (l.count >= 2) g->batched_launches++;
diff --git a/mpcholonavigation_amd/csrc/smpc_inst.h b/mpcholonavigation_amd/csrc/smpc_inst.h
--- a/mpcholonavigation_amd/csrc/smpc_inst.h
+++ b/mpcholonavigation_amd/csrc/smpc_inst.h
@@ -22,7 +22,7 @@
 hipError_t wave_launch(const WaveInst* k, const SmpcDev& p, const SmpcLds& L, uint32_t grid, uint32_t block, hipStream_t st);
 hipError_t wave_launch_many(const WaveInst* k, const SmpcDev* d_many, const SmpcWaveGeom* d_geom, uint32_t n, uint32_t grid_max,
                             uint32_t lds_max, uint32_t block, hipStream_t st);
-hipError_t lane_launch(const LaneInst* k, const SmpcDev& p, const SmpcDev* d_many, uint32_t n, const SmpcLds& L,
+hipError_t lane_launch(const LaneInst* k, const SmpcDev& p, const SmpcLaneCold* d_cold, const SmpcDev* d_many, uint32_t n, const SmpcLds& L,
                        uint32_t grid, uint32_t block, hipStream_t st);
 hipError_t split_launch(const SplitInst* k, const SmpcDev& p, const SmpcLds& L, uint32_t grid, hipStream_t st);
 
diff --git a/mpcholonavigation_amd/csrc/smpc_lane.hip b/mpcholonavigation_amd/csrc/smpc_lane.hip
--- a/mpcholonavigation_amd/csrc/smpc_lane.hip
+++ b/mpcholonavigation_amd/csrc/smpc_lane.hip
@@ -187,16 +187,17 @@
   return lane_find(T == 64u, true, false, 1, false, false, T == 64u, 0, false);
 }
 
-hipError_t lane_launch(const LaneInst* k, const SmpcDev& p, const SmpcDev* d_many, uint32_t n, const SmpcLds& L,
+hipError_t lane_launch(const LaneInst* k, const SmpcDev& p, const SmpcLaneCold* d_cold, const SmpcDev* d_many, uint32_t n, const SmpcLds& L,
                        uint32_t grid, uint32_t block, hipStream_t st)
 {
   if (!k || k->many != (d_many != nullptr)) return hipErrorInvalidValue;
+  if (!d_many && !d_cold) return hipErrorInvalidValue;
   if (k->rr ? block != LANE_BLOCK_RR : (block != LANE_BLOCK && block != LANE_BLOCK / 2)) return hipErrorInvalidValue;
   auto b = [](bool v) {return v ? "true" : "false";};
   snprintf(smpc_last_pass_kernel, sizeof(smpc_last_pass_kernel), "smpc_pass_lane%s<%s, %s, %s, %d, %s, %s, %s, %d, %s>",
            k->pow ? "_pow" : (k->nh ? "_nh" : ""), b(k->full), b(k->obst), b(k->many), k->nch, b(k->rr), b(k->ga), b(k->quads), k->tc, b(k->dep));
   static const SmpcDev none{};
-  void* args[] = {const_cast<SmpcDev*>(d_many ? &none : &p), const_cast<SmpcLds*>(&L), &d_many};
+  void* args[] = {const_cast<SmpcDev*>(d_many ? &none : &p), const_cast<SmpcLds*>(&L), &d_many, &d_cold};
   return inst_launch(k->fn, d_many ? dim3(grid, n) : dim3(grid), block, args, L.total, st);
 }
 
diff --git a/mpcholonavigation_amd/csrc/smpc_lane_common.h b/mpcholonavigation_amd/csrc/smpc_lane_common.h
--- a/mpcholonavigation_amd/csrc/smpc_lane_common.h
+++ b/mpcholonavigation_amd/csrc/smpc_lane_common.h
@@ -13,6 +13,7 @@
 
 typedef unsigned u32x2 __attribute__((ext_vector_type(2)));
 typedef const float __attribute__((address_space(4))) * cfloat_p;
+typedef const SmpcLaneCold __attribute__((address_space(4))) * ccold_p;
 typedef float f32x32 __attribute__((ext_vector_type(32)));
 typedef float f32x4 __attribute__((ext_vector_type(4)));
 typedef float f32x2 __attribute__((ext_vector_type(2)));
diff --git a/mpcholonavigation_amd/csrc/smpc_lane_furthest.inc b/mpcholonavigation_amd/csrc/smpc_lane_furthest.inc
--- a/mpcholonavigation_amd/csrc/smpc_lane_furthest.inc
+++ b/mpcholonavigation_amd/csrc/smpc_lane_furthest.inc
@@ -52,7 +52,9 @@
       };
       float best = 3.4028234663852886e38f;
       uint32_t bj = 0;
-      const uint32_t P4 = (p.P + 3u) & ~3u;
+      LANE_COLD_HERE();
+      const uint32_t c_P = LANE_COLD(P);
+      const uint32_t P4 = (c_P + 3u) & ~3u;
       constexpr bool kWindow = !GA && !DEP && !MANY;
       const uint32_t j_lo = (kWindow && (S >> 2) > 3u) ? ((S >> 2) - 3u) << 2 : 0u;
       for (uint32_t j = j_lo; j < P4; j += 4) {
@@ -69,7 +71,7 @@
         block_d2(s_px + bj, s_py + bj, dd);
         const uint32_t bi = bj + (dd[0] == best ? 0u : dd[1] == best ? 1u : dd[2] == best ? 2u : dd[3] == best ? 3u : 0u);
         float F = (float)bi;
-        if (bi + 1 < p.P) {
+        if (bi + 1 < c_P) {
           const float nx = s_px[bi + 1], ny = s_py[bi + 1];
           const float sgx = nx - s_px[bi], sgy = ny - s_py[bi];
           const float d_next = (nx - x) * (nx - x) + (ny - y) * (ny - y);
@@ -114,8 +116,10 @@
         if (lane == 0)
           (void)__hip_atomic_fetch_max(reinterpret_cast<uint32_t*>(s_prune) + 2, __float_as_uint(m), __ATOMIC_RELAXED,
                                        __HIP_MEMORY_SCOPE_WORKGROUP);
-        if (__builtin_expect(p.timeline != nullptr, 0) && lane == 0)
-          p.timeline[SMPC_SCAN_COUNT_AT + blockIdx.x * 8 + wave] += 1ull;
+        if (__builtin_expect(timeline_on(), 0) && lane == 0) {
+          LANE_COLD_HERE();
+          LANE_COLD(timeline)[SMPC_SCAN_COUNT_AT + blockIdx.x * 8 + wave] += 1ull;
+        }
       }
       }
       }
diff --git a/mpcholonavigation_amd/csrc/smpc_lane_pass.inc b/mpcholonavigation_amd/csrc/smpc_lane_pass.inc
--- a/mpcholonavigation_amd/csrc/smpc_lane_pass.inc
+++ b/mpcholonavigation_amd/csrc/smpc_lane_pass.inc
@@ -1,6 +1,6 @@
 template <bool FULL, bool OBST, bool MANY, int NCH, bool RR, bool GA = false, bool QUADS = FULL, int TC = 0, bool DEP = false>
 __global__ void __launch_bounds__(RR ? LANE_BLOCK_RR : LANE_BLOCK, 1)
-LANE_PASS_KERNEL(const SmpcDev p0, const SmpcLds L, const SmpcDev* __restrict__ many)
+LANE_PASS_KERNEL(const SmpcDev p0, const SmpcLds L, const SmpcDev* __restrict__ many, const SmpcLaneCold* __restrict__ cold)
 {
   constexpr bool POW = LANE_PASS_POW;
   constexpr bool NH = LANE_PASS_NH;
@@ -13,6 +13,12 @@
   static_assert(!DEP || (OBST && !RR && !GA), "deployed-list instances: parking form");
   const SmpcDev& p = MANY ? many[blockIdx.y] : p0;
   const SmpcTickPtrs tk{p.u, p.px, p.py, p.pyaw, p.D, p.pf_idx, p.pvalid, p.pa_active, p.pang_active, p.pal_active};
+  constexpr bool kCold = !MANY;
+  const ccold_p ck0 = (ccold_p)(uintptr_t)cold;
+#define LANE_COLD_HERE() \
+  ccold_p ck = ck0; \
+  if constexpr (kCold) asm volatile("" : "+s"(ck))
+#define LANE_COLD(f) (kCold ? ck->f : p.f)
   extern __shared__ __attribute__((aligned(16))) unsigned char smem[];
   uint8_t* s_map = smem;
   const SmpcLut* s_lut = reinterpret_cast<const SmpcLut*>(smem + L.off_lut);
@@ -30,9 +36,12 @@
   const int lane = tid & (WAVE - 1);
   const int wave = __builtin_amdgcn_readfirstlane(tid >> 6);
   const int nwave = blockDim.x >> 6;
+  auto timeline_on = [&]() -> bool {return kCold ? (p.flags & SD_TIMELINE) != 0u : p.timeline != nullptr;};
   auto stamp = [&](int k) {
-    if (__builtin_expect(p.timeline != nullptr, 0) && tid == 0)
-      p.timeline[blockIdx.x * 8 + k] = __builtin_amdgcn_s_memtime();
+    if (__builtin_expect(timeline_on(), 0) && tid == 0) {
+      LANE_COLD_HERE();
+      LANE_COLD(timeline)[blockIdx.x * 8 + k] = __builtin_amdgcn_s_memtime();
+    }
   };
   stamp(0);
   float* park = reinterpret_cast<float*>(smem + L.off_scr) + (size_t)wave * L.scr_stride;
@@ -486,6 +495,29 @@
       }
     }
 #undef LANE_PARK_QUAD
+    LANE_COLD_HERE();
+#define LANE_EPI_FETCH(type, f) const type c_##f = kCold ? ck->f : type()
+#define LANE_EPI(f) (kCold ? c_##f : p.f)
+    LANE_EPI_FETCH(float, k2); LANE_EPI_FETCH(float, g_vx); LANE_EPI_FETCH(float, g_vy); LANE_EPI_FETCH(float, g_wz);
+    LANE_EPI_FETCH(float, pa_weight); LANE_EPI_FETCH(float, pf_weight); LANE_EPI_FETCH(float, pfw_weight);
+    LANE_EPI_FETCH(float, ga_weight);
+    LANE_EPI_FETCH(float, obs_critical_w); LANE_EPI_FETCH(float, obs_collision_cost);
+    LANE_EPI_FETCH(float, obs_repulsion_w); LANE_EPI_FETCH(float, obs_rep_over_T);
+    LANE_EPI_FETCH(float, cost_w254); LANE_EPI_FETCH(float, cost_collision_cost);
+    LANE_EPI_FETCH(uint32_t, obs_power); LANE_EPI_FETCH(uint32_t, pa_power); LANE_EPI_FETCH(uint32_t, pf_power);
+    LANE_EPI_FETCH(uint32_t, ga_power); LANE_EPI_FETCH(uint32_t, pfw_power);
+    float* c_costs;
+    const float* c_costs_prev;
+    if constexpr (kCold) {
+      float* const a = ck->costs_ab[0];
+      float* const b = ck->costs_ab[1];
+      const bool sw = (p.flags & SD_COSTS_SWAPPED) != 0u;
+      c_costs = sw ? b : a;
+      c_costs_prev = sw ? a : b;
+    } else {
+      c_costs = p.costs;
+      c_costs_prev = p.costs_prev;
+    }
     if (OBST) {
       lookup_wait();
       lookup_accumulate();
@@ -503,68 +535,68 @@
 #include "smpc_lane_furthest.inc"
 #undef LANE_FURTHEST_PRUNE
     }
-    float cost = (p.flags & SD_ACCUMULATE) ? p.costs_prev[bl] : 0.f;
+    float cost = (p.flags & SD_ACCUMULATE) ? c_costs_prev[bl] : 0.f;
     if constexpr (POW) {
       if (OBST) {
         const bool collided = alive == 0.f;
-        const float raw = collided ? p.obs_collision_cost : crit;
-        const float v = (p.obs_critical_w * raw) + (p.obs_repulsion_w * rep / (float)T);
-        cost = add_cost_pow(cost, (double)v, p.obs_power);
+        const float raw = collided ? LANE_EPI(obs_collision_cost) : crit;
+        const float v = (LANE_EPI(obs_critical_w) * raw) + (LANE_EPI(obs_repulsion_w) * rep / (float)T);
+        cost = add_cost_pow(cost, (double)v, LANE_EPI(obs_power));
         n_noncoll += (uint32_t)__popcll(__ballot(live && !collided));
       }
       if (pa_on) {
         const float c_pa = pa_num > 0.f ? pa_sum / pa_num : 0.f;
-        cost = add_cost_pow(cost, (double)(c_pa * p.pa_weight), p.pa_power);
+        cost = add_cost_pow(cost, (double)(c_pa * LANE_EPI(pa_weight)), LANE_EPI(pa_power));
       }
       if (p.flags & SD_PATH_FOLLOW) {
         const double ddx = (double)(x - pf_x), ddy = (double)(y - pf_y);
-        cost = add_cost_pow(cost, (double)in_vgpr(p.pf_weight) * sqrt_unscaled(ddx * ddx + ddy * ddy), p.pf_power);
+        cost = add_cost_pow(cost, (double)in_vgpr(LANE_EPI(pf_weight)) * sqrt_unscaled(ddx * ddx + ddy * ddy), LANE_EPI(pf_power));
       }
       if (ga_on) {
         const double Td = (FULL || TC) ? (double)T : (double)in_vgpr((float)T);
-        cost = add_cost_pow(cost, (double)ga_sum / Td * (double)in_vgpr(p.ga_weight), p.ga_power);
-      }
-      if (p.flags & SD_PREFER_FORWARD) cost = add_cost_pow(cost, (double)((pfw * -dt) * p.pfw_weight), p.pfw_power);
-      cost += p.g_vx * (gx - s_su2[0]);
-      cost += p.g_wz * (gz - s_su2[2]);
-      cost += p.g_vy * (gy - s_su2[1]);
+        cost = add_cost_pow(cost, (double)ga_sum / Td * (double)in_vgpr(LANE_EPI(ga_weight)), LANE_EPI(ga_power));
+      }
+      if (p.flags & SD_PREFER_FORWARD) cost = add_cost_pow(cost, (double)((pfw * -dt) * LANE_EPI(pfw_weight)), LANE_EPI(pfw_power));
+      cost += LANE_EPI(g_vx) * (gx - s_su2[0]);
+      cost += LANE_EPI(g_wz) * (gz - s_su2[2]);
+      cost += LANE_EPI(g_vy) * (gy - s_su2[1]);
     } else {
       float lin = 0.f, uni = 0.f;
       if (OBST) {
         const bool collided = alive == 0.f;
         if (cost_mode) {
-          const float k = p.cost_w254 / (float)T;
+          const float k = LANE_EPI(cost_w254) / (float)T;
           lin = collided ? 0.f : k * rep;
-          uni = collided ? k * p.cost_collision_cost : 0.f;
+          uni = collided ? k * LANE_EPI(cost_collision_cost) : 0.f;
         } else {
-          lin = (collided ? 0.f : p.obs_critical_w * crit) + p.obs_rep_over_T * rep;
-          uni = collided ? p.obs_critical_w * p.obs_collision_cost : 0.f;
+          lin = (collided ? 0.f : LANE_EPI(obs_critical_w) * crit) + LANE_EPI(obs_rep_over_T) * rep;
+          uni = collided ? LANE_EPI(obs_critical_w) * LANE_EPI(obs_collision_cost) : 0.f;
         }
         n_noncoll += (uint32_t)__popcll(__ballot(live && !collided));
       }
       if constexpr (DEP) lin += ext;
       if (p.flags & SD_PATH_FOLLOW) {
         const float fdx = x - pf_x, fdy = y - pf_y;
-        uni += p.pf_weight * fast_sqrt(fdx * fdx + fdy * fdy);
-      }
-      if (p.flags & SD_PREFER_FORWARD) lin += (pfw * -dt) * p.pfw_weight;
-      if (ga_on) uni += (ga_sum / (float)T) * p.ga_weight;
-      lin += p.g_vx * (gx - s_su2[0]);
-      lin += p.g_wz * (gz - s_su2[2]);
-      if constexpr (!NH) lin += p.g_vy * (gy - s_su2[1]);
+        uni += LANE_EPI(pf_weight) * fast_sqrt(fdx * fdx + fdy * fdy);
+      }
+      if (p.flags & SD_PREFER_FORWARD) lin += (pfw * -dt) * LANE_EPI(pfw_weight);
+      if (ga_on) uni += (ga_sum / (float)T) * LANE_EPI(ga_weight);
+      lin += LANE_EPI(g_vx) * (gx - s_su2[0]);
+      lin += LANE_EPI(g_wz) * (gz - s_su2[2]);
+      if constexpr (!NH) lin += LANE_EPI(g_vy) * (gy - s_su2[1]);
       cost += uni + lin;
       if (pa_on) {
         const float c_pa = pa_num > 0.f ? pa_sum * fast_rcp(pa_num) : 0.f;
-        cost += c_pa * p.pa_weight;
-      }
-    }
-    if (live) p.costs[b] = cost;
+        cost += c_pa * LANE_EPI(pa_weight);
+      }
+    }
+    if (live) c_costs[b] = cost;
 
     float cmin = live ? cost : 3.0e38f;
     for (int o = 32; o > 0; o >>= 1) cmin = fminf(cmin, __shfl_xor(cmin, o, WAVE));
     const float m_new = fminf(m_run, cmin);
-    const float f = __builtin_amdgcn_exp2f(p.k2 * (m_run - m_new));
-    const float w = live ? __builtin_amdgcn_exp2f(p.k2 * (cost - m_new)) : 0.f;
+    const float f = __builtin_amdgcn_exp2f(LANE_EPI(k2) * (m_run - m_new));
+    const float w = live ? __builtin_amdgcn_exp2f(LANE_EPI(k2) * (cost - m_new)) : 0.f;
     float wsum = w;
     for (int o = 32; o > 0; o >>= 1) wsum += __shfl_xor(wsum, o, WAVE);
     s_run = fmaf(s_run, f, wsum);
@@ -650,8 +682,10 @@
     if (stamp_k < 5) stamp(stamp_k++);
   }
 
-  if (__builtin_expect(p.timeline != nullptr, 0) && lane == 0)
-    p.timeline[8192 + blockIdx.x * 8 + wave] = __builtin_amdgcn_s_memtime();
+  if (__builtin_expect(timeline_on(), 0) && lane == 0) {
+    LANE_COLD_HERE();
+    LANE_COLD(timeline)[8192 + blockIdx.x * 8 + wave] = __builtin_amdgcn_s_memtime();
+  }
   __syncthreads();
   stamp(5);
   const uint32_t TL = 4 + 3 * T;
@@ -675,7 +709,9 @@
   const float* allp = reinterpret_cast<const float*>(smem + L.off_scr);
   float bm = 3.0e38f;
   for (int w = 0; w < nwave; ++w) bm = fminf(bm, allp[(size_t)w * L.scr_stride]);
-  float* outp = p.partials + (size_t)blockIdx.x * TL;
+  LANE_COLD_HERE();
+  const float b_k2 = LANE_COLD(k2);
+  float* outp = LANE_COLD(partials) + (size_t)blockIdx.x * TL;
   for (uint32_t i = tid; i < TL; i += blockDim.x) {
     float acc = 0.f;
     if (i == 0) {
@@ -687,7 +723,7 @@
     } else {
       for (int w = 0; w < nwave; ++w) {
         const float mw = allp[(size_t)w * L.scr_stride];
-        const float sc = __builtin_amdgcn_exp2f(p.k2 * (mw - bm));
+        const float sc = __builtin_amdgcn_exp2f(b_k2 * (mw - bm));
         acc += sc * allp[(size_t)w * L.scr_stride + i];
       }
     }
@@ -699,3 +735,7 @@
     if (p.tail) smpc_grid_tail<(RR ? LANE_BLOCK_RR : LANE_BLOCK) / 64>(p, smem);
   }
 }
+#undef LANE_EPI
+#undef LANE_EPI_FETCH
+#undef LANE_COLD
+#undef LANE_COLD_HERE
diff --git a/mpcholonavigation_amd/csrc/smpc_prepare.cpp b/mpcholonavigation_amd/csrc/smpc_prepare.cpp
--- a/mpcholonavigation_amd/csrc/smpc_prepare.cpp
+++ b/mpcholonavigation_amd/csrc/smpc_prepare.cpp
@@ -18,6 +18,7 @@
   l.pang_active = o; o += align_up(P, 16);
   l.pal_active = o; o += align_up(P, 16);
   l.lut_cost = o; o += 256 * 4;
+  l.cold = o; o += sizeof(SmpcLaneCold);
   l.prune = o; o += SMPC_PRUNE_FLOATS * 4;
   l.total = o;
   return l;
@@ -872,7 +873,9 @@
   const uint8_t* base;
   bool inline_tick;
 };
-static int hand_over_tick_block(smpc_ctx* c, uint32_t gates, const TickLayout& tl, size_t tick_bytes, HandOver& ho)
+template <class BeforeUpload>
+static int hand_over_tick_block(smpc_ctx* c, uint32_t gates, const TickLayout& tl, size_t tick_bytes, HandOver& ho,
+                                BeforeUpload before_upload)
 {
   const uint32_t T = c->cfg.time_steps;
   uint8_t* h = c->h_tick;
@@ -885,6 +888,9 @@
   c->tick_used = tick_bytes;
   const bool bar = c->bar_tick && !c->defer_upload && !pinned_tick && !inline_tick;
   c->canary_expect = (!pinned_tick && !inline_tick && !c->knobs.fused_reduce) ? c->tick_no : 0u;
+  ho.base = tb;
+  ho.inline_tick = inline_tick;
+  before_upload();
   if (bar) {
     if (c->launched) {
       HIPCK(c, hipStreamSynchronize(c->stream));
@@ -902,8 +908,6 @@
       HIPCK(c, hipMemcpyAsync(c->d_tick + tl.lut_cost, h + tl.lut_cost, 256 * sizeof(float), hipMemcpyHostToDevice,
                               c->stream));
   }
-  ho.base = tb;
-  ho.inline_tick = inline_tick;
   return SMPC_OK;
 }
 
@@ -946,6 +950,7 @@
   d.pa_active = tb + tl.pa_active;
   d.pf_idx = reinterpret_cast<const uint32_t*>(tb + tl.pf_idx);
   d.prune = reinterpret_cast<const float*>(tb + tl.prune);
+  c->cold_dev = reinterpret_cast<const SmpcLaneCold*>(tb + tl.cold);
   d.lut_cost = reinterpret_cast<const float*>(tb + tl.lut_cost);
   d.pang_active = tb + tl.pang_active;
   d.pal_active = tb + tl.pal_active;
@@ -1080,11 +1085,13 @@
   const size_t tick_bytes = prune_table_for_tick(c, b, tl, P);
   if (c->cfg.flags & SMPC_FLAG_PROFILE) HIPCK(c, hipEventRecord(c->ev0, c->stream));
   HandOver ho{};
-  rc = hand_over_tick_block(c, gates, tl, tick_bytes, ho);
+  rc = hand_over_tick_block(c, gates, tl, tick_bytes, ho, [&] {
+    fill_dev_state(c, in, nsamp, step, fp, tl, ho.base);
+    fill_dev_critics(c, in, b.pyaw, near_goal_cost, pang.correct);
+    const SmpcLaneCold cold = smpc_lane_cold(c->dev, c->d_costs[0], c->d_costs[1]);
+    memcpy(c->h_tick + tl.cold, &cold, sizeof(cold));
+  });
   if (rc != SMPC_OK) return rc;
-
-  fill_dev_state(c, in, nsamp, step, fp, tl, ho.base);
-  fill_dev_critics(c, in, b.pyaw, near_goal_cost, pang.correct);
   fill_dev_footprint_inline(c, gates, tl, ho.inline_tick);
   int mode_now = 0;
   rc = plan_launch(c, in, gates, nsamp, mode_now);
```

Result: no change. 6.181 billion, median of 6 (+0.5%).
